# kalsifer-742/sunray

Measured on AMD Instinct MI355X. Metric: Mray/s (closest-hit + any-hit queries traversed per second), 1920x1080, 1 spp, 1M-triangle scene, higher is better.
Workload: dtype f32; 1 GPU; procedural heightfield 999714 triangles (257872 BVH nodes), 1920x1080, 1 spp, full reference frame per step: raytracing_ris + raytracing_final, 10 bounces, 16 RIS candidates, ReSTIR DI+GI on; primary_hit_hand_off=True, parallelism=single GPU, frames_in_flight=2, last_frame_crc32=7e278857

## Files before the change

### sunray_amd/csrc/bvh_build.cpp

```cpp
#include <algorithm>
#include <chrono>
#include <cmath>
#include <cstring>
#include <future>

#include "bvh_layout.h"
#include "host.h"

namespace srh {

namespace {

struct Aabb {
    float lo[3], hi[3];
    void reset() { for (int a = 0; a < 3; a++) { lo[a] = INFINITY; hi[a] = -INFINITY; } }
    void add(const float* p) { for (int a = 0; a < 3; a++) { lo[a] = std::min(lo[a], p[a]); hi[a] = std::max(hi[a], p[a]); } }
    void add(const Aabb& b) { for (int a = 0; a < 3; a++) { lo[a] = std::min(lo[a], b.lo[a]); hi[a] = std::max(hi[a], b.hi[a]); } }
    float half_area() const {
        const float dx = hi[0] - lo[0], dy = hi[1] - lo[1], dz = hi[2] - lo[2];
        if (!(dx >= 0.0f)) return 0.0f;
        return dx * dy + dy * dz + dz * dx;
    }
};

#ifndef SR_SAH_BINS
#define SR_SAH_BINS 16
#endif
constexpr int kBins = SR_SAH_BINS;
constexpr uint32_t kLeafMax = srl::kLeafMax;
constexpr uint32_t kParallelMin = 1u << 15;

struct Builder {
    std::vector<Aabb> bounds;
    std::vector<float> centroid[3];
    std::vector<uint32_t> order;
    uint32_t max_depth;
    double root_area = 1.0;

    struct Sub {
        std::vector<float> nodes;
        uint32_t depth = 0;
        double cost = 0.0;
    };

    explicit Builder(uint32_t md) : max_depth(md) {}

    static int leaf_ref(uint32_t first, uint32_t count) { return (int)~((first << 3) | count); }

    static void put_box(float* n, int which, const Aabb& b) {
        float lo[3], hi[3];
        for (int a = 0; a < 3; a++) {
            lo[a] = std::nextafter(b.lo[a], -INFINITY);
            hi[a] = std::nextafter(b.hi[a], INFINITY);
        }
        if (which == 0) { n[0] = lo[0]; n[1] = hi[0]; n[2] = lo[1]; n[3] = hi[1]; n[8] = lo[2]; n[9] = hi[2]; }
        else { n[4] = lo[0]; n[5] = hi[0]; n[6] = lo[1]; n[7] = hi[1]; n[10] = lo[2]; n[11] = hi[2]; }
    }
    static void put_child(float* n, int which, int ref) { memcpy(n + 12 + which, &ref, 4); }

    Aabb range_bounds(uint32_t first, uint32_t count) const {
        Aabb b; b.reset();
        for (uint32_t i = first; i < first + count; i++) b.add(bounds[order[i]]);
        return b;
    }

    uint32_t partition(uint32_t first, uint32_t count, uint32_t depth) {
        const uint32_t last = first + count;
        uint32_t need = 0;
        for (uint32_t c = (count + kLeafMax - 1) / kLeafMax; c > 1; c = (c + 1) / 2) need++;
        const bool force_median = depth + need + 1 >= max_depth;
        Aabb cb; cb.reset();
        for (uint32_t i = first; i < last; i++) {
            const uint32_t id = order[i];
            const float c[3] = {centroid[0][id], centroid[1][id], centroid[2][id]};
            cb.add(c);
        }
        int best_axis = -1, best_bin = -1;
        float best_cost = INFINITY;
        if (!force_median) {
            for (int ax = 0; ax < 3; ax++) {
                const float lo = cb.lo[ax], ext = cb.hi[ax] - cb.lo[ax];
                if (!(ext > 0.0f)) continue;
                const float scale = (float)kBins * (1.0f - 1e-6f) / ext;
                Aabb bb[kBins]; uint32_t bc[kBins];
                for (int b = 0; b < kBins; b++) { bb[b].reset(); bc[b] = 0; }
                for (uint32_t i = first; i < last; i++) {
                    const uint32_t id = order[i];
                    int b = (int)((centroid[ax][id] - lo) * scale);
                    b = b < 0 ? 0 : (b >= kBins ? kBins - 1 : b);
                    bb[b].add(bounds[id]); bc[b]++;
                }
                float ra[kBins]; uint32_t rc[kBins];
                Aabb acc; acc.reset(); uint32_t n = 0;
                for (int b = kBins - 1; b >= 1; b--) { acc.add(bb[b]); n += bc[b]; ra[b] = acc.half_area(); rc[b] = n; }
                acc.reset(); n = 0;
                for (int b = 0; b < kBins - 1; b++) {
                    acc.add(bb[b]); n += bc[b];
                    if (n == 0 || rc[b + 1] == 0) continue;
                    const float cost = acc.half_area() * (float)n + ra[b + 1] * (float)rc[b + 1];
                    if (cost < best_cost) { best_cost = cost; best_axis = ax; best_bin = b; }
                }
            }
        }
        if (best_axis >= 0) {
            const float lo = cb.lo[best_axis], ext = cb.hi[best_axis] - cb.lo[best_axis];
            const float scale = (float)kBins * (1.0f - 1e-6f) / ext;
            const std::vector<float>& cen = centroid[best_axis];
            auto mid_it = std::partition(order.begin() + first, order.begin() + last, [&](uint32_t id) {
                int b = (int)((cen[id] - lo) * scale);
                b = b < 0 ? 0 : (b >= kBins ? kBins - 1 : b);
                return b <= best_bin;
            });
            const uint32_t mid = (uint32_t)(mid_it - order.begin());
            if (mid != first && mid != last) return mid;
        }
        int ax = 0;
        float e = cb.hi[0] - cb.lo[0];
        for (int a = 1; a < 3; a++) if (cb.hi[a] - cb.lo[a] > e) { e = cb.hi[a] - cb.lo[a]; ax = a; }
        const uint32_t mid = first + count / 2;
        const std::vector<float>& cen = centroid[ax];
        std::nth_element(order.begin() + first, order.begin() + mid, order.begin() + last,
                         [&](uint32_t a, uint32_t b) { return cen[a] < cen[b] || (cen[a] == cen[b] && a < b); });
        return mid;
    }

    void build_sub(uint32_t first, uint32_t count, uint32_t depth, Sub& out) {
        const uint32_t mid = partition(first, count, depth);
        const uint32_t cnt[2] = {mid - first, first + count - mid};
        const uint32_t beg[2] = {first, mid};
        const bool par = cnt[0] >= kParallelMin && cnt[1] >= kParallelMin && depth < 4;
        if (!par) {
            emit_node(beg, cnt, depth, out, out);
            return;
        }
        Sub child[2];
        std::future<void> fut = std::async(std::launch::async, [&] { build_sub(beg[1], cnt[1], depth + 1, child[1]); });
        build_sub(beg[0], cnt[0], depth + 1, child[0]);
        fut.get();
        out.nodes.assign(16, 0.0f);
        uint32_t below = 0;
        for (int c = 0; c < 2; c++) {
            const Aabb cb = range_bounds(beg[c], cnt[c]);
            put_box(&out.nodes[0], c, cb);
            out.cost += cb.half_area() / root_area;
            const size_t at = out.nodes.size();
            const int off = (int)(at / 16);
            out.nodes.insert(out.nodes.end(), child[c].nodes.begin(), child[c].nodes.end());
            for (size_t n = at; n < out.nodes.size(); n += 16)
                for (int k = 0; k < 2; k++) {
                    int ref; memcpy(&ref, &out.nodes[n + 12 + k], 4);
                    if (ref >= 0) { ref += off; memcpy(&out.nodes[n + 12 + k], &ref, 4); }
                }
            std::vector<float>().swap(child[c].nodes);
            out.cost += child[c].cost;
            below = std::max(below, child[c].depth);
            put_child(&out.nodes[0], c, off);
        }
        out.depth = below + 1;
    }
    void emit_node(const uint32_t beg[2], const uint32_t cnt[2], uint32_t depth, Sub& arr, Sub& stats) {
        const size_t self = arr.nodes.size();
        arr.nodes.resize(self + 16, 0.0f);
        uint32_t below = 0;
        for (int c = 0; c < 2; c++) {
            const Aabb cb = range_bounds(beg[c], cnt[c]);
            put_box(&arr.nodes[self], c, cb);
            stats.cost += cb.half_area() / root_area * (cnt[c] <= kLeafMax ? (double)cnt[c] : 1.0);
            if (cnt[c] <= kLeafMax) { put_child(&arr.nodes[self], c, leaf_ref(beg[c], cnt[c])); continue; }
            const int ref = (int)(arr.nodes.size() / 16);
            Sub sub_stats;
            build_sub_inplace(beg[c], cnt[c], depth + 1, arr, sub_stats);
            stats.cost += sub_stats.cost;
            below = std::max(below, sub_stats.depth);
            put_child(&arr.nodes[self], c, ref);
        }
        stats.depth = below + 1;
    }
    void build_sub_inplace(uint32_t first, uint32_t count, uint32_t depth, Sub& arr, Sub& stats) {
        const uint32_t mid = partition(first, count, depth);
        const uint32_t cnt[2] = {mid - first, first + count - mid};
        const uint32_t beg[2] = {first, mid};
        emit_node(beg, cnt, depth, arr, stats);
    }
};

}

namespace {
struct Child4 { float lo[3], hi[3]; int ref; };
inline Child4 child_of(const float* n2, int which) {
    Child4 c;
    if (which == 0) { c.lo[0] = n2[0]; c.hi[0] = n2[1]; c.lo[1] = n2[2]; c.hi[1] = n2[3]; c.lo[2] = n2[8]; c.hi[2] = n2[9]; }
    else { c.lo[0] = n2[4]; c.hi[0] = n2[5]; c.lo[1] = n2[6]; c.hi[1] = n2[7]; c.lo[2] = n2[10]; c.hi[2] = n2[11]; }
    memcpy(&c.ref, n2 + 12 + which, 4);
    return c;
}
inline float area_of(const Child4& c) {
    const float dx = c.hi[0] - c.lo[0], dy = c.hi[1] - c.lo[1], dz = c.hi[2] - c.lo[2];
    if (!(dx >= 0.0f)) return -1.0f;
    return dx * dy + dy * dz + dz * dx;
}
constexpr double kGuardCells = 1.0 / 32.0;

struct Collapser {
    const std::vector<float>& n2;
    std::vector<uint32_t>& out;
    std::vector<uint8_t> height;
    uint32_t max_depth = 0;
    uint32_t height_of(int node2) {
        uint32_t h = 0;
        for (int c = 0; c < 2; c++) {
            int ref; memcpy(&ref, &n2[(size_t)node2 * 16 + 12 + c], 4);
            if (ref >= 0) h = std::max(h, height_of(ref));
        }
        height[node2] = (uint8_t)(h + 1);
        return h + 1;
    }
    uint32_t need_of(const Child4& c) const { return c.ref >= 0 ? height[c.ref] : 0u; }
    uint32_t emit(int node2, uint32_t depth, uint32_t budget, int* out_index) {
        constexpr int W = srl::kBvhWidth;
        Child4 kids[W];
        int nk = 0;
        kids[nk++] = child_of(&n2[(size_t)node2 * 16], 0);
        kids[nk++] = child_of(&n2[(size_t)node2 * 16], 1);
        while (nk < W) {
            int best = -1; float best_area = -1.0f;
            for (int i = 0; i < nk; i++) if (kids[i].ref >= 0) { const float a = area_of(kids[i]); if (a > best_area) { best_area = a; best = i; } }
            if (best < 0) break;
            const Child4 ca = child_of(&n2[(size_t)kids[best].ref * 16], 0), cb = child_of(&n2[(size_t)kids[best].ref * 16], 1);
            bool fits = need_of(ca) + (uint32_t)nk <= budget && need_of(cb) + (uint32_t)nk <= budget;
            for (int i = 0; i < nk && fits; i++) if (i != best && need_of(kids[i]) + (uint32_t)nk > budget) fits = false;
            if (!fits) break;
            kids[best] = ca;
            kids[nk++] = cb;
        }
        bool real[W];
        int n_real = 0;
        float lo_n[3] = {INFINITY, INFINITY, INFINITY}, hi_n[3] = {-INFINITY, -INFINITY, -INFINITY};
        for (int i = 0; i < W; i++) real[i] = false;
        for (int i = 0; i < nk; i++) {
            const bool empty_leaf = kids[i].ref < 0 && ((~(uint32_t)kids[i].ref) & 7u) == 0u;
            real[i] = !empty_leaf;
            if (!real[i]) continue;
            n_real++;
            for (int a = 0; a < 3; a++) { lo_n[a] = std::min(lo_n[a], kids[i].lo[a]); hi_n[a] = std::max(hi_n[a], kids[i].hi[a]); }
        }
        const size_t self = out.size();
        *out_index = (int)(self / srl::kNodeDwords);
        out.resize(self + srl::kNodeDwords, 0u);
        max_depth = std::max(max_depth, depth);
        uint32_t plane[6 * srl::kPlaneDwords];
        for (auto& v : plane) v = 0u;
        uint32_t exps = 0;
        float origin[3] = {0.0f, 0.0f, 0.0f};
        if (n_real > 0) {
            for (int a = 0; a < 3; a++) {
                origin[a] = std::nextafter(lo_n[a] - (hi_n[a] - lo_n[a]) * (1.0f / 2048.0f), -INFINITY);
                const float ext = hi_n[a] - origin[a];
                int e = -126;
                if (ext > 0.0f && ext / 255.0f > 0.0f) { int fe; (void)std::frexp(ext / 255.0f, &fe); e = std::max(fe, -126); }
                for (;;) {
                    const float scale = std::ldexp(1.0f, e);
                    bool ok = true;
                    for (int i = 0; i < nk && ok; i++) {
                        if (!real[i]) continue;
                        int qh = (int)std::ceil(((double)kids[i].hi[a] - (double)origin[a]) / (double)scale + kGuardCells);
                        qh = std::max(qh, 0);
                        while (qh <= 255 && fmaf((float)qh, scale, origin[a]) < kids[i].hi[a]) qh++;
                        if (qh > 255) ok = false;
                    }
                    if (ok) break;
                    e++;
                }
                const float scale = std::ldexp(1.0f, e);
                exps |= (uint32_t)(e + 127) << (8 * a);
                for (int i = 0; i < W; i++) {
                    uint32_t ql = 255u, qh = 0u;
                    if (i < nk && real[i]) {
                        int l = (int)std::floor(((double)kids[i].lo[a] - (double)origin[a]) / (double)scale - kGuardCells);
                        l = std::min(std::max(l, 0), 255);
                        while (l > 0 && fmaf((float)l, scale, origin[a]) > kids[i].lo[a]) l--;
                        int h = (int)std::ceil(((double)kids[i].hi[a] - (double)origin[a]) / (double)scale + kGuardCells);
                        h = std::max(h, 0);
                        while (fmaf((float)h, scale, origin[a]) < kids[i].hi[a]) h++;
                        ql = (uint32_t)l; qh = (uint32_t)h;
                    }
                    plane[a * srl::kPlaneDwords + i / 4] |= ql << (8 * (i % 4));
                    plane[(3 + a) * srl::kPlaneDwords + i / 4] |= qh << (8 * (i % 4));
                }
            }
        } else {
            for (int a = 0; a < 3; a++) {
                for (int d = 0; d < srl::kPlaneDwords; d++) { plane[a * srl::kPlaneDwords + d] = 0xFFFFFFFFu; plane[(3 + a) * srl::kPlaneDwords + d] = 0u; }
                exps |= 127u << (8 * a);
            }
        }
        uint32_t below = 0;
        int refs[W];
        for (int i = 0; i < W; i++) {
            refs[i] = Builder::leaf_ref(0, 0);
            if (i < nk && real[i]) {
                if (kids[i].ref >= 0) {
                    int idx = 0;
                    below = std::max(below, emit(kids[i].ref, depth + 1, budget - (uint32_t)(n_real - 1), &idx));
                    refs[i] = idx;
                } else refs[i] = kids[i].ref;
            }
        }
        uint32_t* q = &out[self];
        memcpy(q + 0, origin, 12); q[3] = exps;
        memcpy(q + srl::kPlaneOffset, plane, sizeof(plane));
        memcpy(q + srl::kChildOffset, refs, sizeof(refs));
        return below + (uint32_t)std::max(n_real - 1, 0);
    }
};
}

static void collapse_to_bvh4(BvhResult& res, uint32_t stack_budget) {
    res.nodes.clear();
    Collapser c{res.nodes2, res.nodes, {}, 0};
    c.height.assign(res.nodes2.size() / 16, 0);
    c.height_of(0);
    int root = 0;
    res.max_stack = c.emit(0, 1, stack_budget, &root);
    res.max_depth = c.max_depth;
    res.n_nodes = (uint32_t)(res.nodes.size() / srl::kNodeDwords);
}

void flatten_instances(const std::vector<HostMesh>& meshes, const FrameInstanceData& fid, std::vector<BuildTri>& out) {
    out.clear();
    out.reserve(fid.n_triangles);
    for (uint32_t ii = 0; ii < fid.instances.size(); ii++) {
        const HostInstance& inst = fid.instances[ii];
        const HostMesh& mesh = meshes[inst.mesh_slot];
        const float* m = inst.o2w.m;
        const uint32_t nprim = mesh.n_indices / 3;
        for (uint32_t p = 0; p < nprim; p++) {
            float w[3][3];
            for (int j = 0; j < 3; j++) {
                const float* q = mesh.vertices[mesh.indices[3 * p + j]].position;
                w[j][0] = ((m[0] * q[0] + m[1] * q[1]) + m[2] * q[2]) + m[3] * 1.0f;
                w[j][1] = ((m[4] * q[0] + m[5] * q[1]) + m[6] * q[2]) + m[7] * 1.0f;
                w[j][2] = ((m[8] * q[0] + m[9] * q[1]) + m[10] * q[2]) + m[11] * 1.0f;
            }
            BuildTri t;
            for (int a = 0; a < 3; a++) { t.v0[a] = w[0][a]; t.e1[a] = w[1][a] - w[0][a]; t.e2[a] = w[2][a] - w[0][a]; }
            t.prim = p; t.inst = ii; t.gid = inst.tri_offset + p;
            out.push_back(t);
        }
    }
}

namespace {
void build_core(Builder& b, uint32_t n, const Aabb& root, uint32_t max_depth, BvhResult& res) {
    b.root_area = std::max((double)root.half_area(), 1e-30);
    Builder::Sub top;
    if (n <= kLeafMax) {
        top.nodes.assign(16, 0.0f);
        if (n > 0) Builder::put_box(top.nodes.data(), 0, root);
        else { float* q = top.nodes.data(); q[0] = q[2] = q[8] = INFINITY; q[1] = q[3] = q[9] = -INFINITY; }
        { float* q = top.nodes.data(); q[4] = q[6] = q[10] = INFINITY; q[5] = q[7] = q[11] = -INFINITY; }
        Builder::put_child(top.nodes.data(), 0, Builder::leaf_ref(0, n));
        Builder::put_child(top.nodes.data(), 1, Builder::leaf_ref(0, 0));
        top.depth = 1;
        top.cost = (double)n;
    } else {
        b.build_sub(0, n, 0, top);
    }
    res.nodes2.swap(top.nodes);
    res.sah_cost = (float)top.cost;
    collapse_to_bvh4(res, max_depth);
    res.order = b.order;
}
}

void build_bvh(const std::vector<BuildTri>& tris, uint32_t max_depth, BvhResult& res) {
    const auto t_start = std::chrono::steady_clock::now();
    const uint32_t n = (uint32_t)tris.size();
    Builder b(max_depth);
    b.bounds.resize(n);
    for (int a = 0; a < 3; a++) b.centroid[a].resize(n);
    b.order.resize(n);
    Aabb root; root.reset();
    for (uint32_t i = 0; i < n; i++) {
        const BuildTri& t = tris[i];
        float p1[3], p2[3];
        for (int a = 0; a < 3; a++) { p1[a] = t.v0[a] + t.e1[a]; p2[a] = t.v0[a] + t.e2[a]; }
        Aabb bb; bb.reset(); bb.add(t.v0); bb.add(p1); bb.add(p2);
        for (int a = 0; a < 3; a++) {
            const float pad = 4e-6f * (std::fabs(t.e1[a]) + std::fabs(t.e2[a]));
            bb.lo[a] -= pad; bb.hi[a] += pad;
        }
        b.bounds[i] = bb;
        for (int a = 0; a < 3; a++) b.centroid[a][i] = 0.5f * bb.lo[a] + 0.5f * bb.hi[a];
        b.order[i] = i;
        root.add(bb);
    }
    build_core(b, n, root, max_depth, res);
    res.tris.resize((size_t)n * 12);
    for (uint32_t i = 0; i < n; i++) {
        const BuildTri& t = tris[b.order[i]];
        float* q = &res.tris[(size_t)i * 12];
        q[0] = t.v0[0]; q[1] = t.v0[1]; q[2] = t.v0[2]; q[3] = t.e1[0];
        q[4] = t.e1[1]; q[5] = t.e1[2]; q[6] = t.e2[0]; q[7] = t.e2[1];
        q[8] = t.e2[2];
        memcpy(q + 9, &t.gid, 4);
        q[10] = 0.0f; q[11] = 0.0f;
    }
    res.build_ms = std::chrono::duration<double, std::milli>(std::chrono::steady_clock::now() - t_start).count();
}

void build_bvh_boxes(const std::vector<BuildBox>& boxes, uint32_t max_depth, BvhResult& res) {
    const auto t_start = std::chrono::steady_clock::now();
    const uint32_t n = (uint32_t)boxes.size();
    Builder b(max_depth);
    b.bounds.resize(n);
    for (int a = 0; a < 3; a++) b.centroid[a].resize(n);
    b.order.resize(n);
    Aabb root; root.reset();
    for (uint32_t i = 0; i < n; i++) {
        Aabb bb;
        for (int a = 0; a < 3; a++) { bb.lo[a] = boxes[i].lo[a]; bb.hi[a] = boxes[i].hi[a]; }
        b.bounds[i] = bb;
        for (int a = 0; a < 3; a++) b.centroid[a][i] = 0.5f * bb.lo[a] + 0.5f * bb.hi[a];
        b.order[i] = i;
        root.add(bb);
    }
    build_core(b, n, root, max_depth, res);
    res.tris.clear();
    res.build_ms = std::chrono::duration<double, std::milli>(std::chrono::steady_clock::now() - t_start).count();
}

}
```

### sunray_amd/csrc/bvh_gpu.hip

```cpp
#include <hip/hip_runtime.h>

#include <cmath>
#include <cstddef>
#include <cstdint>
#include <type_traits>

#include <hipcub/hipcub.hpp>

#include <vector>

#include "bvh_gpu.h"
#include "bvh_layout.h"
#include "tl_record.h"
#include "traverse.h"

namespace srd {

__device__ __forceinline__ void triangle_vertices(const SrMeshInfo* meshes, const FlatInstance& inst, uint32_t prim, const SrVertex* v[3]) {
    const SrMeshInfo mi = meshes[inst.mesh_slot];
    const uint32_t* idx = (const uint32_t*)(uintptr_t)mi.indices;
    const SrVertex* vtx = (const SrVertex*)(uintptr_t)mi.vertices;
    for (int j = 0; j < 3; j++) v[j] = vtx + idx[3 * prim + j];
}

__device__ __forceinline__ void world_triangle(const SrMeshInfo* meshes, const FlatInstance& inst, uint32_t prim, float v0[3], float e1[3], float e2[3],
                                               const SrVertex* v[3]) {
    triangle_vertices(meshes, inst, prim, v);
    const float* m = inst.o2w;
    float w[3][3];
    for (int j = 0; j < 3; j++) {
        const float* q = v[j]->position;
        w[j][0] = ((m[0] * q[0] + m[1] * q[1]) + m[2] * q[2]) + m[3] * 1.0f;
        w[j][1] = ((m[4] * q[0] + m[5] * q[1]) + m[6] * q[2]) + m[7] * 1.0f;
        w[j][2] = ((m[8] * q[0] + m[9] * q[1]) + m[10] * q[2]) + m[11] * 1.0f;
    }
    for (int a = 0; a < 3; a++) { v0[a] = w[0][a]; e1[a] = w[1][a] - w[0][a]; e2[a] = w[2][a] - w[0][a]; }
}

__device__ __forceinline__ void write_shade(float4* shade, const SrVertex* const v[3], float tail_y, float tail_z, float tail_w) {
    shade[0] = make_float4(v[0]->normal[0], v[0]->normal[1], v[0]->normal[2], v[1]->normal[0]);
    shade[1] = make_float4(v[1]->normal[1], v[1]->normal[2], v[2]->normal[0], v[2]->normal[1]);
    shade[2] = make_float4(v[2]->normal[2], tail_y, tail_z, tail_w);
}
__device__ __forceinline__ void write_shade_tex(float4* q, const SrVertex* const v[3]) {
    q[0] = make_float4(v[0]->base_color_tex_coord[0], v[0]->base_color_tex_coord[1], v[1]->base_color_tex_coord[0], v[1]->base_color_tex_coord[1]);
    q[1] = make_float4(v[2]->base_color_tex_coord[0], v[2]->base_color_tex_coord[1], v[0]->normal_tex_coord[0], v[0]->normal_tex_coord[1]);
    q[2] = make_float4(v[1]->normal_tex_coord[0], v[1]->normal_tex_coord[1], v[2]->normal_tex_coord[0], v[2]->normal_tex_coord[1]);
    q[3] = make_float4(v[0]->tangent[0], v[0]->tangent[1], v[0]->tangent[2], v[0]->tangent[3] >= 0.0f ? 1.0f : -1.0f);
    q[4] = make_float4(v[1]->tangent[0], v[1]->tangent[1], v[1]->tangent[2], v[2]->tangent[0]);
    q[5] = make_float4(v[2]->tangent[1], v[2]->tangent[2], 0.0f, 0.0f);
}

template <bool RESHADE, bool TEX>
__global__ void flatten_slots_kernel(float4* tris, typename std::conditional<RESHADE, float4*, const float4*>::type shade, const SrMeshInfo* meshes,
                                     const FlatInstance* instances, uint32_t n_tris, float4* shade_tex) {
    const uint32_t slot = blockIdx.x * blockDim.x + threadIdx.x;
    if (slot >= n_tris) return;
    const uint32_t gid = __float_as_uint(tris[(size_t)slot * 3 + 2].y);
    float4 tail = make_float4(0.0f, 0.0f, 0.0f, 0.0f);
    if constexpr (RESHADE) tail = shade[(size_t)slot * 3 + 2]; else tail.y = shade[(size_t)slot * 3 + 2].y;
    const uint32_t ii = __float_as_uint(tail.y);
    const FlatInstance inst = instances[ii];
    if (gid < inst.tri_offset) return;
    float v0[3], e1[3], e2[3];
    const SrVertex* v[3];
    world_triangle(meshes, inst, gid - inst.tri_offset, v0, e1, e2, v);
    tris[(size_t)slot * 3 + 0] = make_float4(v0[0], v0[1], v0[2], e1[0]);
    tris[(size_t)slot * 3 + 1] = make_float4(e1[1], e1[2], e2[0], e2[1]);
    tris[(size_t)slot * 3 + 2] = make_float4(e2[2], __uint_as_float(gid), 0.0f, 0.0f);
    if constexpr (RESHADE) {
        write_shade(shade + (size_t)slot * 3, v, tail.y, tail.z, tail.w);
        if constexpr (TEX) write_shade_tex(shade_tex + (size_t)slot * 6, v);
    }
}

__device__ __forceinline__ void tri_box(const float4* tris, uint32_t slot, float lo[3], float hi[3]) {
    const float4 a = tris[(size_t)slot * 3 + 0], b = tris[(size_t)slot * 3 + 1], c = tris[(size_t)slot * 3 + 2];
    const float v0[3] = {a.x, a.y, a.z}, e1[3] = {a.w, b.x, b.y}, e2[3] = {b.z, b.w, c.x};
    for (int k = 0; k < 3; k++) {
        const float p1 = v0[k] + e1[k], p2 = v0[k] + e2[k];
        const float pad = 4e-6f * (fabsf(e1[k]) + fabsf(e2[k]));
        const float l = fminf(v0[k], fminf(p1, p2)) - pad, h = fmaxf(v0[k], fmaxf(p1, p2)) + pad;
        lo[k] = fminf(lo[k], nextafterf(l, -INFINITY));
        hi[k] = fmaxf(hi[k], nextafterf(h, INFINITY));
    }
}

struct TriPrims {
    const float4* tris;
    __device__ __forceinline__ void add(uint32_t i, float lo[3], float hi[3]) const { tri_box(tris, i, lo, hi); }
};
struct BoxPrims {
    const float* boxes;
    const uint32_t* map;
    __device__ __forceinline__ void add(uint32_t i, float lo[3], float hi[3]) const {
        const float* b = boxes + (size_t)(map ? map[i] : i) * 6;
        for (int a = 0; a < 3; a++) { lo[a] = fminf(lo[a], b[a]); hi[a] = fmaxf(hi[a], b[3 + a]); }
    }
};

struct VertPrims {
    const float4* tris;
    __device__ __forceinline__ void add(uint32_t i, float lo[3], float hi[3]) const {
        const float4 a = tris[(size_t)i * 3 + 0], b = tris[(size_t)i * 3 + 1], c = tris[(size_t)i * 3 + 2];
        const float v0[3] = {a.x, a.y, a.z}, v1[3] = {a.w, b.x, b.y}, v2[3] = {b.z, b.w, c.x};
        for (int k = 0; k < 3; k++) {
            const float e1 = v1[k] - v0[k], e2 = v2[k] - v0[k];
            const float p1 = v0[k] + e1, p2 = v0[k] + e2;
            const float pad = 4e-6f * (fabsf(e1) + fabsf(e2));
            const float l = fminf(fminf(v0[k], fminf(p1, p2)), fminf(v1[k], v2[k])) - pad;
            const float h = fmaxf(fmaxf(v0[k], fmaxf(p1, p2)), fmaxf(v1[k], v2[k])) + pad;
            lo[k] = fminf(lo[k], nextafterf(l, -INFINITY));
            hi[k] = fmaxf(hi[k], nextafterf(h, INFINITY));
        }
    }
};

constexpr double kGuardCells = 1.0 / 32.0;

template <class Prims>
__global__ void refit_level_kernel(uint32_t* nodes, const Prims prims, float* node_box, const uint32_t* level_nodes, uint32_t first, uint32_t count) {
    constexpr int W = srl::kBvhWidth;
    const uint32_t i = blockIdx.x * blockDim.x + threadIdx.x;
    if (i >= count) return;
    const uint32_t node = level_nodes ? level_nodes[first + i] : first + i;
    uint32_t* q = nodes + (size_t)node * srl::kNodeDwords;
    float lo[W][3], hi[W][3];
    bool real[W];
    float lo_n[3] = {INFINITY, INFINITY, INFINITY}, hi_n[3] = {-INFINITY, -INFINITY, -INFINITY};
    int n_real = 0;
    for (int c = 0; c < W; c++) {
        const int ref = (int)q[srl::kChildOffset + c];
        for (int a = 0; a < 3; a++) { lo[c][a] = INFINITY; hi[c][a] = -INFINITY; }
        real[c] = false;
        if (ref >= 0) {
            const float* b = node_box + (size_t)ref * 6;
            for (int a = 0; a < 3; a++) { lo[c][a] = b[a]; hi[c][a] = b[3 + a]; }
            real[c] = lo[c][0] <= hi[c][0];
        } else {
            const uint32_t v = ~(uint32_t)ref, t0 = v >> 3, cnt = v & 7u;
            for (uint32_t t = 0; t < cnt; t++) prims.add(t0 + t, lo[c], hi[c]);
            real[c] = cnt != 0u;
        }
        if (!real[c]) continue;
        n_real++;
        for (int a = 0; a < 3; a++) { lo_n[a] = fminf(lo_n[a], lo[c][a]); hi_n[a] = fmaxf(hi_n[a], hi[c][a]); }
    }
    uint32_t plane[6 * srl::kPlaneDwords], exps = 0;
    for (int k = 0; k < 6 * srl::kPlaneDwords; k++) plane[k] = 0u;
    float origin[3] = {0.0f, 0.0f, 0.0f};
    if (n_real > 0) {
        for (int a = 0; a < 3; a++) {
            origin[a] = nextafterf(lo_n[a] - (hi_n[a] - lo_n[a]) * (1.0f / 2048.0f), -INFINITY);
            const float ext = hi_n[a] - origin[a];
            int e = -126;
            if (ext > 0.0f && ext < INFINITY && ext / 255.0f > 0.0f) { int fe; (void)frexpf(ext / 255.0f, &fe); e = max(fe, -126); }
            if (!(ext < INFINITY)) e = 127;
            for (; e < 127; e++) {
                const float scale = ldexpf(1.0f, e);
                bool ok = true;
                for (int c = 0; c < W && ok; c++) {
                    if (!real[c]) continue;
                    int qh = (int)ceil(((double)hi[c][a] - (double)origin[a]) / (double)scale + kGuardCells);
                    qh = max(qh, 0);
                    while (qh <= 255 && fmaf((float)qh, scale, origin[a]) < hi[c][a]) qh++;
                    if (qh > 255) ok = false;
                }
                if (ok) break;
            }
            const float scale = ldexpf(1.0f, e);
            exps |= (uint32_t)(e + 127) << (8 * a);
            for (int c = 0; c < W; c++) {
                uint32_t ql = 255u, qh = 0u;
                if (real[c]) {
                    int l = (int)floor(((double)lo[c][a] - (double)origin[a]) / (double)scale - kGuardCells);
                    l = min(max(l, 0), 255);
                    while (l > 0 && fmaf((float)l, scale, origin[a]) > lo[c][a]) l--;
                    int h = (int)ceil(((double)hi[c][a] - (double)origin[a]) / (double)scale + kGuardCells);
                    h = min(max(h, 0), 255);
                    while (h < 255 && fmaf((float)h, scale, origin[a]) < hi[c][a]) h++;
                    ql = (uint32_t)l; qh = (uint32_t)h;
                }
                plane[a * srl::kPlaneDwords + c / 4] |= ql << (8 * (c % 4));
                plane[(3 + a) * srl::kPlaneDwords + c / 4] |= qh << (8 * (c % 4));
            }
        }
    } else {
        for (int a = 0; a < 3; a++) {
            for (int d = 0; d < srl::kPlaneDwords; d++) { plane[a * srl::kPlaneDwords + d] = 0xFFFFFFFFu; plane[(3 + a) * srl::kPlaneDwords + d] = 0u; }
            exps |= 127u << (8 * a);
        }
    }
    q[0] = __float_as_uint(origin[0]); q[1] = __float_as_uint(origin[1]); q[2] = __float_as_uint(origin[2]); q[3] = exps;
    for (int k = 0; k < 6 * srl::kPlaneDwords; k++) q[srl::kPlaneOffset + k] = plane[k];
    float* b = node_box + (size_t)node * 6;
    for (int a = 0; a < 3; a++) { b[a] = lo_n[a]; b[3 + a] = hi_n[a]; }
}


__device__ __forceinline__ uint32_t find_instance(const FlatInstance* inst, uint32_t n_inst, uint32_t gid) {
    uint32_t lo = 0, hi = n_inst;
    while (hi - lo > 1) { const uint32_t mid = (lo + hi) >> 1; if (inst[mid].tri_offset <= gid) lo = mid; else hi = mid; }
    return lo;
}
__device__ __forceinline__ uint32_t enc_f(float f) { const uint32_t b = __float_as_uint(f); return (b & 0x80000000u) ? ~b : (b | 0x80000000u); }
__device__ __forceinline__ float dec_f(uint32_t e) { return __uint_as_float((e & 0x80000000u) ? (e & 0x7FFFFFFFu) : ~e); }

__global__ void lbvh_prims_kernel(const SrMeshInfo* meshes, const FlatInstance* instances, uint32_t n_inst, uint32_t n_tris, float4* W, float4* cent,
                                  uint32_t* bounds_enc) {
    const uint32_t gid = blockIdx.x * blockDim.x + threadIdx.x;
    float lo[3] = {INFINITY, INFINITY, INFINITY}, hi[3] = {-INFINITY, -INFINITY, -INFINITY};
    if (gid < n_tris) {
        const uint32_t ii = find_instance(instances, n_inst, gid);
        const FlatInstance inst = instances[ii];
        float v0[3], e1[3], e2[3];
        const SrVertex* v[3];
        world_triangle(meshes, inst, gid - inst.tri_offset, v0, e1, e2, v);
        W[(size_t)gid * 3 + 0] = make_float4(v0[0], v0[1], v0[2], e1[0]);
        W[(size_t)gid * 3 + 1] = make_float4(e1[1], e1[2], e2[0], e2[1]);
        W[(size_t)gid * 3 + 2] = make_float4(e2[2], __uint_as_float(gid), 0.0f, 0.0f);
        tri_box(W, gid, lo, hi);
        cent[gid] = make_float4(0.5f * lo[0] + 0.5f * hi[0], 0.5f * lo[1] + 0.5f * hi[1], 0.5f * lo[2] + 0.5f * hi[2], __uint_as_float(ii));
    }
    for (int a = 0; a < 3; a++) {
        float l = lo[a], h = hi[a];
        for (int o = 32; o > 0; o >>= 1) { l = fminf(l, __shfl_xor(l, o)); h = fmaxf(h, __shfl_xor(h, o)); }
        if ((threadIdx.x & 63) == 0) {
            if (l <= h) { atomicMin(bounds_enc + a, enc_f(l)); atomicMax(bounds_enc + 3 + a, enc_f(h)); }
        }
    }
}

__device__ __forceinline__ unsigned long long spread21(uint32_t v) {
    unsigned long long x = v & 0x1FFFFFull;
    x = (x | x << 32) & 0x1F00000000FFFFull;
    x = (x | x << 16) & 0x1F0000FF0000FFull;
    x = (x | x << 8) & 0x100F00F00F00F00Full;
    x = (x | x << 4) & 0x10C30C30C30C30C3ull;
    x = (x | x << 2) & 0x1249249249249249ull;
    return x;
}

__global__ void lbvh_morton_kernel(const float4* cent, const uint32_t* bounds_enc, uint32_t n_tris, unsigned long long* keys, uint32_t* vals) {
    const uint32_t gid = blockIdx.x * blockDim.x + threadIdx.x;
    if (gid >= n_tris) return;
    const float4 c = cent[gid];
    const float p[3] = {c.x, c.y, c.z};
    uint32_t q[3];
    for (int a = 0; a < 3; a++) {
        const float lo = dec_f(bounds_enc[a]), hi = dec_f(bounds_enc[3 + a]);
        const float ext = hi - lo;
        float t = ext > 0.0f ? (p[a] - lo) / ext : 0.0f;
        t = fminf(fmaxf(t, 0.0f), 1.0f);
        q[a] = min((uint32_t)(t * 2097152.0f), 2097151u);
    }
    keys[gid] = spread21(q[0]) | (spread21(q[1]) << 1) | (spread21(q[2]) << 2);
    vals[gid] = gid;
}

__device__ __forceinline__ int lbvh_delta(const unsigned long long* keys, int n, int i, int j) {
    if (j < 0 || j >= n) return -1;
    const unsigned long long a = keys[i], b = keys[j];
    if (a != b) return __clzll((long long)(a ^ b));
    return 64 + __clz(i ^ j);
}

__global__ void lbvh_hierarchy_kernel(const unsigned long long* keys, int n, int2* children, uint32_t* parent_of_inner, uint32_t* parent_of_leaf, uint2* range) {
    const int i = blockIdx.x * blockDim.x + threadIdx.x;
    if (i >= n - 1) return;
    const int d = lbvh_delta(keys, n, i, i + 1) - lbvh_delta(keys, n, i, i - 1) >= 0 ? 1 : -1;
    const int dmin = lbvh_delta(keys, n, i, i - d);
    int lmax = 2;
    while (lbvh_delta(keys, n, i, i + lmax * d) > dmin) lmax <<= 1;
    int l = 0;
    for (int t = lmax >> 1; t >= 1; t >>= 1) if (lbvh_delta(keys, n, i, i + (l + t) * d) > dmin) l += t;
    const int j = i + l * d;
    const int dnode = lbvh_delta(keys, n, i, j);
    int s = 0;
    for (int t = l;;) {
        t = (t + 1) >> 1;
        if (lbvh_delta(keys, n, i, i + (s + t) * d) > dnode) s += t;
        if (t <= 1) break;
    }
    const int gamma = i + s * d + min(d, 0);
    const int first = min(i, j), last = max(i, j);
    int2 ch;
    ch.x = first == gamma ? ~gamma : gamma;
    ch.y = last == gamma + 1 ? ~(gamma + 1) : gamma + 1;
    children[i] = ch;
    range[i] = make_uint2((uint32_t)first, (uint32_t)last);
    if (ch.x >= 0) parent_of_inner[ch.x] = (uint32_t)i; else parent_of_leaf[~ch.x] = (uint32_t)i;
    if (ch.y >= 0) parent_of_inner[ch.y] = (uint32_t)i; else parent_of_leaf[~ch.y] = (uint32_t)i;
    if (i == 0) parent_of_inner[0] = 0xFFFFFFFFu;
}

template <class Prims>
__global__ void lbvh_fit_kernel(const Prims prims, const uint32_t* sorted_gid, int n, const int2* children, const uint32_t* parent_of_inner,
                                const uint32_t* parent_of_leaf, const uint2* range, float* bin_box, uint32_t* bin_height, uint32_t* bin_size,
                                uint32_t* flags) {
    const int i = blockIdx.x * blockDim.x + threadIdx.x;
    if (i >= n) return;
    uint32_t node = parent_of_leaf[i];
    while (node != 0xFFFFFFFFu) {
        __threadfence();
        if (atomicAdd(flags + node, 1u) == 0u) return;
        __threadfence();
        const int2 ch = children[node];
        float lo[3] = {INFINITY, INFINITY, INFINITY}, hi[3] = {-INFINITY, -INFINITY, -INFINITY};
        uint32_t h = 0, size = 0;
        const int cc[2] = {ch.x, ch.y};
        for (int c = 0; c < 2; c++) {
            if (cc[c] < 0) { prims.add(sorted_gid[~cc[c]], lo, hi); size += 1u; }
            else {
                const volatile float* b = bin_box + (size_t)cc[c] * 6;
                for (int a = 0; a < 3; a++) { lo[a] = fminf(lo[a], b[a]); hi[a] = fmaxf(hi[a], b[3 + a]); }
                h = max(h, ((const volatile uint32_t*)bin_height)[cc[c]]);
                if (!range) size += ((const volatile uint32_t*)bin_size)[cc[c]];
            }
        }
        if (range) { const uint2 r = range[node]; size = r.y - r.x + 1u; }
        float* b = bin_box + (size_t)node * 6;
        for (int a = 0; a < 3; a++) { b[a] = lo[a]; b[3 + a] = hi[a]; }
        bin_size[node] = size;
        bin_height[node] = (size <= srl::kLeafMax) ? 0u : h + 1u;
        node = parent_of_inner[node];
    }
}

constexpr uint32_t kNoNode = 0xFFFFFFFFu;
constexpr int kMaxBinaryWalk = 4096 + 64;

__device__ __forceinline__ bool binary_ref_ok(int ref, uint32_t n) { return ref < 0 ? (uint32_t)~ref < n : (uint32_t)ref + 1u < n; }

__host__ __device__ __forceinline__ uint32_t median_height(uint32_t k) {
    uint32_t h = 0;
    for (int i = 0; i < 32 && k > srl::kLeafMax; i++) { k = (k + 1u) >> 1; h++; }
    return h;
}

__global__ void rebalance_links_kernel(const int2* children, const uint32_t* bin_size, const uint32_t* bin_height, uint32_t n, uint32_t root, uint4* link,
                                       uint2* leaf_link) {
    const uint32_t u = blockIdx.x * blockDim.x + threadIdx.x;
    if (u + 1u >= n) return;
    const int2 ch = children[u];
    if (!binary_ref_ok(ch.x, n) || !binary_ref_ok(ch.y, n)) return;
    const uint32_t sl = ch.x < 0 ? 1u : bin_size[ch.x], sr = ch.y < 0 ? 1u : bin_size[ch.y];
    if (ch.x < 0) leaf_link[~ch.x] = make_uint2(u, 0u); else { link[ch.x].x = u; link[ch.x].z = 0u; }
    if (ch.y < 0) leaf_link[~ch.y] = make_uint2(u, sl); else { link[ch.y].x = u; link[ch.y].z = sl; }
    link[u].y = min(bin_height[u], 0xFFFFu) | (1u + max(median_height(sl), median_height(sr))) << 16;
    link[u].w = sl;
    if (u == root) { link[u].x = kNoNode; link[u].z = 0u; }
}

__global__ void rebalance_walk_kernel(const uint4* link, const uint2* leaf_link, const uint32_t* bin_size, uint32_t n, int cap, uint32_t* leaf_at_pos,
                                      uint32_t* inner_at_gap, uint2* rb_range, uint32_t* rb_gap, uint32_t* error) {
    const uint32_t t = blockIdx.x * blockDim.x + threadIdx.x;
    if (t >= 2u * n - 1u) return;
    const bool leaf = t < n;
    const uint32_t x = leaf ? t : t - n;
    const uint32_t u0 = leaf ? leaf_link[x].x : x;
    if (!leaf) rb_range[x] = make_uint2(0u, 0u);
    int depth = 0;
    uint32_t cur = u0;
    for (; depth < kMaxBinaryWalk; depth++) {
        if (cur >= n - 1u) { atomicExch(error, 1u); return; }
        const uint32_t p = link[cur].x;
        if (p == kNoNode) break;
        cur = p;
    }
    if (depth >= kMaxBinaryWalk) { atomicExch(error, 1u); return; }
    uint32_t acc = leaf ? leaf_link[x].y : 0u, r = kNoNode, rel = 0u;
    cur = u0;
    for (int d = depth; d >= 0; d--) {
        const uint4 L = link[cur];
        const int allowance = cap - d, h = (int)(L.y & 0xFFFFu), need = (int)(L.y >> 16);
        if (h <= allowance) r = kNoNode;
        else if (need > allowance) { r = cur; rel = acc; }
        acc += L.z;
        cur = L.x;
    }
    if (r == kNoNode) return;
    if (leaf) { if (acc < n) leaf_at_pos[acc] = x; return; }
    const uint32_t gap = acc + link[x].w - 1u;
    if (gap >= n - 1u) { atomicExch(error, 1u); return; }
    inner_at_gap[gap] = x;
    rb_range[x] = make_uint2(acc - rel, bin_size[r]);
    rb_gap[x] = gap | (r == x ? 0x80000000u : 0u);
}

__device__ __forceinline__ uint32_t median_gap(uint32_t lo, uint32_t hi) { return lo + ((hi - lo + 1u) >> 1) - 1u; }
__device__ __forceinline__ int median_child(uint32_t lo, uint32_t hi, const uint32_t* leaf_at_pos, const uint32_t* inner_at_gap) {
    return hi - lo == 1u ? ~(int)leaf_at_pos[lo] : (int)inner_at_gap[median_gap(lo, hi)];
}

__global__ void rebalance_rebuild_kernel(const uint4* link, const uint2* rb_range, const uint32_t* rb_gap, const uint32_t* leaf_at_pos,
                                         const uint32_t* inner_at_gap, uint32_t n, int2* children, uint32_t* stat) {
    const uint32_t x = blockIdx.x * blockDim.x + threadIdx.x;
    if (x + 1u >= n) return;
    const uint2 R = rb_range[x];
    if (R.y < 2u || (uint64_t)R.x + R.y > n) return;
    const uint32_t g = rb_gap[x] & 0x7FFFFFFFu;
    uint32_t lo = R.x, hi = R.x + R.y;
    for (int i = 0; i < 64 && hi - lo >= 2u; i++) {
        const uint32_t m = median_gap(lo, hi);
        if (g == m) break;
        if (g < m) hi = m + 1u; else lo = m + 1u;
    }
    if (hi - lo < 2u || median_gap(lo, hi) != g) return;
    const uint32_t mid = g + 1u;
    const int2 ch = make_int2(median_child(lo, mid, leaf_at_pos, inner_at_gap), median_child(mid, hi, leaf_at_pos, inner_at_gap));
    if (!binary_ref_ok(ch.x, n) || !binary_ref_ok(ch.y, n)) { atomicExch(stat + 4, 1u); return; }
    children[x] = ch;
    if (rb_gap[x] & 0x80000000u) {
        const uint32_t top = inner_at_gap[median_gap(R.x, R.x + R.y)];
        const uint4 L = link[x];
        if (top + 1u >= n || (L.x != kNoNode && L.x + 1u >= n)) { atomicExch(stat + 4, 1u); return; }
        if (L.x == kNoNode) stat[0] = top;
        else ((int*)children)[2 * (size_t)L.x + (L.z ? 1 : 0)] = (int)top;
        atomicAdd(stat + 1, 1u);
        atomicAdd(stat + 2, R.y);
    }
}

__global__ void rebalance_parents_kernel(const int2* children, uint32_t n, const uint32_t* root, uint32_t* parent_of_inner, uint32_t* parent_of_leaf) {
    const uint32_t u = blockIdx.x * blockDim.x + threadIdx.x;
    if (u + 1u >= n) return;
    const int2 ch = children[u];
    if (!binary_ref_ok(ch.x, n) || !binary_ref_ok(ch.y, n)) return;
    if (ch.x >= 0) parent_of_inner[ch.x] = u; else parent_of_leaf[~ch.x] = u;
    if (ch.y >= 0) parent_of_inner[ch.y] = u; else parent_of_leaf[~ch.y] = u;
    if (u == *root) parent_of_inner[u] = kNoNode;
}

__global__ void rebalance_finish_kernel(const uint32_t* bin_height, uint32_t n, uint32_t* stat) {
    if (blockIdx.x != 0 || threadIdx.x != 0) return;
    stat[3] = stat[0] + 1u < n ? bin_height[stat[0]] : kNoNode;
}

struct LbvhKid { int ref; uint32_t size; float area; uint32_t need; bool inner; };

__device__ __forceinline__ LbvhKid lbvh_kid(int ref, const uint32_t* bin_size, const float* bin_box, const uint32_t* bin_height) {
    LbvhKid k;
    k.ref = ref; k.area = 0.0f; k.need = 0; k.inner = false;
    if (ref < 0) { k.size = 1; return k; }
    k.size = bin_size[ref];
    if (k.size <= srl::kLeafMax) return k;
    const float* b = bin_box + (size_t)ref * 6;
    const float dx = b[3] - b[0], dy = b[4] - b[1], dz = b[5] - b[2];
    k.area = dx * dy + dy * dz + dz * dx; k.need = bin_height[ref]; k.inner = true;
    return k;
}

__global__ void lbvh_collapse_kernel(uint32_t* nodes, uint32_t level_first, uint32_t level_count, uint32_t node_cap, int* bin_of_node, uint32_t* budget_of_node,
                                     uint32_t* prefix_of_node, uint32_t* first_of_node, const int2* children, const uint32_t* bin_size, const float* bin_box,
                                     const uint32_t* bin_height, uint32_t* slot_of_sorted, uint32_t* counters) {
    const uint32_t t = blockIdx.x * blockDim.x + threadIdx.x;
    if (t >= level_count) return;
    const uint32_t self = level_first + t;
    const int bin = bin_of_node[self];
    const uint32_t budget = budget_of_node[self];
    constexpr int W = srl::kBvhWidth;
    LbvhKid kids[W];
    int nk = 0;
    const int2 ch = children[bin];
    kids[nk++] = lbvh_kid(ch.x, bin_size, bin_box, bin_height);
    kids[nk++] = lbvh_kid(ch.y, bin_size, bin_box, bin_height);
    while (nk < W) {
        int best = -1; float best_area = -1.0f;
        for (int i = 0; i < nk; i++) if (kids[i].inner && kids[i].area > best_area) { best_area = kids[i].area; best = i; }
        if (best < 0) break;
        const int2 cb = children[kids[best].ref];
        const LbvhKid ka = lbvh_kid(cb.x, bin_size, bin_box, bin_height), kb = lbvh_kid(cb.y, bin_size, bin_box, bin_height);
        bool fits = ka.need + (uint32_t)nk <= budget && kb.need + (uint32_t)nk <= budget;
        for (int i = 0; i < nk && fits; i++) if (i != best && kids[i].need + (uint32_t)nk > budget) fits = false;
        if (!fits) break;
        kids[best] = ka;
        kids[nk++] = kb;
    }
    uint32_t* q = nodes + (size_t)self * srl::kNodeDwords;
    for (int k = 0; k < srl::kNodeDwords; k++) q[k] = 0u;
    const uint32_t mine = prefix_of_node[self] + (uint32_t)(nk - 1);
    atomicMax(counters + 1, mine);
    uint32_t first = first_of_node[self];
    for (int i = 0; i < W; i++) {
        uint32_t ref = 0xFFFFFFFFu;
        if (i < nk) {
            if (kids[i].inner) {
                const uint32_t idx = atomicAdd(counters + 0, 1u);
                if (idx < node_cap) {
                    bin_of_node[idx] = kids[i].ref;
                    budget_of_node[idx] = budget - (uint32_t)(nk - 1);
                    prefix_of_node[idx] = mine;
                    first_of_node[idx] = first;
                    ref = idx;
                } else { atomicExch(counters + 2, 1u); }
            } else {
// ... 582 lines not shown
```

### sunray_amd/csrc/bvh_layout.h

```cpp
#pragma once
namespace srl {
constexpr int kBvhWidth = 4;
constexpr int kPlaneDwords = kBvhWidth / 4;
constexpr int kPlaneOffset = 4;
constexpr int kChildOffset = 12;
constexpr int kNodeDwords = 16;
constexpr int kNodeBytes = kNodeDwords * 4;
#ifndef SR_LEAF_MAX
#define SR_LEAF_MAX 2
#endif
constexpr unsigned kLeafMax = SR_LEAF_MAX;
}
```

### sunray_amd/csrc/kernels.hip

```cpp
#include <algorithm>
#include "kernels.h"

namespace srd {

constexpr int kBlock = 256;
constexpr int kPassBlock = 64;
constexpr int kPassTile = 8;
static int lds_extra_rows(int two_level) { return two_level ? kWsRowsTl : kWsRows; }
#ifndef SR_PASS_WAVES
#define SR_PASS_WAVES 4
#endif
constexpr int kPassWaves = SR_PASS_WAVES;
#ifndef SR_TL_PASS_WAVES
#define SR_TL_PASS_WAVES 3
#endif
constexpr int pass_waves(int v) { return (v & 4) ? (kPassWaves < SR_TL_PASS_WAVES ? kPassWaves : SR_TL_PASS_WAVES) : kPassWaves; }

SRD void flush_counter(unsigned long long* counters, int which, uint32_t v) {
    for (int off = 32; off > 0; off >>= 1) v += __shfl_xor(v, off);
    if ((threadIdx.x & 63) == 0 && v) atomicAdd(counters + (blockIdx.x & (kCounterSlots - 1u)) * kCounterStride + which, (unsigned long long)v);
}

template <bool ANY, bool STATS, bool TL>
__global__ __launch_bounds__(kBlock) void trace_rays_kernel(DevScene sc, const SrRay* __restrict__ rays, uint32_t n,
                                                            SrHit* __restrict__ hits, uint32_t* __restrict__ occluded) {
    extern __shared__ __attribute__((aligned(16))) int s_stack[];
    const int lane = threadIdx.x & 63;
    int* stack = s_stack + threadIdx.x;
    uint32_t n_queries = 0;
    TravStats st; st.boxes = 0; st.tris = 0;
    const uint32_t base = (blockIdx.x * (kBlock / 64) + (threadIdx.x >> 6)) * 64u;
    if (base < n) {
        const uint32_t i = base + lane;
        const uint32_t ic = i < n ? i : n - 1u;
        const float4 ra = reinterpret_cast<const float4*>(rays)[(size_t)ic * 2 + 0];
        const float4 rb = reinterpret_cast<const float4*>(rays)[(size_t)ic * 2 + 1];
        TravHit h;
        const bool found = traverse_ws<ANY, STATS, TL>(sc, i < n, mk3(ra.x, ra.y, ra.z), mk3(rb.x, rb.y, rb.z), ra.w, rb.w, h, stack, kBlock, st);
        if (i < n) {
            n_queries++;
            if (ANY) occluded[i] = found ? 1u : 0u;
            else {
                float4 o;
                o.x = h.t; o.y = h.u; o.z = h.v; o.w = __uint_as_float(h.gid);
                reinterpret_cast<float4*>(hits)[i] = o;
            }
        }
    }
    flush_counter(sc.counters, (ANY ? 1 : 0), n_queries);
    if (STATS) { flush_counter(sc.counters, 2, st.boxes); flush_counter(sc.counters, 3, st.tris); }
}

__global__ __launch_bounds__(kBlock) void shade_closest_hit_kernel(DevScene sc, const SrHit* __restrict__ hits, uint32_t n,
                                                                   SrRayPayload* __restrict__ out) {
    const uint32_t i = blockIdx.x * kBlock + threadIdx.x;
    if (i >= n) return;
    const SrHit h = hits[i];
    TravHit th;
    th.t = h.t; th.u = h.u; th.v = h.v; th.gid = (h.t < 0.0f || h.tri >= sc.n_tris) ? 0xFFFFFFFFu : h.tri;
    th.slot = 0u; th.inst = 0u;
    const bool two_level = sc.tl_instances != nullptr;
    if (th.gid != 0xFFFFFFFFu) { if (two_level) tl_locate(sc, th.gid, th.slot, th.inst); else th.slot = sc.slot_of_gid[th.gid]; }
    const Payload p = two_level ? shade_hit<true, true>(sc, th) : shade_hit<true, false>(sc, th);
    SrRayPayload o;
    o.emission[0] = p.emission.x; o.emission[1] = p.emission.y; o.emission[2] = p.emission.z;
    o.dist = p.dist; o.albedo_packed = p.albedo_packed; o.normal_packed = p.normal_packed;
    o.material_info = p.material_info; o.transmission_ior_packed = p.transmission_ior_packed;
    out[i] = o;
}

__global__ __launch_bounds__(kBlock) void any_hit_kernel(DevScene sc, const SrHit* __restrict__ hits, uint32_t n, uint32_t* __restrict__ ignored) {
    const uint32_t i = blockIdx.x * kBlock + threadIdx.x;
    if (i >= n) return;
    const SrHit h = hits[i];
    const bool hit = !(h.t < 0.0f) && h.tri < sc.n_tris;
    uint32_t slot = 0u, inst = 0u;
    if (hit) { if (sc.tl_instances) tl_locate(sc, h.tri, slot, inst); else slot = sc.slot_of_gid[h.tri]; }
    ignored[i] = (hit && any_hit_ignores(sc, slot, h.u, h.v)) ? 1u : 0u;
}

struct Row4 { float x, y, z, w; };
SRD float dot4(const float* r, float x, float y, float z, float w) { return ((r[0] * x + r[1] * y) + r[2] * z) + r[3] * w; }

SRD void primary_ray(const SrMatrices& m, uint32_t px, uint32_t py, uint32_t W, uint32_t H, f3& origin, f3& dir, f2& inUV) {
    const float cx = (float)px + 0.5f, cy = (float)py + 0.5f;
    inUV.x = cx / (float)W; inUV.y = cy / (float)H;
    const float dx = inUV.x * 2.0f - 1.0f, dy = inUV.y * 2.0f - 1.0f;
    const float* vi = m.view_inverse;
    const float* pi = m.proj_inverse;
    origin = mk3(dot4(vi + 0, 0.0f, 0.0f, 0.0f, 1.0f), dot4(vi + 4, 0.0f, 0.0f, 0.0f, 1.0f), dot4(vi + 8, 0.0f, 0.0f, 0.0f, 1.0f));
    const f3 target = mk3(dot4(pi + 0, dx, dy, 1.0f, 1.0f), dot4(pi + 4, dx, dy, 1.0f, 1.0f), dot4(pi + 8, dx, dy, 1.0f, 1.0f));
    const f3 tn = norm3(target);
    dir = mk3(dot4(vi + 0, tn.x, tn.y, tn.z, 0.0f), dot4(vi + 4, tn.x, tn.y, tn.z, 0.0f), dot4(vi + 8, tn.x, tn.y, tn.z, 0.0f));
}

struct PixelCtx {
    const PassArgs& a;
    int* stack;
    uint32_t n_q;
    TravStats st;
};
constexpr uint32_t kCountAny = 1u, kCountClosest = 1u << 16, kCountReusedAny = 1u << 31;
SRD uint32_t counted_any(uint32_t n_q) { return n_q & 0xFFFFu; }
SRD uint32_t counted_closest(uint32_t n_q) { return (n_q >> 16) & 0x7FFFu; }

template <int V, bool ANY>
SRD bool trace_ray(PixelCtx& cx, bool want, f3 o, f3 d, float tmin, float tmax, TravHit& h) {
    return traverse_ws<ANY, (V & 1) != 0, (V & 4) != 0>(cx.a.sc, want, o, d, tmin, tmax, h, cx.stack, kPassBlock, cx.st);
}
template <int V>
SRD Payload trace_closest_shaded(PixelCtx& cx, f3 o, f3 d, float tmin, float tmax) {
    TravHit h;
    trace_ray<V, false>(cx, true, o, d, tmin, tmax, h);
    cx.n_q += kCountClosest;
    return shade_hit<(V & 2) != 0, (V & 4) != 0>(cx.a.sc, h);
}
template <int V>
SRD float trace_shadow(PixelCtx& cx, f3 o, f3 d, float dist) {
    if (dist > 0.002f) {
        TravHit h;
        cx.n_q += kCountAny;
        return trace_ray<V, true>(cx, true, o, d, 0.001f, dist - 0.001f, h) ? 1.0f : -1.0f;
    }
    return -1.0f;
}

SRD void store_gbuffer(const PassArgs& a, uint32_t pix, float depth, f3 n, float rough, f3 diffuse, float mx, float my) {
    a.depth_img[pix] = (uint16_t)f32_to_f16_bits(depth);
    a.normal_img[pix] = pack_rgba8_snorm(n.x, n.y, n.z, rough);
    a.diffuse_img[pix] = pack_b10g11r11(diffuse.x, diffuse.y, diffuse.z);
    a.motion_vec_img[pix] = pack_half_2x16(mx, my);
}
SRD f3 load_normal(const PassArgs& a, uint32_t pix) {
    const uint32_t v = a.normal_img[pix];
    return mk3(unsnorm8(v), unsnorm8(v >> 8), unsnorm8(v >> 16));
}
SRD float load_depth(const PassArgs& a, uint32_t pix) { return f16_bits_to_f32(a.depth_img[pix]); }

SRD void zero_reservoir(SrReservoir& r) {
    r.light_pos[0] = r.light_pos[1] = r.light_pos[2] = 0.0f; r.w_sum = 0.0f;
    r.light_normal[0] = r.light_normal[1] = r.light_normal[2] = 0.0f; r.M = 0.0f;
    r.light_idx = 0u; r.W = 0.0f; r.hit_normal_packed = 0u; r.depth = 0.0f;
}
SRD void zero_reservoir_gi(SrReservoirGI& r) {
    r.sample_pos[0] = r.sample_pos[1] = r.sample_pos[2] = 0.0f; r.w_sum = 0.0f;
    r.sample_radiance[0] = r.sample_radiance[1] = r.sample_radiance[2] = 0.0f; r.M = 0.0f;
    r.sample_normal_packed = 0u; r.W = 0.0f; r.hit_normal_packed = 0u; r.depth = 0.0f;
}
template <typename T>
SRD T load48(const T* p) {
    T r;
    const float4* s = reinterpret_cast<const float4*>(p);
    float4* d = reinterpret_cast<float4*>(&r);
    d[0] = s[0]; d[1] = s[1]; d[2] = s[2];
    return r;
}
template <typename T>
SRD void store48(T* p, const T& v) {
    float4* d = reinterpret_cast<float4*>(p);
    const float4* s = reinterpret_cast<const float4*>(&v);
    d[0] = s[0]; d[1] = s[1]; d[2] = s[2];
}

SRD void store_payload(SrRayPayload* p, const Payload& v) {
    float4* d = reinterpret_cast<float4*>(p);
    d[0] = make_float4(v.emission.x, v.emission.y, v.emission.z, v.dist);
    d[1] = make_float4(__uint_as_float(v.albedo_packed), __uint_as_float(v.normal_packed), __uint_as_float(v.material_info), __uint_as_float(v.transmission_ior_packed));
}
SRD Payload load_payload(const SrRayPayload* p) {
    const float4* s = reinterpret_cast<const float4*>(p);
    const float4 a = s[0], b = s[1];
    Payload v;
    v.emission = mk3(a.x, a.y, a.z); v.dist = a.w;
    v.albedo_packed = __float_as_uint(b.x); v.normal_packed = __float_as_uint(b.y);
    v.material_info = __float_as_uint(b.z); v.transmission_ior_packed = __float_as_uint(b.w);
    return v;
}

SRD f3 light_emission(const DevScene& sc, uint32_t indirection_idx) { return ld3(sc.lights[indirection_idx].emission); }
struct LightTri { f3 wv0, wv1, wv2, emission, normal; float area; };
SRD LightTri fetch_light(const DevScene& sc, uint32_t idx) {
    const float4* q = reinterpret_cast<const float4*>(sc.lights + idx);
    const float4 a = q[0], b = q[1], c = q[2], e = q[3];
    LightTri r;
    r.wv0 = mk3(a.x, a.y, a.z); r.area = a.w;
    r.wv1 = mk3(b.x, b.y, b.z);
    r.wv2 = mk3(c.x, c.y, c.z);
    r.emission = mk3(e.x, e.y, e.z);
    r.normal = mk3(b.w, c.w, e.w);
    return r;
}

SRD bool thread_pixel(const PassArgs& a, uint32_t& px, uint32_t& py, uint32_t& cost_slot) {
    const uint32_t b = blockIdx.x;
    const uint32_t xcd = b & 7u, k = b >> 3;
    cost_slot = 0xFFFFFFFFu;
    uint32_t tile;
    if (a.tile_order) {
        tile = a.tile_order[xcd * a.order_cap + k];
    } else {
        const uint32_t bx0 = (a.tiles_x * xcd) >> 3, bx1 = (a.tiles_x * (xcd + 1u)) >> 3;
        const uint32_t bw = bx1 - bx0;
        if (bw == 0u || k >= bw * a.tiles_y) return false;
        tile = (k / bw) * a.tiles_x + bx0 + k % bw;
    }
    if (tile >= a.tiles_x * a.tiles_y) return false;
    cost_slot = tile;
    const uint32_t tx = tile % a.tiles_x, ty = tile / a.tiles_x;
    const uint32_t l = threadIdx.x;
    px = a.x0 + tx * (uint32_t)kPassTile + (l & 7u);
    py = a.y0 + ty * (uint32_t)kPassTile + (l >> 3);
    return px < a.x1 && py < a.y1;
}
SRD void record_tile_cost(const PassArgs& a, uint32_t cost_slot, unsigned long long t_start) {
    if (a.tile_cost && cost_slot != 0xFFFFFFFFu && threadIdx.x == 0) {
        const unsigned long long dt = __builtin_amdgcn_s_memtime() - t_start;
        a.tile_cost[cost_slot] = (uint32_t)(dt > 0xFFFFFFFFull ? 0xFFFFFFFFull : dt);
    }
}

SRD uint32_t band_cap_cols_dev(uint32_t tiles_x) { return min(tiles_x, (tiles_x * 3u) / 16u + 2u); }

constexpr uint32_t kMaxScheduleCols = 1024;
__global__ void tile_order_kernel(const uint32_t* __restrict__ cost, uint32_t* __restrict__ order, uint32_t tiles_x, uint32_t tiles_y, uint32_t order_cap) {
    __shared__ unsigned long long s_col[kMaxScheduleCols];
    __shared__ uint32_t s_b[9];
    __shared__ unsigned long long s_sum[2];
    const uint32_t band = blockIdx.x;
    const uint32_t cap_cols = band_cap_cols_dev(tiles_x);
    const bool balance = tiles_x <= kMaxScheduleCols && tiles_x >= 16u;
    if (balance) {
        for (uint32_t x = threadIdx.x; x < tiles_x; x += blockDim.x) {
            unsigned long long c = 0;
            for (uint32_t y = 0; y < tiles_y; y++) c += cost[(size_t)y * tiles_x + x];
            s_col[x] = c + 1ull;
        }
    }
    if (threadIdx.x < 2) s_sum[threadIdx.x] = 0;
    __syncthreads();
    if (threadIdx.x == 0) {
        s_b[0] = 0u; s_b[8] = tiles_x;
        if (balance) {
            unsigned long long total = 0;
            for (uint32_t x = 0; x < tiles_x; x++) total += s_col[x];
            unsigned long long run = 0;
            uint32_t x = 0;
            for (uint32_t i = 1; i < 8u; i++) {
                const unsigned long long target = total / 8ull * i;
                while (x < tiles_x && run + s_col[x] / 2ull < target) run += s_col[x++];
                uint32_t cut = x;
                cut = max(cut, s_b[i - 1] + 1u);
                cut = min(cut, s_b[i - 1] + cap_cols);
                cut = max(cut, tiles_x > (8u - i) * cap_cols ? tiles_x - (8u - i) * cap_cols : 0u);
                cut = min(cut, tiles_x - (8u - i));
                while (x < cut) run += s_col[x++];
                s_b[i] = cut;
            }
        } else {
            for (uint32_t i = 1; i < 8u; i++) s_b[i] = (tiles_x * i) >> 3;
        }
    }
    __syncthreads();
    const uint32_t bx0 = s_b[band], bx1 = s_b[band + 1];
    const uint32_t bw = bx1 - bx0, n = bw * tiles_y;
    uint32_t* const mine = order + (size_t)band * order_cap;
    const uint32_t q = max(tiles_y / 4u, 1u) * bw;
    unsigned long long head = 0, tail = 0;
    for (uint32_t i = threadIdx.x; i < q; i += blockDim.x) {
        const uint32_t r = i / bw, x = bx0 + i % bw;
        head += cost[(size_t)r * tiles_x + x];
        tail += cost[(size_t)(tiles_y - 1u - r) * tiles_x + x];
    }
    atomicAdd(&s_sum[0], head);
    atomicAdd(&s_sum[1], tail);
    __syncthreads();
    const bool bottom_up = s_sum[1] > s_sum[0];
    __shared__ unsigned long long s_key[1024];
    __shared__ uint16_t s_row_at[1024];
    if (tiles_y <= 1024u) {
        for (uint32_t r = threadIdx.x; r < tiles_y; r += blockDim.x) {
            unsigned long long k = 0;
            for (uint32_t x = 0; x < bw; x++) k = max(k, (unsigned long long)cost[(size_t)r * tiles_x + bx0 + x]);
            s_key[r] = k;
        }
        __syncthreads();
        if (threadIdx.x == 0) {
            uint32_t rs = 0;
            for (uint32_t r = 1; r < tiles_y; r++) if (s_key[r] > s_key[rs]) rs = r;
            rs = bottom_up ? (rs > 4u ? rs - 4u : 0u) : min(rs + 4u, tiles_y - 1u);
            uint32_t at = 0;
            if (bottom_up) { for (uint32_t r = rs; r < tiles_y; r++) s_row_at[at++] = (uint16_t)r; for (uint32_t r = rs; r-- > 0;) s_row_at[at++] = (uint16_t)r; }
            else { for (uint32_t r = rs + 1; r-- > 0;) s_row_at[at++] = (uint16_t)r; for (uint32_t r = rs + 1; r < tiles_y; r++) s_row_at[at++] = (uint16_t)r; }
        }
        __syncthreads();
        for (uint32_t i = threadIdx.x; i < order_cap; i += blockDim.x) {
            uint32_t t = 0xFFFFFFFFu;
            if (i < n) t = (uint32_t)s_row_at[i / bw] * tiles_x + bx0 + i % bw;
            mine[i] = t;
        }
        return;
    }
    for (uint32_t i = threadIdx.x; i < order_cap; i += blockDim.x) {
        uint32_t t = 0xFFFFFFFFu;
        if (i < n) {
            const uint32_t r = i / bw, x = i % bw;
            t = (bottom_up ? tiles_y - 1u - r : r) * tiles_x + bx0 + x;
        }
        mine[i] = t;
    }
}

template <int V, bool ANY>
SRD bool ws_query(PixelCtx& cx, bool want, f3 o, f3 d, float tmin, float tmax, TravHit& h) {
    if (want) cx.n_q += ANY ? kCountAny : kCountClosest;
    return trace_ray<V, ANY>(cx, want, o, d, tmin, tmax, h);
}

template <int V>
__global__ __launch_bounds__(kPassBlock, pass_waves(V)) void ris_kernel(const PassArgs a) {
    extern __shared__ __attribute__((aligned(16))) int s_stack[];
    PixelCtx cx{a, s_stack + threadIdx.x, 0u, {0u, 0u}};
    const DevScene& sc = a.sc;
    uint32_t px = 0, py = 0, cost_slot = 0;
    const unsigned long long t_start = __builtin_amdgcn_s_memtime();
    const bool active = thread_pixel(a, px, py, cost_slot);
    if (active) {
        const uint32_t W = a.width, H = a.height;
        const uint32_t pix = py * W + px;
        const uint32_t cur_buf = a.frame_count & 1u, hist_buf = cur_buf ^ 1u;
        SrReservoir* reservoir_cur = a.reservoirs[cur_buf];
        const SrReservoir* reservoir_hist = a.reservoirs[hist_buf];
        SrReservoirGI* reservoir_gi_cur = a.reservoirs_gi[cur_buf];
        const SrReservoirGI* reservoir_gi_hist = a.reservoirs_gi[hist_buf];
        const float* pvp = a.mats.prev_view_proj;

        uint32_t rng = init_rng(px, py, a.frame_count, W);
        f3 origin, direction; f2 inUV;
        primary_ray(a.mats, px, py, W, H, origin, direction, inUV);
        f3 rayOrigin = origin, rayDir = direction;

        Payload prd;
        f3 hitPos = splat(0.0f), hit_normal = splat(0.0f), hit_albedo = splat(0.0f);
        float roughness = 0.5f, metallic = 0.0f;
        f3 V_view = splat(0.0f);
        float prev_u = -1.0f, prev_v = -1.0f;
        bool prev_valid = false, found_diffuse_surface = false;
        float virtual_distance = 0.0f;

        for (uint32_t vb = 0; vb < a.cfg.virtual_bounces; vb++) {
            prd = trace_closest_shaded<V>(cx, rayOrigin, rayDir, 0.001f, 10000.0f);
            if (vb == 0u && a.primary_payload) store_payload(a.primary_payload + pix, prd);
            if (prd.dist < 0.0f) break;
            hitPos = rayOrigin + rayDir * prd.dist;
            hit_normal = unpack_normal(prd.normal_packed);
            hit_albedo = unpack_unorm_rgb(prd.albedo_packed);
            const f2 mat_info = unpack_half_2x16(prd.material_info);
            roughness = fmaxf(mat_info.x, 0.01f);
            metallic = clampf(mat_info.y, 0.0f, 1.0f);
            const f2 trans_ior = unpack_half_2x16(prd.transmission_ior_packed);
            const float transmission = trans_ior.x;
            V_view = -rayDir;
            virtual_distance += prd.dist;
            if (transmission > 0.5f) {
                const float ior = fmaxf(trans_ior.y, 1.0f);
                const bool is_inside = dot3(rayDir, hit_normal) > 0.0f;
                const f3 N = is_inside ? -hit_normal : hit_normal;
                const float eta = is_inside ? (ior / 1.0f) : (1.0f / ior);
                const float cos_theta = fminf(dot3(-rayDir, N), 1.0f);
                float R0 = (1.0f - eta) / (1.0f + eta);
                R0 = R0 * R0;
                float fresnel = R0 + (1.0f - R0) * pow5f(1.0f - cos_theta);
                const f3 refracted = refract3(rayDir, N, eta);
                if (len3(refracted) < 0.01f) fresnel = 1.0f;
                if (rnd(rng) < fresnel) rayDir = reflect3(rayDir, N);
                else rayDir = refracted;
                rayOrigin = hitPos + rayDir * 0.001f;
            } else if (metallic > 0.9f && roughness < 0.1f) {
                rayOrigin = hitPos + hit_normal * 0.001f;
                rayDir = reflect3(rayDir, hit_normal);
            } else {
                const f3 vwp = origin + direction * virtual_distance;
                const float clip_x = dot4(pvp + 0, vwp.x, vwp.y, vwp.z, 1.0f);
                const float clip_y = dot4(pvp + 4, vwp.x, vwp.y, vwp.z, 1.0f);
                const float clip_w = dot4(pvp + 12, vwp.x, vwp.y, vwp.z, 1.0f);
                prev_valid = clip_w > 0.01f;
                if (prev_valid) {
                    const float iw = 1.0f / clip_w;
                    prev_u = (clip_x * iw) * 0.5f + 0.5f;
                    prev_v = (clip_y * iw) * 0.5f + 0.5f;
                    prev_valid = (prev_u >= 0.0f && prev_v >= 0.0f) && (prev_u < 1.0f && prev_v < 1.0f);
                }
                const float mvx = prev_valid ? (inUV.x - prev_u) : (inUV.x + 2.0f);
                const float mvy = prev_valid ? (inUV.y - prev_v) : (inUV.y + 2.0f);
                const f3 denoiser_albedo = lerp3(hit_albedo, splat(1.0f), metallic);
                store_gbuffer(a, pix, virtual_distance, hit_normal, roughness, denoiser_albedo, mvx, mvy);
                found_diffuse_surface = true;
                break;
            }
        }

        if (!found_diffuse_surface) {
            store_gbuffer(a, pix, 100000.0f, splat(0.0f), 0.0f, splat(0.0f), 0.0f, 0.0f);
            SrReservoir empty; zero_reservoir(empty);
            store48(reservoir_cur + pix, empty);
        } else {
            SrReservoir current_r; zero_reservoir(current_r);
            const uint32_t num_lights = sc.num_lights;
            if (num_lights > 0 && roughness > 0.2f) {
                for (uint32_t i = 0; i < a.cfg.ris_candidates; i++) {
                    uint32_t cand_idx = (uint32_t)(rnd(rng) * (float)num_lights);
                    if (cand_idx > num_lights - 1) cand_idx = num_lights - 1;
                    const LightTri lt = fetch_light(sc, cand_idx);
                    const float cand_area = lt.area;
                    const float sqr1 = sqrtf(rnd(rng));
                    const float u = 1.0f - sqr1;
                    const float v = rnd(rng) * sqr1;
                    const float w = 1.0f - u - v;
                    const f3 cand_pos = lt.wv0 * u + lt.wv1 * v + lt.wv2 * w;
                    const f3 cand_normal = lt.normal;
                    const f3 f_y = eval_unshadowed_light(hitPos, hit_normal, V_view, hit_albedo, roughness, metallic, lt.emission, cand_pos, cand_normal);
                    const float p_hat = maxc(f_y);
                    const float p_y = 1.0f / fmaxf((float)num_lights * cand_area, 0.0001f);
                    current_r.w_sum += (p_hat / p_y);
                    current_r.M += 1.0f;
                    if (rnd(rng) < ((p_hat / p_y) / fmaxf(current_r.w_sum, 0.0001f))) {
                        current_r.light_idx = cand_idx;
                        st3(current_r.light_pos, cand_pos);
                        st3(current_r.light_normal, cand_normal);
                    }
                }
                if (current_r.w_sum > 0.0f) {
                    const f3 fw = eval_unshadowed_light(hitPos, hit_normal, V_view, hit_albedo, roughness, metallic,
                                                        light_emission(sc, current_r.light_idx), ld3(current_r.light_pos), ld3(current_r.light_normal));
                    current_r.W = current_r.w_sum / fmaxf(current_r.M * maxc(fw), 0.0001f);
                }
                if (a.frame_count > 0 && prev_valid) {
                    const float ppx = prev_u * (float)W, ppy = prev_v * (float)H;
                    const float j0 = rnd(rng), j1 = rnd(rng);
                    const int pcx = (int)(ppx + (j0 - 0.5f)), pcy = (int)(ppy + (j1 - 0.5f));
                    if (pcx >= 0 && pcy >= 0 && pcx < (int)W && pcy < (int)H) {
                        SrReservoir history_r = load48(reservoir_hist + ((uint32_t)pcy * W + (uint32_t)pcx));
                        history_r.M = fminf(history_r.M, 10.0f);
                        history_r.W = fminf(history_r.W, 20.0f);
                        const f3 hist_normal = unpack_normal(history_r.hit_normal_packed);
                        const float normal_conf_di = smoothstepf(0.9f, 0.99f, dot3(hit_normal, hist_normal));
                        const float depth_diff_di = fabsf(virtual_distance - history_r.depth) / fmaxf(virtual_distance, 1e-4f);
                        const float depth_conf_di = 1.0f - smoothstepf(0.05f, 0.20f, depth_diff_di);
                        const float conf_di = normal_conf_di * depth_conf_di;
                        history_r.M *= conf_di;
                        if (history_r.W > 0.0f) {
                            history_r.light_idx = history_r.light_idx < num_lights - 1 ? history_r.light_idx : num_lights - 1;
                            const f3 fh = eval_unshadowed_light(hitPos, hit_normal, V_view, hit_albedo, roughness, metallic,
                                                                light_emission(sc, history_r.light_idx), ld3(history_r.light_pos), ld3(history_r.light_normal));
                            const float hist_rand = rnd(rng);
                            merge_reservoirs(current_r, history_r, maxc(fh), hist_rand);
                            const f3 fm = eval_unshadowed_light(hitPos, hit_normal, V_view, hit_albedo, roughness, metallic,
                                                                light_emission(sc, current_r.light_idx), ld3(current_r.light_pos), ld3(current_r.light_normal));
                            current_r.W = current_r.w_sum / fmaxf(current_r.M * maxc(fm), 0.0001f);
                        }
                    }
                }
            }
            if (current_r.W > 0.0f) {
                f3 vis_dir = ld3(current_r.light_pos) - hitPos;
                const float vis_dist = fmaxf(len3(vis_dir), 0.0001f);
                vis_dir = vis_dir / vis_dist;
                if (dot3(hit_normal, vis_dir) <= 0.0f) current_r.W = 0.0f;
                else {
                    prd.dist = trace_shadow<V>(cx, hitPos + hit_normal * 0.001f, vis_dir, vis_dist);
                    if (prd.dist >= 0.0f) current_r.W = 0.0f;
                }
            }
            current_r.hit_normal_packed = pack_normal(hit_normal);
            current_r.depth = virtual_distance;
            store48(reservoir_cur + pix, current_r);

            SrReservoirGI gi; zero_reservoir_gi(gi);
            const float gr1 = rnd(rng), gr2 = rnd(rng);
            const f3 gi_dir = get_random_bounce(hit_normal, gr1, gr2);
            const float gi_NdotL = fmaxf(dot3(hit_normal, gi_dir), 0.0f);
            if (gi_NdotL > 0.0f) {
                const f3 gi_origin = hitPos + hit_normal * 0.001f;
                prd = trace_closest_shaded<V>(cx, gi_origin, gi_dir, 0.001f, 10000.0f);
                f3 sample_pos = splat(0.0f), sample_normal = splat(0.0f), sample_radiance = splat(0.0f);
                if (prd.dist > 0.0f) {
                    sample_pos = gi_origin + gi_dir * prd.dist;
                    sample_normal = unpack_normal(prd.normal_packed);
                    const f3 x2_albedo = unpack_unorm_rgb(prd.albedo_packed);
                    sample_radiance = prd.emission;
                    if (num_lights > 0) {
                        uint32_t nee_idx = (uint32_t)(rnd(rng) * (float)num_lights);
                        if (nee_idx > num_lights - 1) nee_idx = num_lights - 1;
                        const LightTri lt = fetch_light(sc, nee_idx);
                        const float sq = sqrtf(rnd(rng));
                        const float nu = 1.0f - sq;
                        const float nv = rnd(rng) * sq;
                        const float nw = 1.0f - nu - nv;
                        const f3 nee_pos = lt.wv0 * nu + lt.wv1 * nv + lt.wv2 * nw;
                        const f3 nee_normal = lt.normal;
                        const float nee_area = lt.area;
                        f3 to_light = nee_pos - sample_pos;
                        const float nee_dist = fmaxf(len3(to_light), 0.0001f);
                        to_light = to_light / nee_dist;
                        const float nee_cos_surf = fmaxf(dot3(sample_normal, to_light), 0.0f);
                        const float nee_cos_light = fmaxf(dot3(nee_normal, -to_light), 0.0f);
                        if (nee_cos_surf > 0.0f && nee_cos_light > 0.0f) {
                            prd.dist = trace_shadow<V>(cx, sample_pos + sample_normal * 0.001f, to_light, nee_dist);
                            if (prd.dist < 0.0f) {
                                const float nee_pdf_sa = (nee_dist * nee_dist) / fmaxf(nee_cos_light * nee_area * (float)num_lights, 0.0001f);
                                sample_radiance = sample_radiance + (lt.emission * x2_albedo * nee_cos_surf) / (nee_pdf_sa * 3.14159f);
                            }
                        }
                    }
                }
                sample_radiance = vmin(sample_radiance, splat(5.0f));
                const float p_hat = gi_target_pdf(hitPos, hit_normal, hit_albedo, metallic, sample_pos, sample_radiance);
                const float pdf = gi_NdotL / 3.14159f;
                gi.M = 1.0f;
                gi.w_sum = (pdf > 0.0f) ? (p_hat / pdf) : 0.0f;
                gi.W = (p_hat > 0.0f) ? (gi.w_sum / (gi.M * p_hat)) : 0.0f;
                st3(gi.sample_pos, sample_pos);
                gi.sample_normal_packed = pack_normal(sample_normal);
                st3(gi.sample_radiance, sample_radiance);
            }
            if (a.frame_count > 0 && prev_valid) {
                const float ppx = prev_u * (float)W, ppy = prev_v * (float)H;
                const float j0 = rnd(rng), j1 = rnd(rng);
                const int gx = (int)(ppx + (j0 - 0.5f)), gy = (int)(ppy + (j1 - 0.5f));
                if (gx >= 0 && gy >= 0 && gx < (int)W && gy < (int)H) {
                    SrReservoirGI hgi = load48(reservoir_gi_hist + ((uint32_t)gy * W + (uint32_t)gx));
                    const f3 gi_hist_normal = unpack_normal(hgi.hit_normal_packed);
                    const float normal_conf = smoothstepf(0.8f, 0.95f, dot3(hit_normal, gi_hist_normal));
                    const float depth_diff = fabsf(virtual_distance - hgi.depth) / fmaxf(virtual_distance, 1e-4f);
                    const float depth_conf = 1.0f - smoothstepf(0.05f, 0.20f, depth_diff);
                    const float conf = normal_conf * depth_conf;
                    hgi.M = fminf(hgi.M, 12.0f) * conf;
                    hgi.W = fminf(hgi.W, 10.0f);
                    if (hgi.W > 0.0f && hgi.M > 0.0f) {
                        const float p_hat_hist = gi_target_pdf(hitPos, hit_normal, hit_albedo, metallic, ld3(hgi.sample_pos), ld3(hgi.sample_radiance));
                        const float mr = rnd(rng);
                        merge_reservoirs_gi(gi, hgi, p_hat_hist, 1.0f, mr);
                        const float p_hat_merged = gi_target_pdf(hitPos, hit_normal, hit_albedo, metallic, ld3(gi.sample_pos), ld3(gi.sample_radiance));
                        gi.W = (p_hat_merged > 1e-6f) ? (gi.w_sum / (gi.M * p_hat_merged)) : 0.0f;
                    }
                }
            }
            gi.hit_normal_packed = pack_normal(hit_normal);
            gi.depth = virtual_distance;
            store48(reservoir_gi_cur + pix, gi);
        }
    }
    record_tile_cost(a, cost_slot, t_start);
    if (!(a.cfg.flags & SR_TRACE_FLAG_UNCOUNTED)) {
        const bool counted = (a.cfg.count_rows == 0u || (py - a.cfg.count_y0) < a.cfg.count_rows) &&
                             (a.cfg.count_cols == 0u || (px - a.cfg.count_x0) < a.cfg.count_cols);
        flush_counter(sc.counters, 0, counted ? counted_closest(cx.n_q) : 0u);
        flush_counter(sc.counters, 1, counted ? counted_any(cx.n_q) : 0u);
        if (V & 1) { flush_counter(sc.counters, 2, counted ? cx.st.boxes : 0u); flush_counter(sc.counters, 3, counted ? cx.st.tris : 0u); }
    }
}
template <int V>
__global__ __launch_bounds__(kPassBlock, pass_waves(V)) void final_kernel(const PassArgs a) {
    extern __shared__ __attribute__((aligned(16))) int s_stack[];
    PixelCtx cx{a, s_stack + threadIdx.x, 0u, {0u, 0u}};
    const DevScene& sc = a.sc;
    uint32_t px = 0, py = 0, cost_slot = 0;
    const unsigned long long t_start = __builtin_amdgcn_s_memtime();
    const bool active = thread_pixel(a, px, py, cost_slot);
    const uint32_t W = a.width, H = a.height;
    const uint32_t pix = active ? py * W + px : 0u;
    const int ipx = (int)px, ipy = (int)py;
    const uint32_t cur_buf = a.frame_count & 1u;
    const SrReservoir* reservoir_cur = a.reservoirs[cur_buf];
    const SrReservoirGI* reservoir_gi_cur = a.reservoirs_gi[cur_buf];
    const uint32_t num_lights = sc.num_lights;

    uint32_t rng = init_rng(px, py, a.frame_count, W);
    const int BOUNCES = (int)a.cfg.max_bounces;
    const int SHADOW_BOUNCES = (int)a.cfg.shadow_bounces;
    f3 origin, rayDir0; f2 inUV;
    primary_ray(a.mats, px, py, W, H, origin, rayDir0, inUV);
    f3 rayOrigin = origin, rayDir = rayDir0;
    f3 throughput = splat(1.0f), radiance = splat(0.0f);
    bool restir_evaluated = (a.cfg.enable_restir == 0);
    bool prev_did_nee = false;
    Payload prd;
    TravHit h; bool occ;

    bool in_loop = active;
    for (int bounce = 0; bounce < BOUNCES; bounce++) {
        if (__builtin_amdgcn_ballot_w64(in_loop) == 0ull) break;
        const bool reuse_primary = bounce == 0 && a.primary_payload != nullptr;
        if (!reuse_primary) ws_query<V, false>(cx, in_loop, rayOrigin, rayDir, 0.001f, 10000.0f, h);
        bool do_restir = false, do_nee = false, do_bounce = false;
        f3 hit_normal = splat(0.0f), hit_albedo = splat(0.0f), hitPos = splat(0.0f), V_view = splat(0.0f);
        float roughness = 0.5f, metallic = 0.0f;
        if (in_loop) {
            if (reuse_primary) prd = load_payload(a.primary_payload + pix);
            else prd = shade_hit<(V & 2) != 0, (V & 4) != 0>(sc, h);
            if (prd.dist < 0.0f) in_loop = false;
            else {
                hit_normal = unpack_normal(prd.normal_packed);
                hit_albedo = unpack_unorm_rgb(prd.albedo_packed);
                hitPos = rayOrigin + rayDir * prd.dist;
                V_view = -rayDir;
                const f2 mat_info = unpack_half_2x16(prd.material_info);
                roughness = fmaxf(mat_info.x, 0.01f);
                metallic = clampf(mat_info.y, 0.0f, 1.0f);
                const f2 trans_ior = unpack_half_2x16(prd.transmission_ior_packed);
                const float transmission = trans_ior.x;
                const float ior = fmaxf(trans_ior.y, 1.0f);
                if (!prev_did_nee) radiance = radiance + prd.emission * throughput;
                prev_did_nee = false;
                const float brightness = maxc(prd.emission);
                if (brightness > 1.0f) in_loop = false;
                else if (transmission > 0.5f) {
                    const bool is_inside = dot3(rayDir, hit_normal) > 0.0f;
                    const f3 N = is_inside ? -hit_normal : hit_normal;
                    const float eta = is_inside ? (ior / 1.0f) : (1.0f / ior);
                    const float cos_theta = fminf(dot3(-rayDir, N), 1.0f);
                    float R0 = (1.0f - eta) / (1.0f + eta);
                    R0 = R0 * R0;
                    float fresnel = R0 + (1.0f - R0) * pow5f(1.0f - cos_theta);
                    const f3 refracted = refract3(rayDir, N, eta);
                    if (len3(refracted) < 0.01f) fresnel = 1.0f;
                    if (rnd(rng) < fresnel) rayDir = reflect3(rayDir, N);
                    else {
                        rayDir = refracted;
                        if (is_inside) {
                            const f3 absorption = 1.0f - hit_albedo;
                            const f3 e = -absorption * prd.dist * 5.0f;
                            throughput = throughput * mk3(exp_pinned(e.x), exp_pinned(e.y), exp_pinned(e.z));
                        } else throughput = throughput * hit_albedo;
                    }
                    rayOrigin = hitPos + rayDir * 0.001f;
                } else {
                    do_bounce = true;
                    if (num_lights > 0 && bounce < SHADOW_BOUNCES) {
                        if (!restir_evaluated && roughness > 0.2f) { restir_evaluated = true; do_restir = true; do_bounce = false; }
                        else if (restir_evaluated && roughness > 0.2f) do_nee = true;
                    }
                }
            }
        }

        if (__builtin_amdgcn_ballot_w64(do_restir) != 0ull) {
            SrReservoir spatial_r; zero_reservoir(spatial_r);
            f3 f_y_winner = splat(0.0f), shadow_dir = splat(0.0f);
            float shadow_dist = 0.0f;
            bool di_pending = false, want_di = false;
            if (do_restir) {
                SrReservoir center_r = load48(reservoir_cur + pix);
                if (center_r.W > 0.0f && center_r.light_idx < num_lights) {
                    center_r.light_idx = center_r.light_idx < num_lights - 1 ? center_r.light_idx : num_lights - 1;
                    const f3 fc = eval_unshadowed_light(hitPos, hit_normal, V_view, hit_albedo, roughness, metallic,
                                                        light_emission(sc, center_r.light_idx), ld3(center_r.light_pos), ld3(center_r.light_normal));
                    const float cr = rnd(rng);
                    merge_reservoirs(spatial_r, center_r, maxc(fc), cr);
                }
                const float current_depth = len3(hitPos - origin);
                for (int s = 0; s < 5; s++) {
                    const float angle = rnd(rng) * 2.0f * 3.14159f;
                    const float radius = sqrtf(rnd(rng)) * 30.0f;
                    float sa, ca; sincos_pinned(angle, sa, ca);
                    const int ncx = ipx + (int)(ca * radius), ncy = ipy + (int)(sa * radius);
                    if (ncx < 0 || ncy < 0 || ncx >= (int)W || ncy >= (int)H) continue;
                    const uint32_t pi_n = (uint32_t)ncy * W + (uint32_t)ncx;
                    const f3 neighbor_normal = load_normal(a, pi_n);
                    const float neighbor_depth = load_depth(a, pi_n);
                    if (dot3(hit_normal, neighbor_normal) < 0.9f) continue;
                    if (fabsf(current_depth - neighbor_depth) > 0.1f * current_depth) continue;
                    SrReservoir nr = load48(reservoir_cur + pi_n);
                    nr.W = fminf(nr.W, 20.0f);
                    nr.M = fminf(nr.M, 10.0f);
                    if (nr.W > 0.0f && nr.light_idx < num_lights) {
                        nr.light_idx = nr.light_idx < num_lights - 1 ? nr.light_idx : num_lights - 1;
                        const f3 fn = eval_unshadowed_light(hitPos, hit_normal, V_view, hit_albedo, roughness, metallic,
                                                            light_emission(sc, nr.light_idx), ld3(nr.light_pos), ld3(nr.light_normal));
                        const float nrnd = rnd(rng);
                        merge_reservoirs(spatial_r, nr, maxc(fn), nrnd);
                    }
                }
                if (spatial_r.w_sum > 0.0f) {
                    f_y_winner = eval_unshadowed_light(hitPos, hit_normal, V_view, hit_albedo, roughness, metallic,
                                                       light_emission(sc, spatial_r.light_idx), ld3(spatial_r.light_pos), ld3(spatial_r.light_normal));
                    spatial_r.W = spatial_r.w_sum / fmaxf(spatial_r.M * maxc(f_y_winner), 1e-3f);
                    spatial_r.W = fminf(spatial_r.W, 50.0f);
                    shadow_dir = ld3(spatial_r.light_pos) - hitPos;
                    shadow_dist = fmaxf(len3(shadow_dir), 0.0001f);
                    shadow_dir = shadow_dir / shadow_dist;
                    if (dot3(hit_normal, shadow_dir) > 0.0f) { di_pending = true; want_di = shadow_dist > 0.002f; }
                }
            }
            occ = ws_query<V, true>(cx, want_di, hitPos, shadow_dir, 0.001f, shadow_dist - 0.001f, h);
            if (di_pending) {
                prd.dist = want_di ? (occ ? 1.0f : -1.0f) : -1.0f;
                if (prd.dist < 0.0f) radiance = radiance + f_y_winner * throughput * spatial_r.W;
                prev_did_nee = true;
            }

            SrReservoirGI combined; zero_reservoir_gi(combined);
            float gi_current_depth = 0.0f;
            bool gi_sample_seen = false;
            if (do_restir) {
                combined = load48(reservoir_gi_cur + pix);
                gi_current_depth = len3(hitPos - origin);
            }
            for (int s = 0; s < 3; s++) {
                bool cand = false, want_g = false;
                uint32_t cand_pix = 0u;
                float jacobian = 0.0f, d_new = 0.0f;
                f3 gi_spatial_dir = splat(0.0f);
                if (do_restir) {
                    const float gi_angle = rnd(rng) * 2.0f * 3.14159f;
                    const float gi_radius = sqrtf(rnd(rng)) * 20.0f;
                    float sa, ca; sincos_pinned(gi_angle, sa, ca);
                    const int ncx = ipx + (int)(ca * gi_radius), ncy = ipy + (int)(sa * gi_radius);
                    bool ok = !(ncx == ipx && ncy == ipy);
                    ok = ok && !(ncx < 0 || ncy < 0 || ncx >= (int)W || ncy >= (int)H);
                    if (ok) {
                        const uint32_t pi_nn = (uint32_t)ncy * W + (uint32_t)ncx;
                        const f3 neighbor_normal = load_normal(a, pi_nn);
                        const float neighbor_depth = load_depth(a, pi_nn);
                        ok = !(dot3(hit_normal, neighbor_normal) < 0.9f);
                        ok = ok && !(fabsf(gi_current_depth - neighbor_depth) > 0.1f * gi_current_depth);
                        if (ok) {
                            SrReservoirGI nr = load48(reservoir_gi_cur + pi_nn);
                            ok = !(nr.W <= 0.0f);
                            if (ok) {
                                nr.W = fminf(nr.W, 10.0f);
                                nr.M = fminf(nr.M, 10.0f);
                                f3 n_origin, n_dir; f2 n_uv;
                                primary_ray(a.mats, (uint32_t)ncx, (uint32_t)ncy, W, H, n_origin, n_dir, n_uv);
                                const f3 neighbor_x1 = origin + n_dir * neighbor_depth;
                                const f3 nsp = ld3(nr.sample_pos);
                                const f3 w_new = nsp - hitPos;
                                const f3 w_old = nsp - neighbor_x1;
                                d_new = fmaxf(len3(w_new), 1e-4f);
                                const float d_old = fmaxf(len3(w_old), 1e-4f);
                                const f3 n_x2 = unpack_normal(nr.sample_normal_packed);
                                const float cos_new = fmaxf(dot3(n_x2, (-w_new) / d_new), 0.0f);
                                const float cos_old = fmaxf(dot3(n_x2, (-w_old) / d_old), 0.0f);
                                ok = !(cos_new <= 0.0f || cos_old <= 0.0f);
                                if (ok) {
                                    jacobian = (cos_new * d_old * d_old) / fmaxf(cos_old * d_new * d_new, 1e-4f);
                                    jacobian = clampf(jacobian, 0.0f, 10.0f);
                                    gi_spatial_dir = w_new / d_new;
                                    ok = !(dot3(hit_normal, gi_spatial_dir) <= 0.0f);
                                    if (ok) { cand = true; cand_pix = pi_nn; want_g = d_new > 0.002f; }
                                }
                            }
                        }
                    }
                }
                occ = ws_query<V, true>(cx, want_g, hitPos, gi_spatial_dir, 0.001f, d_new - 0.001f, h);
                if (cand) {
                    prd.dist = want_g ? (occ ? 1.0f : -1.0f) : -1.0f;
                    if (!(prd.dist >= 0.0f)) {
                        SrReservoirGI nr = load48(reservoir_gi_cur + cand_pix);
                        nr.W = fminf(nr.W, 10.0f);
                        nr.M = fminf(nr.M, 10.0f);
                        const float p_hat_neighbor = gi_target_pdf(hitPos, hit_normal, hit_albedo, metallic, ld3(nr.sample_pos), ld3(nr.sample_radiance));
                        const float gr = rnd(rng);
                        if (merge_reservoirs_gi(combined, nr, p_hat_neighbor, jacobian, gr)) gi_sample_seen = true;
                    }
                }
            }
            bool gif_pending = false, want_gif = false;
            f3 gi_x2_dir = splat(0.0f);
            float gi_x2_dist = 0.0f, gi_NdotL = 0.0f;
            if (do_restir) {
                const float p_hat_final = gi_target_pdf(hitPos, hit_normal, hit_albedo, metallic, ld3(combined.sample_pos), ld3(combined.sample_radiance));
                combined.W = (p_hat_final > 1e-3f) ? (combined.w_sum / fmaxf(combined.M, 1.0f) / p_hat_final) : 0.0f;
                combined.W = fminf(combined.W, 20.0f);
                if (combined.W > 0.0f) {
                    gi_x2_dir = ld3(combined.sample_pos) - hitPos;
                    gi_x2_dist = fmaxf(len3(gi_x2_dir), 0.0001f);
                    gi_x2_dir = gi_x2_dir / gi_x2_dist;
                    gi_NdotL = fmaxf(dot3(hit_normal, gi_x2_dir), 0.0f);
                    if (gi_NdotL > 0.0f) {
                        gif_pending = true; want_gif = gi_x2_dist > 0.002f;
                        if (gi_sample_seen && !(a.cfg.flags & SR_TRACE_FLAG_TRACE_EVERY_QUERY)) { if (want_gif) cx.n_q |= kCountReusedAny; want_gif = false; }
                    }
                }
            }
            occ = ws_query<V, true>(cx, want_gif, hitPos, gi_x2_dir, 0.001f, gi_x2_dist - 0.001f, h);
            if (gif_pending) {
                prd.dist = want_gif ? (occ ? 1.0f : -1.0f) : -1.0f;
                if (prd.dist < 0.0f) {
                    const f3 gi_f_diffuse = hit_albedo * (1.0f - metallic) / 3.14159f;
                    radiance = radiance + ld3(combined.sample_radiance) * gi_f_diffuse * gi_NdotL * combined.W * throughput;
                }
            }
            if (do_restir) in_loop = false;
        }

        if (__builtin_amdgcn_ballot_w64(do_nee) != 0ull) {
            bool nee_pending = false, want_nee = false;
            f3 shadow_ray_dir = splat(0.0f), nee_emission = splat(0.0f);
            float light_dist = 0.0f, cos_theta_light = 0.0f, cos_theta_surface = 0.0f, light_area = 0.0f;
            if (do_nee) {
                uint32_t light_idx = (uint32_t)(rnd(rng) * (float)num_lights);
                if (light_idx > num_lights - 1) light_idx = num_lights - 1;
                const LightTri lt = fetch_light(sc, light_idx);
                light_area = lt.area;
                nee_emission = lt.emission;
                const float r1_nee = rnd(rng);
                const float r2_nee = rnd(rng);
                const float sqr1 = sqrtf(r1_nee);
                const float u = 1.0f - sqr1;
                const float v = r2_nee * sqr1;
                const float w = 1.0f - u - v;
                const f3 light_pos = lt.wv0 * u + lt.wv1 * v + lt.wv2 * w;
                const f3 light_normal = lt.normal;
                shadow_ray_dir = light_pos - hitPos;
                light_dist = len3(shadow_ray_dir);
                shadow_ray_dir = shadow_ray_dir / light_dist;
                cos_theta_light = fmaxf(dot3(light_normal, -shadow_ray_dir), 0.0f);
                cos_theta_surface = fmaxf(dot3(hit_normal, shadow_ray_dir), 0.0f);
                if (cos_theta_light > 0.0f && cos_theta_surface > 0.0f) { nee_pending = true; want_nee = light_dist > 0.002f; }
            }
            occ = ws_query<V, true>(cx, want_nee, hitPos, shadow_ray_dir, 0.001f, light_dist - 0.001f, h);
            if (nee_pending) {
                prd.dist = want_nee ? (occ ? 1.0f : -1.0f) : -1.0f;
                if (prd.dist < 0.0f) {
                    const float solid_angle_pdf = (light_dist * light_dist) / fmaxf(cos_theta_light * light_area * (float)num_lights, 1e-4f);
                    const f3 nee_contrib = (nee_emission * hit_albedo * throughput * cos_theta_surface) / (solid_angle_pdf * 3.14159f);
                    radiance = radiance + vmin(nee_contrib, splat(5.0f));
                }
                prev_did_nee = true;
            }
        }

        if (in_loop && do_bounce) {
            const f3 N = hit_normal;
            const f3 F0 = lerp3(splat(0.04f), hit_albedo, metallic);
            const float cos_theta = fmaxf(dot3(N, V_view), 0.0f);
            const f3 F = F0 + (1.0f - F0) * pow5f(clampf(1.0f - cos_theta, 0.0f, 1.0f));
            const float p_specular = clampf(maxc(F), 0.05f, 1.0f);
            float r1, r2;
            if (bounce == 0) {
                const int bw = (int)a.blue_noise_w, bh = (int)a.blue_noise_h;
                const int n1x = ipx % bw, n1y = ipy % bh;
                const int n2x = (ipx + 47) % bw, n2y = (ipy + 71) % bh;
                const float bn_1 = (float)a.blue_noise_tex[((size_t)n1y * bw + n1x) * 4] / 255.0f;
                const float bn_2 = (float)a.blue_noise_tex[((size_t)n2y * bw + n2x) * 4] / 255.0f;
                r1 = fracf(bn_1 + (float)(a.frame_count % 1024u) * 0.75487766f);
                r2 = fracf(bn_2 + (float)(a.frame_count % 1024u) * 0.56984029f);
            } else {
                r1 = rnd(rng);
                r2 = rnd(rng);
            }
            if (rnd(rng) < p_specular) {
                const f3 Hh = sample_ggx_vndf(N, V_view, roughness, r1, r2);
                rayDir = reflect3(-V_view, Hh);
                if (dot3(N, rayDir) <= 0.0f) {
                    rayDir = get_random_bounce(N, r1, r2);
                    throughput = throughput * (hit_albedo * (1.0f - metallic) * (1.0f - F) / (1.0f - p_specular));
                } else {
                    const float NdotL_b = fmaxf(dot3(N, rayDir), 0.001f);
                    const float alpha_b = roughness * roughness;
                    const float G1_L = smith_g1_ggx(NdotL_b, alpha_b);
                    throughput = throughput * ((F * G1_L) / p_specular);
                }
            } else {
                rayDir = get_random_bounce(N, r1, r2);
                throughput = throughput * (hit_albedo * (1.0f - metallic) * (1.0f - F) / (1.0f - p_specular));
            }
            const float p = maxc(throughput);
            if (p < 0.001f) in_loop = false;
            else {
                bool cont = true;
                if (bounce > 2) {
                    if (rnd(rng) > p) cont = false;
                    else throughput = throughput / p;
                }
                if (cont) rayOrigin = hitPos + hit_normal * 0.001f;
                else in_loop = false;
            }
        }
    }
    if (active) {
        f3 total_radiance = splat(0.0f) + radiance;
        total_radiance = vmin(total_radiance, splat(10.0f));
        const f3 color = total_radiance / 1.0f;
        float4 o;
        o.x = color.x; o.y = color.y; o.z = color.z; o.w = 1.0f;
        reinterpret_cast<float4*>(a.raw_color)[pix] = o;
    }
    record_tile_cost(a, cost_slot, t_start);
    if (!(a.cfg.flags & SR_TRACE_FLAG_UNCOUNTED)) {
        const bool counted = (a.cfg.count_rows == 0u || (py - a.cfg.count_y0) < a.cfg.count_rows) &&
                             (a.cfg.count_cols == 0u || (px - a.cfg.count_x0) < a.cfg.count_cols);
        flush_counter(sc.counters, 0, counted ? counted_closest(cx.n_q) : 0u);
        flush_counter(sc.counters, 1, counted ? counted_any(cx.n_q) : 0u);
        flush_counter(sc.counters, 4, (counted && active && BOUNCES > 0 && a.primary_payload != nullptr) ? 1u : 0u);
        flush_counter(sc.counters, 5, counted ? cx.n_q >> 31 : 0u);
        if (V & 1) { flush_counter(sc.counters, 2, counted ? cx.st.boxes : 0u); flush_counter(sc.counters, 3, counted ? cx.st.tris : 0u); }
    }
}

}

using namespace srd;

int srk_launch_trace(const DevScene& sc, const SrRay* rays, uint32_t n, SrHit* hits, uint32_t* occluded,
                     int any, int stats, int two_level, int stack_entries, hipStream_t stream) {
    if (n == 0) return 0;
    dim3 grid((n + kBlock - 1) / kBlock), block(kBlock);
    const size_t lds = (size_t)(stack_entries + lds_extra_rows(two_level)) * kBlock * sizeof(int);
    const int v = (any ? 1 : 0) | (stats ? 2 : 0) | (two_level ? 4 : 0);
    switch (v) {
        case 0: trace_rays_kernel<false, false, false><<<grid, block, lds, stream>>>(sc, rays, n, hits, occluded); break;
        case 1: trace_rays_kernel<true, false, false><<<grid, block, lds, stream>>>(sc, rays, n, hits, occluded); break;
        case 2: trace_rays_kernel<false, true, false><<<grid, block, lds, stream>>>(sc, rays, n, hits, occluded); break;
        case 3: trace_rays_kernel<true, true, false><<<grid, block, lds, stream>>>(sc, rays, n, hits, occluded); break;
        case 4: trace_rays_kernel<false, false, true><<<grid, block, lds, stream>>>(sc, rays, n, hits, occluded); break;
        case 5: trace_rays_kernel<true, false, true><<<grid, block, lds, stream>>>(sc, rays, n, hits, occluded); break;
        case 6: trace_rays_kernel<false, true, true><<<grid, block, lds, stream>>>(sc, rays, n, hits, occluded); break;
        default: trace_rays_kernel<true, true, true><<<grid, block, lds, stream>>>(sc, rays, n, hits, occluded); break;
    }
    return (int)hipGetLastError();
}

int srk_launch_shade(const DevScene& sc, const SrHit* hits, uint32_t n, SrRayPayload* out, hipStream_t stream) {
    if (n == 0) return 0;
    shade_closest_hit_kernel<<<dim3((n + kBlock - 1) / kBlock), dim3(kBlock), 0, stream>>>(sc, hits, n, out);
    return (int)hipGetLastError();
}

int srk_launch_any_hit(const DevScene& sc, const SrHit* hits, uint32_t n, uint32_t* ignored, hipStream_t stream) {
    if (n == 0) return 0;
    any_hit_kernel<<<dim3((n + kBlock - 1) / kBlock), dim3(kBlock), 0, stream>>>(sc, hits, n, ignored);
    return (int)hipGetLastError();
}

int srk_launch_pass(const PassArgs& args_in, int which, int stats, int textured, int two_level, int stack_entries, hipStream_t stream) {
    PassArgs args = args_in;
    args.tiles_x = (args.x1 - args.x0 + kPassTile - 1) / kPassTile;
    args.tiles_y = (args.y1 - args.y0 + kPassTile - 1) / kPassTile;
    args.order_cap = srk_pass_order_cap(args.x1 - args.x0, args.y1 - args.y0);
    const uint32_t n_tiles = args.tiles_x * args.tiles_y;
    if (n_tiles == 0) return 0;
    dim3 grid(args.order_cap * 8), block(kPassBlock);
    const size_t lds = (size_t)(stack_entries + lds_extra_rows(two_level)) * kPassBlock * sizeof(int);
    const int v = (stats ? 1 : 0) | (textured ? 2 : 0) | (two_level ? 4 : 0);
    if (which == 0) {
        switch (v) {
            case 0: ris_kernel<0><<<grid, block, lds, stream>>>(args); break;
            case 1: ris_kernel<1><<<grid, block, lds, stream>>>(args); break;
            case 2: ris_kernel<2><<<grid, block, lds, stream>>>(args); break;
            case 3: ris_kernel<3><<<grid, block, lds, stream>>>(args); break;
            case 4: ris_kernel<4><<<grid, block, lds, stream>>>(args); break;
            case 5: ris_kernel<5><<<grid, block, lds, stream>>>(args); break;
            case 6: ris_kernel<6><<<grid, block, lds, stream>>>(args); break;
            default: ris_kernel<7><<<grid, block, lds, stream>>>(args); break;
        }
    } else {
        switch (v) {
            case 0: final_kernel<0><<<grid, block, lds, stream>>>(args); break;
            case 1: final_kernel<1><<<grid, block, lds, stream>>>(args); break;
            case 2: final_kernel<2><<<grid, block, lds, stream>>>(args); break;
            case 3: final_kernel<3><<<grid, block, lds, stream>>>(args); break;
            case 4: final_kernel<4><<<grid, block, lds, stream>>>(args); break;
            case 5: final_kernel<5><<<grid, block, lds, stream>>>(args); break;
            case 6: final_kernel<6><<<grid, block, lds, stream>>>(args); break;
            default: final_kernel<7><<<grid, block, lds, stream>>>(args); break;
        }
    }
    return (int)hipGetLastError();
}

int srk_lds_rows(int stack_entries, int two_level) { return stack_entries + lds_extra_rows(two_level); }

uint32_t srk_pass_tile_count(uint32_t width, uint32_t rows) { return ((width + kPassTile - 1) / kPassTile) * ((rows + kPassTile - 1) / kPassTile); }

uint32_t srk_pass_order_cap(uint32_t width, uint32_t rows) {
    const uint32_t tiles_x = (width + kPassTile - 1) / kPassTile, tiles_y = (rows + kPassTile - 1) / kPassTile;
    const uint32_t cap_cols = std::max(std::min(tiles_x, (tiles_x * 3u) / 16u + 2u), (tiles_x + 7u) / 8u);
    return cap_cols * tiles_y;
}

int srk_launch_tile_order(const uint32_t* tile_cost, uint32_t* tile_order, uint32_t width, uint32_t rows, hipStream_t stream) {
    const uint32_t tiles_x = (width + kPassTile - 1) / kPassTile, tiles_y = (rows + kPassTile - 1) / kPassTile;
    if (tiles_x * tiles_y == 0) return 0;
    tile_order_kernel<<<dim3(8), dim3(256), 0, stream>>>(tile_cost, tile_order, tiles_x, tiles_y, srk_pass_order_cap(width, rows));
    return (int)hipGetLastError();
}
```

### sunray_amd/csrc/rt_device.h

```cpp
#pragma once
#include <hip/hip_runtime.h>
#include <hip/hip_fp16.h>
#include <stdint.h>

#include "../../include/sunray_hip.h"

namespace srd {

struct f3 { float x, y, z; };
struct f2 { float x, y; };

#define SRD __device__ __forceinline__

SRD f3 mk3(float x, float y, float z) { f3 r; r.x = x; r.y = y; r.z = z; return r; }
SRD f3 splat(float s) { return mk3(s, s, s); }
SRD f3 ld3(const float* p) { return mk3(p[0], p[1], p[2]); }
SRD void st3(float* p, f3 v) { p[0] = v.x; p[1] = v.y; p[2] = v.z; }
SRD f3 operator+(f3 a, f3 b) { return mk3(a.x + b.x, a.y + b.y, a.z + b.z); }
SRD f3 operator-(f3 a, f3 b) { return mk3(a.x - b.x, a.y - b.y, a.z - b.z); }
SRD f3 operator*(f3 a, f3 b) { return mk3(a.x * b.x, a.y * b.y, a.z * b.z); }
SRD f3 operator*(f3 a, float s) { return mk3(a.x * s, a.y * s, a.z * s); }
SRD f3 operator*(float s, f3 a) { return mk3(s * a.x, s * a.y, s * a.z); }
SRD f3 operator-(f3 a) { return mk3(-a.x, -a.y, -a.z); }
SRD f3 operator-(float s, f3 a) { return mk3(s - a.x, s - a.y, s - a.z); }
SRD f3 operator/(f3 a, float s) { float r = 1.0f / s; return mk3(a.x * r, a.y * r, a.z * r); }

SRD float dot3(f3 a, f3 b) { return (a.x * b.x + a.y * b.y) + a.z * b.z; }
SRD f3 cross3(f3 a, f3 b) { return mk3(a.y * b.z - a.z * b.y, a.z * b.x - a.x * b.z, a.x * b.y - a.y * b.x); }
SRD float len3(f3 a) { return sqrtf(dot3(a, a)); }
SRD f3 norm3(f3 a) { float r = 1.0f / sqrtf(dot3(a, a)); return a * r; }
SRD float clampf(float x, float lo, float hi) { return fminf(fmaxf(x, lo), hi); }
SRD f3 vmin(f3 a, f3 b) { return mk3(fminf(a.x, b.x), fminf(a.y, b.y), fminf(a.z, b.z)); }
SRD float maxc(f3 a) { return fmaxf(a.x, fmaxf(a.y, a.z)); }
SRD f3 lerp3(f3 a, f3 b, float t) { return a + (b - a) * t; }
SRD float fracf(float x) { return x - floorf(x); }
SRD float smoothstepf(float a, float b, float x) {
    float t = clampf((x - a) / (b - a), 0.0f, 1.0f);
    return t * t * (3.0f - 2.0f * t);
}
SRD f3 reflect3(f3 i, f3 n) { return i - (2.0f * dot3(n, i)) * n; }
SRD f3 refract3(f3 i, f3 n, float eta) {
    float ni = dot3(n, i);
    float k = 1.0f - eta * eta * (1.0f - ni * ni);
    if (k < 0.0f) return splat(0.0f);
    return eta * i - (eta * ni + sqrtf(k)) * n;
}
SRD float pow5f(float x) { float x2 = x * x; float x4 = x2 * x2; return x4 * x; }

SRD void sincos_pinned(float x, float& s, float& c) {
    float kf = rintf(x * 0.63661977236758134f);
    int k = (int)kf;
    float r = fmaf(-kf, 1.5703125f, x);
    r = fmaf(-kf, 4.837512969970703125e-4f, r);
    r = fmaf(-kf, 7.54978995489188216e-8f, r);
    float z = r * r;
    float ps = fmaf(fmaf(-1.9515295891e-4f, z, 8.3321608736e-3f), z, -1.6666654611e-1f);
    float sr = fmaf(r * z, ps, r);
    float pc = fmaf(fmaf(2.443315711809948e-5f, z, -1.388731625493765e-3f), z, 4.166664568298827e-2f);
    float cr = fmaf(z * z, pc, fmaf(-0.5f, z, 1.0f));
    int q = k & 3;
    float s0 = (q & 1) ? cr : sr;
    float c0 = (q & 1) ? sr : cr;
    s = (q & 2) ? -s0 : s0;
    c = ((q == 1) || (q == 2)) ? -c0 : c0;
}
SRD float exp_pinned(float x) {
    if (!(x == x)) return x;
    if (x > 88.72283935546875f) return __builtin_inff();
    if (x < -103.9720840454f) return 0.0f;
    float kf = rintf(x * 1.44269504088896341f);
    float r = fmaf(-kf, 0.693359375f, x);
    r = fmaf(-kf, -2.12194440e-4f, r);
    float z = r * r;
    float p = fmaf(1.9875691500e-4f, r, 1.3981999507e-3f);
    p = fmaf(p, r, 8.3334519073e-3f);
    p = fmaf(p, r, 4.1665795894e-2f);
    p = fmaf(p, r, 1.6666665459e-1f);
    p = fmaf(p, r, 5.0000001201e-1f);
    float y = fmaf(p, z, r) + 1.0f;
    int k = (int)kf;
    int k1 = k / 2, k2 = k - k1;
    return ldexpf(ldexpf(y, k1), k2);
}

SRD float log_pinned(float x) {
    if (!(x == x)) return x;
    if (x < 0.0f) return __builtin_nanf("");
    if (x == 0.0f) return -__builtin_inff();
    if (x == __builtin_inff()) return x;
    int e = 0;
    if (x < 1.17549435e-38f) { x = x * 33554432.0f; e = -25; }
    const uint32_t u = __float_as_uint(x);
    e += (int)(u >> 23) - 126;
    float m = __uint_as_float((u & 0x007fffffu) | 0x3f000000u);
    if (m < 0.707106781186547524f) { e -= 1; m = m + m - 1.0f; }
    else m = m - 1.0f;
    const float z = m * m;
    float y = fmaf(7.0376836292e-2f, m, -1.1514610310e-1f);
    y = fmaf(y, m, 1.1676998740e-1f);
    y = fmaf(y, m, -1.2420140846e-1f);
    y = fmaf(y, m, 1.4249322787e-1f);
    y = fmaf(y, m, -1.6668057665e-1f);
    y = fmaf(y, m, 2.0000714765e-1f);
    y = fmaf(y, m, -2.4999993993e-1f);
    y = fmaf(y, m, 3.3333331174e-1f);
    y = y * m * z;
    const float fe = (float)e;
    y = fmaf(-2.12194440e-4f, fe, y);
    y = fmaf(-0.5f, z, y);
    float r = m + y;
    r = fmaf(0.693359375f, fe, r);
    return r;
}

SRD float pow_pinned(float x, float y) { return exp_pinned(y * log_pinned(x)); }

SRD uint32_t f32_to_f16_bits(float f) { return (uint32_t)__half_as_ushort(__float2half_rn(f)); }
SRD float f16_bits_to_f32(uint32_t h) { return __half2float(__ushort_as_half((unsigned short)(h & 0xFFFFu))); }

SRD uint32_t pcg_hash(uint32_t x) {
    x ^= x >> 16; x *= 0x7feb352du; x ^= x >> 15; x *= 0x846ca68bu; x ^= x >> 16;
    return x;
}
SRD uint32_t init_rng(uint32_t px, uint32_t py, uint32_t frame, uint32_t launch_w) {
    return pcg_hash((py * launch_w + px) ^ pcg_hash(frame));
}
SRD float rnd(uint32_t& seed) {
    seed = seed * 747796405u + 2891336453u;
    uint32_t word = ((seed >> ((seed >> 28u) + 4u)) ^ seed) * 277803737u;
    uint32_t result = (word >> 22u) ^ word;
    return (float)result * 2.3283064365386963e-10f;
}

SRD uint32_t pack_snorm_2x16(float x, float y) {
    int ix = (int)rintf(clampf(x, -1.0f, 1.0f) * 32767.0f);
    int iy = (int)rintf(clampf(y, -1.0f, 1.0f) * 32767.0f);
    return ((uint32_t)ix & 0xFFFFu) | (((uint32_t)iy & 0xFFFFu) << 16);
}
SRD f2 unpack_snorm_2x16(uint32_t p) {
    int x = (int)(p << 16) >> 16;
    int y = (int)p >> 16;
    f2 r;
    r.x = clampf((float)x / 32767.0f, -1.0f, 1.0f);
    r.y = clampf((float)y / 32767.0f, -1.0f, 1.0f);
    return r;
}
SRD uint32_t pack_unorm_4x8(float x, float y, float z, float w) {
    uint32_t cx = (uint32_t)rintf(clampf(x, 0.0f, 1.0f) * 255.0f);
    uint32_t cy = (uint32_t)rintf(clampf(y, 0.0f, 1.0f) * 255.0f);
    uint32_t cz = (uint32_t)rintf(clampf(z, 0.0f, 1.0f) * 255.0f);
    uint32_t cw = (uint32_t)rintf(clampf(w, 0.0f, 1.0f) * 255.0f);
    return cx | (cy << 8) | (cz << 16) | (cw << 24);
}
SRD f3 unpack_unorm_rgb(uint32_t p) {
    return mk3((float)(p & 0xFFu) / 255.0f, (float)((p >> 8) & 0xFFu) / 255.0f, (float)((p >> 16) & 0xFFu) / 255.0f);
}
SRD uint32_t pack_half_2x16(float x, float y) { return f32_to_f16_bits(x) | (f32_to_f16_bits(y) << 16); }
SRD f2 unpack_half_2x16(uint32_t p) { f2 r; r.x = f16_bits_to_f32(p & 0xFFFFu); r.y = f16_bits_to_f32(p >> 16); return r; }

SRD uint32_t pack_normal(f3 n) {
    n = n / (fabsf(n.x) + fabsf(n.y) + fabsf(n.z));
    float px, py;
    if (n.z >= 0.0f) { px = n.x; py = n.y; }
    else {
        px = (1.0f - fabsf(n.y)) * (n.x >= 0.0f ? 1.0f : -1.0f);
        py = (1.0f - fabsf(n.x)) * (n.y >= 0.0f ? 1.0f : -1.0f);
    }
    return pack_snorm_2x16(px, py);
}
SRD f3 unpack_normal(uint32_t p) {
    f2 v = unpack_snorm_2x16(p);
    f3 n = mk3(v.x, v.y, 1.0f - fabsf(v.x) - fabsf(v.y));
    float t = fmaxf(-n.z, 0.0f);
    n.x += (n.x >= 0.0f) ? -t : t;
    n.y += (n.y >= 0.0f) ? -t : t;
    return norm3(n);
}

SRD uint32_t snorm8(float x) {
    if (!(x == x)) return 0u;
    int i = (int)rintf(clampf(x, -1.0f, 1.0f) * 127.0f);
    return (uint32_t)i & 0xFFu;
}
SRD uint32_t pack_rgba8_snorm(float x, float y, float z, float w) {
    return snorm8(x) | (snorm8(y) << 8) | (snorm8(z) << 16) | (snorm8(w) << 24);
}
SRD float unsnorm8(uint32_t b) { int i = (int)(int8_t)(b & 0xFFu); return fmaxf((float)i / 127.0f, -1.0f); }
template <int MANT>
SRD uint32_t to_ufloat(float f) {
    uint32_t u = __float_as_uint(f);
    const uint32_t max_finite = (30u << MANT) | ((1u << MANT) - 1u);
    if ((u & 0x7fffffffu) > 0x7f800000u) return (31u << MANT) | 1u;
    if (u & 0x80000000u) return 0u;
    if (u == 0x7f800000u) return 31u << MANT;
    if (u >= 0x47800000u) return max_finite;
    uint32_t r;
    if (u >= 0x38800000u) {
        uint32_t t = u - 0x38000000u;
        const uint32_t sh = 23u - MANT;
        t = t + ((1u << (sh - 1u)) - 1u) + ((t >> sh) & 1u);
        r = t >> sh;
    } else {
        if (u < 0x30000000u) return 0u;
        uint32_t e = u >> 23;
        uint32_t m = (u & 0x7fffffu) | 0x800000u;
        uint32_t s = 136u - MANT - e;
        if (s > 31u) return 0u;
        r = m >> s;
        uint32_t lower = m & ((1u << s) - 1u);
        uint32_t half = 1u << (s - 1u);
        if (lower > half || (lower == half && (r & 1u))) r++;
    }
    return r > max_finite ? max_finite : r;
}
SRD uint32_t pack_b10g11r11(float r, float g, float b) {
    return to_ufloat<6>(r) | (to_ufloat<6>(g) << 11) | (to_ufloat<5>(b) << 22);
}

template <int MANT>
SRD float from_ufloat(uint32_t v) {
    const uint32_t e = v >> MANT, m = v & ((1u << MANT) - 1u);
    if (e == 0u) return (float)m * __uint_as_float((uint32_t)(127 - 14 - MANT) << 23);
    if (e == 31u) return __uint_as_float(0x7f800000u | (m << (23 - MANT)));
    return __uint_as_float(((e + 112u) << 23) | (m << (23 - MANT)));
}
SRD f3 unpack_b10g11r11(uint32_t v) { return mk3(from_ufloat<6>(v & 0x7ffu), from_ufloat<6>((v >> 11) & 0x7ffu), from_ufloat<5>(v >> 22)); }

SRD void build_onb(f3 n, f3& t, f3& b) {
    float sign_n = n.z >= 0.0f ? 1.0f : -1.0f;
    float a = -1.0f / (sign_n + n.z);
    float bb = n.x * n.y * a;
    t = mk3(1.0f + sign_n * n.x * n.x * a, sign_n * bb, -sign_n * n.x);
    b = mk3(bb, sign_n + n.y * n.y * a, -n.y);
}
SRD float smith_v_ggx(float NdotV, float NdotL, float alpha) {
    float a2 = alpha * alpha;
    float ggxV = NdotL * sqrtf(NdotV * NdotV * (1.0f - a2) + a2);
    float ggxL = NdotV * sqrtf(NdotL * NdotL * (1.0f - a2) + a2);
    return 0.5f / fmaxf(ggxV + ggxL, 0.0001f);
}
SRD float smith_g1_ggx(float NdotX, float alpha) {
    float a2 = alpha * alpha;
    float denom = NdotX + sqrtf(a2 + (1.0f - a2) * NdotX * NdotX);
    return 2.0f * NdotX / fmaxf(denom, 0.0001f);
}
SRD f3 get_random_bounce(f3 normal, float r1, float r2) {
    float phi = 2.0f * 3.14159f * r1;
    float r = sqrtf(r2);
    f3 u, v;
    build_onb(normal, u, v);
    float s, c;
    sincos_pinned(phi, s, c);
    return norm3(u * c * r + v * s * r + normal * sqrtf(1.0f - r2));
}
SRD f3 sample_ggx_vndf(f3 normal, f3 V_world, float roughness, float r1, float r2) {
    f3 T, B;
    build_onb(normal, T, B);
    f3 Vl = mk3(dot3(V_world, T), dot3(V_world, B), dot3(V_world, normal));
    float a = fmaxf(roughness * roughness, 0.001f);
    f3 Vh = norm3(mk3(a * Vl.x, a * Vl.y, Vl.z));
    float lensq = Vh.x * Vh.x + Vh.y * Vh.y;
    f3 T1 = lensq > 0.0f ? mk3(-Vh.y, Vh.x, 0.0f) * (1.0f / sqrtf(lensq)) : mk3(1.0f, 0.0f, 0.0f);
    f3 T2 = cross3(Vh, T1);
    float rr = sqrtf(r1);
    float phi = 2.0f * 3.14159265f * r2;
    float sp, cp;
    sincos_pinned(phi, sp, cp);
    float t1 = rr * cp;
    float t2 = rr * sp;
    float s = 0.5f * (1.0f + Vh.z);
    t2 = (1.0f - s) * sqrtf(1.0f - t1 * t1) + s * t2;
    f3 Nh = t1 * T1 + t2 * T2 + sqrtf(fmaxf(0.0f, 1.0f - t1 * t1 - t2 * t2)) * Vh;
    f3 Hl = norm3(mk3(a * Nh.x, a * Nh.y, fmaxf(0.0f, Nh.z)));
    return T * Hl.x + B * Hl.y + normal * Hl.z;
}
SRD f3 eval_unshadowed_light(f3 hit_pos, f3 hit_normal, f3 V_view, f3 hit_albedo, float roughness, float metallic,
                             f3 emission, f3 light_pos, f3 light_normal) {
    f3 L = light_pos - hit_pos;
    float dist = fmaxf(len3(L), 0.0001f);
    L = L / dist;
    float NdotL = fmaxf(dot3(hit_normal, L), 0.0f);
    float cos_light = fmaxf(dot3(light_normal, -L), 0.0f);
    if (NdotL <= 0.0f || cos_light <= 0.0f) return splat(0.0f);
    f3 H = norm3(V_view + L);
    float NdotH = fmaxf(dot3(hit_normal, H), 0.0f);
    float VdotH = fmaxf(dot3(V_view, H), 0.0f);
    float NdotV = fmaxf(dot3(hit_normal, V_view), 0.001f);
    float a = roughness * roughness;
    float a2 = a * a;
    float denom = (NdotH * NdotH * (a2 - 1.0f) + 1.0f);
    float D = a2 / (3.14159f * denom * denom);
    f3 F0 = lerp3(splat(0.04f), hit_albedo, metallic);
    f3 F = F0 + (1.0f - F0) * pow5f(1.0f - VdotH);
    float V_term = smith_v_ggx(NdotV, NdotL, a);
    f3 specular_brdf = (D * V_term) * F;
    f3 diffuse_brdf = hit_albedo * (1.0f - metallic) * (splat(1.0f) - F) / 3.14159f;
    float geometry = (NdotL * cos_light) / fmaxf(dist * dist, 0.0001f);
    return emission * (diffuse_brdf + specular_brdf) * geometry;
}
SRD float gi_target_pdf(f3 shade_pos, f3 shade_normal, f3 albedo, float metallic, f3 sample_pos, f3 sample_radiance) {
    f3 w = sample_pos - shade_pos;
    float d = fmaxf(len3(w), 0.0001f);
    w = w / d;
    float NdotL = fmaxf(dot3(shade_normal, w), 0.0f);
    f3 f_diffuse = albedo * (1.0f - metallic) / 3.14159f;
    f3 contrib = sample_radiance * f_diffuse * NdotL;
    return maxc(contrib);
}
SRD void merge_reservoirs(SrReservoir& r, const SrReservoir& nr, float p_hat_new, float random_val) {
    r.M += nr.M;
    float weight = p_hat_new * nr.W * nr.M;
    r.w_sum += weight;
    if (random_val < (weight / fmaxf(r.w_sum, 0.0001f))) {
        r.light_idx = nr.light_idx;
        r.light_pos[0] = nr.light_pos[0]; r.light_pos[1] = nr.light_pos[1]; r.light_pos[2] = nr.light_pos[2];
        r.light_normal[0] = nr.light_normal[0]; r.light_normal[1] = nr.light_normal[1]; r.light_normal[2] = nr.light_normal[2];
    }
}
SRD bool merge_reservoirs_gi(SrReservoirGI& r, const SrReservoirGI& nr, float p_hat_new, float jacobian, float random_val) {
    r.M += nr.M;
    float weight = p_hat_new * nr.W * nr.M * jacobian;
    r.w_sum += weight;
    const bool taken = random_val < (weight / fmaxf(r.w_sum, 0.0001f));
    if (taken) {
        r.sample_pos[0] = nr.sample_pos[0]; r.sample_pos[1] = nr.sample_pos[1]; r.sample_pos[2] = nr.sample_pos[2];
        r.sample_radiance[0] = nr.sample_radiance[0]; r.sample_radiance[1] = nr.sample_radiance[1]; r.sample_radiance[2] = nr.sample_radiance[2];
        r.sample_normal_packed = nr.sample_normal_packed;
    }
    return taken;
}
SRD f3 transform_point(const float* m, f3 p) {
    return mk3(((m[0] * p.x + m[1] * p.y) + m[2] * p.z) + m[3] * 1.0f,
               ((m[4] * p.x + m[5] * p.y) + m[6] * p.z) + m[7] * 1.0f,
               ((m[8] * p.x + m[9] * p.y) + m[10] * p.z) + m[11] * 1.0f);
}

}
```

### sunray_amd/csrc/traverse.h

```cpp
#pragma once
#include "bvh_layout.h"
#include "rt_device.h"

namespace srd {

constexpr int kStackMax = 31;
constexpr int kMaxBinaryDepth = 31;
constexpr int kSentinel = 0x7fffffff;

struct DevInstance {
    float w2o[12];
    float o2w[12];
};
struct DevMeshConst {
    float emission[3];
    uint32_t albedo_packed;
    uint32_t material_info;
    uint32_t transmission_ior_packed;
    uint32_t textured;
    uint32_t _pad;
};
struct DevMeshTex {
    float base_color[4];
    float emissive_factor[3], emissive_strength;
    float roughness, metallic;
    uint32_t img_base, img_mr;
    uint32_t img_normal, img_emissive;
    uint32_t samplers;
    uint32_t alpha_mode;
    float alpha_cutoff;
    uint32_t _pad;
};
struct DevTexture {
    const uint32_t* texels;
    uint32_t w, h;
};

struct DevLight {
    float wv0[3], area;
    float wv1[3], nx;
    float wv2[3], ny;
    float emission[3], nz;
};

constexpr uint32_t kCounterSlots = 256, kCounterStride = 8;

struct DevScene {
    const float4* nodes;
    const float4* tris;
    const float4* shade;
    const float4* shade_tex;
    const DevMeshConst* mesh_const;
    const DevMeshTex* mesh_tex;
    const DevTexture* textures;
    const DevInstance* instances;
    const DevLight* lights;
    const uint32_t* slot_of_gid;
    const float4* blas_nodes;
    const uint32_t* tl_inst;
    const struct DevTlInstance* tl_instances;
    unsigned long long* counters;
    uint32_t num_lights;
    uint32_t n_tris;
    uint32_t n_instances;
    uint32_t _pad;
};

struct TravHit {
    float t, u, v;
    uint32_t gid, slot;
    uint32_t inst;
};

struct DevTlInstance {
    float w2o[12];
    float o2w[12];
    uint32_t blas_root;
    uint32_t tri_offset;
    float pad_a, pad_b;
    uint32_t mesh_slot;
    uint32_t prim_base;
    uint32_t flags;
    uint32_t _pad;
};

struct TravStats { uint32_t boxes, tris; };

constexpr float kBaryEps = 1e-6f;
SRD float dot_fma(f3 a, f3 b) { return fmaf(a.z, b.z, fmaf(a.y, b.y, a.x * b.x)); }
SRD f3 cross_fma(f3 a, f3 b) {
    return mk3(fmaf(a.y, b.z, -(a.z * b.y)), fmaf(a.z, b.x, -(a.x * b.z)), fmaf(a.x, b.y, -(a.y * b.x)));
}
SRD bool intersect_tri(f3 o, f3 d, f3 v0, f3 e1, f3 e2, float tmin, float tmax, float& t, float& u, float& v) {
    f3 pvec = cross_fma(d, e2);
    float det = dot_fma(e1, pvec);
    float inv = 1.0f / det;
    f3 tvec = o - v0;
    u = dot_fma(tvec, pvec) * inv;
    f3 qvec = cross_fma(tvec, e1);
    v = dot_fma(d, qvec) * inv;
    t = dot_fma(e2, qvec) * inv;
    return (u >= -kBaryEps) && (v >= -kBaryEps) && (u + v <= 1.0f + kBaryEps) && (t > tmin) && (t < tmax);
}

struct RaySetup {
    f3 inv;
};
SRD float box_dir(float d) { return fabsf(d) >= 7.888609e-31f ? d : copysignf(7.888609e-31f, d); }
SRD RaySetup ray_setup(f3 o, f3 d) {
    RaySetup r;
    r.inv = mk3(1.0f / box_dir(d.x), 1.0f / box_dir(d.y), 1.0f / box_dir(d.z));
    return r;
}
template <int C>
SRD float plane_q(uint32_t packed) { return (float)((packed >> (8 * C)) & 0xFFu); }
struct NodePlanes {
    uint32_t nx, ny, nz, fx, fy, fz;
    float ax, ay, az;
    float bx, by, bz;
};
template <int C>
SRD bool child_hit(const NodePlanes& p, float t_lo, float t_hi, float& tnear) {
    const float t0 = fmaxf(fmaxf(fmaf(plane_q<C>(p.nx), p.ax, p.bx), fmaf(plane_q<C>(p.ny), p.ay, p.by)),
                           fmaxf(fmaf(plane_q<C>(p.nz), p.az, p.bz), t_lo));
    float far = fminf(fminf(fmaf(plane_q<C>(p.fx), p.ax, p.bx), fmaf(plane_q<C>(p.fy), p.ay, p.by)), fmaf(plane_q<C>(p.fz), p.az, p.bz));
    far = fmaf(fabsf(far), 5e-7f, far);
    tnear = t0;
    return t0 <= fminf(far, t_hi);
}

SRD int pick(int4 c, uint32_t i) {
    const int lo = (i & 1u) ? c.y : c.x;
    const int hi = (i & 1u) ? c.w : c.z;
    return (i & 2u) ? hi : lo;
}

constexpr int kWsRows = 7, kWsRowsTl = 8;
constexpr int kEarlyTriWalking = 16, kEarlyTriBlocked = 16;
SRD uint32_t ord_f32(float f) { const uint32_t b = __float_as_uint(f + 0.0f); return b ^ ((b >> 31) ? 0xFFFFFFFFu : 0x80000000u); }
SRD float unord_f32(uint32_t k) { return __uint_as_float(k ^ ((k >> 31) ? 0x80000000u : 0xFFFFFFFFu)); }
SRD uint32_t lanes_below(unsigned long long m) { return __builtin_amdgcn_mbcnt_hi((uint32_t)(m >> 32), __builtin_amdgcn_mbcnt_lo((uint32_t)m, 0u)); }
struct NodePlanesTl {
    uint32_t nx, ny, nz, fx, fy, fz;
    float ax, ay, az;
    float bnx, bny, bnz, bfx, bfy, bfz;
};
template <int C>
SRD bool child_hit_tl(const NodePlanesTl& p, float t_lo, float t_hi, float& tnear) {
    const float t0 = fmaxf(fmaxf(fmaf(plane_q<C>(p.nx), p.ax, p.bnx), fmaf(plane_q<C>(p.ny), p.ay, p.bny)),
                           fmaxf(fmaf(plane_q<C>(p.nz), p.az, p.bnz), t_lo));
    float far = fminf(fminf(fmaf(plane_q<C>(p.fx), p.ax, p.bfx), fmaf(plane_q<C>(p.fy), p.ay, p.bfy)), fmaf(plane_q<C>(p.fz), p.az, p.bfz));
    far = fmaf(fabsf(far), 5e-7f, far);
    tnear = t0;
    return t0 <= fminf(far, t_hi);
}

template <bool ANY, bool STATS, bool TL = false>
SRD bool traverse_ws(const DevScene& sc, bool want, f3 o, f3 d, float tmin, float tmax, TravHit& hit, int* lds_col, int stride, TravStats& st) {
    const float4* __restrict__ nodes = sc.nodes;
    const float4* __restrict__ tris = sc.tris;
    const uint32_t tid = threadIdx.x, lane = tid & 63u;
    int* const blk = lds_col - tid;
    unsigned long long* const keys = reinterpret_cast<unsigned long long*>(blk);
    int* const xch = blk + 2 * stride + (tid & ~63u);
    int* const pay = blk + 3 * stride;
    int* const stack_base = lds_col + (TL ? kWsRowsTl : kWsRows) * stride;
    keys[tid] = ~0ull;
    uint32_t root = tid;
    RaySetup rs = ray_setup(o, d);
    float t_lo = fminf(tmin, 0.0f) - fabsf(tmin);
    float cull = fmaf(fabsf(tmax), 1e-5f, tmax);
    float best_t = tmax;
    uint32_t best_gid = 0xFFFFFFFFu;
    int sp = 0, sb = 0, leaf = 0;
    int node = want ? 0 : kSentinel;
    bool in_blas = false;
    int lsp = 0;
    uint32_t inst = 0u, leaf_inst = 0u;
    f3 ro = o;
    f3 winv = rs.inv;
    f3 pad = splat(0.0f);
    auto leave = [&]() { in_blas = false; ro = o; rs.inv = winv; pad = splat(0.0f); };
    auto pop = [&]() -> int {
        if (TL) { if (in_blas && sp == lsp) leave(); }
        return sp == sb ? kSentinel : stack_base[(--sp) * stride];
    };
    for (;;) {
        if (node != kSentinel) {
            const unsigned long long k = keys[root];
            if (ANY) { if (k == 0ull) { node = kSentinel; sp = sb; if (TL) { in_blas = false; } } }
            else if (k != ~0ull) { const float ts = unord_f32((uint32_t)(k >> 32)); cull = fminf(cull, fmaf(fabsf(ts), 1e-5f, ts)); }
        }
        if (__builtin_amdgcn_ballot_w64(node != kSentinel || (TL && leaf != 0)) == 0ull) break;
        for (;;) {
            const bool inner = node != kSentinel && (node >= 0 || (TL && !in_blas));
            {
                const unsigned long long walking = __builtin_amdgcn_ballot_w64(inner && leaf == 0);
                if (walking == 0ull) break;
                if ((int)__popcll(walking) <= kEarlyTriWalking &&
                    (int)__popcll(__builtin_amdgcn_ballot_w64(node != kSentinel && node < 0 && leaf != 0 && (!TL || in_blas))) >= kEarlyTriBlocked) break;
            }
            const bool idle = node == kSentinel && leaf == 0;
            const unsigned long long idle_mask = __builtin_amdgcn_ballot_w64(idle);
            if (idle_mask != 0ull) {
                const bool can_give = node != kSentinel && sp > sb;
                const unsigned long long donor_mask = __builtin_amdgcn_ballot_w64(can_give);
                if (donor_mask != 0ull) {
                    const uint32_t n = min((uint32_t)__popcll(idle_mask), (uint32_t)__popcll(donor_mask));
                    const uint32_t drank = lanes_below(donor_mask), irank = lanes_below(idle_mask);
                    const bool gives = can_give && drank < n, takes = idle && irank < n;
                    if (gives) xch[drank] = (int)lane;
                    __builtin_amdgcn_fence(__ATOMIC_SEQ_CST, "wavefront");
                    const int dl = takes ? xch[irank] : (int)lane;
                    const int d_sb = __shfl(sb, dl);
                    const uint32_t d_root = (uint32_t)__shfl((int)root, dl);
                    const float ox = __shfl(o.x, dl), oy = __shfl(o.y, dl), oz = __shfl(o.z, dl);
                    const float dx = __shfl(d.x, dl), dy = __shfl(d.y, dl), dz = __shfl(d.z, dl);
                    const float d_tmin = __shfl(tmin, dl), d_tmax = __shfl(tmax, dl), d_cull = __shfl(cull, dl);
                    const float ix = __shfl(rs.inv.x, dl), iy = __shfl(rs.inv.y, dl), iz = __shfl(rs.inv.z, dl);
                    bool d_blas = false;
                    uint32_t d_inst = 0u;
                    f3 d_ro = splat(0.0f), d_pad = splat(0.0f), d_winv = splat(0.0f);
                    if (TL) {
                        d_blas = __shfl((int)(in_blas && sb == lsp), dl) != 0;
                        d_inst = (uint32_t)__shfl((int)inst, dl);
                        d_ro = mk3(__shfl(ro.x, dl), __shfl(ro.y, dl), __shfl(ro.z, dl));
                        d_pad = mk3(__shfl(pad.x, dl), __shfl(pad.y, dl), __shfl(pad.z, dl));
                        d_winv = mk3(__shfl(winv.x, dl), __shfl(winv.y, dl), __shfl(winv.z, dl));
                    }
                    if (takes) {
                        node = stack_base[d_sb * stride + (dl - (int)lane)];
                        o = mk3(ox, oy, oz); d = mk3(dx, dy, dz); tmin = d_tmin; tmax = d_tmax; cull = d_cull; root = d_root;
                        rs.inv = mk3(ix, iy, iz);
                        t_lo = fminf(tmin, 0.0f) - fabsf(tmin);
                        best_t = tmax; best_gid = 0xFFFFFFFFu;
                        sp = 0; sb = 0;
                        if (TL) {
                            winv = d_winv; lsp = 0;
                            in_blas = d_blas; inst = d_inst; leaf_inst = d_inst;
                            if (d_blas) { ro = d_ro; pad = d_pad; }
                            else { ro = o; rs.inv = d_winv; pad = splat(0.0f); }
                        }
                        if (node < 0 && (!TL || in_blas)) { leaf = node; node = kSentinel; }
                    }
                    __builtin_amdgcn_fence(__ATOMIC_SEQ_CST, "wavefront");
                    if (gives) { if (TL) { if (in_blas && sb == lsp) lsp++; } sb++; }
                }
            }
            if (TL && node != kSentinel && node < 0 && !in_blas) {
                const uint32_t lv = ~(uint32_t)node;
                const uint32_t first = lv >> 3, cnt = lv & 7u;
                if (cnt == 0u) node = pop();
                else {
                    for (uint32_t k = 1; k < cnt; k++) { stack_base[sp * stride] = (int)~(((first + k) << 3) | 1u); sp++; }
                    inst = sc.tl_inst[first];
                    const float4* q = reinterpret_cast<const float4*>(sc.tl_instances + inst);
                    const float4 r0 = q[0], r1 = q[1], r2 = q[2], m6 = q[6];
                    if ((__float_as_uint(q[7].z) & 1u) == 0u) {
                        ro = mk3(((r0.x * o.x + r0.y * o.y) + r0.z * o.z) + r0.w, ((r1.x * o.x + r1.y * o.y) + r1.z * o.z) + r1.w,
                                 ((r2.x * o.x + r2.y * o.y) + r2.z * o.z) + r2.w);
                        const f3 rd = mk3((r0.x * d.x + r0.y * d.y) + r0.z * d.z, (r1.x * d.x + r1.y * d.y) + r1.z * d.z, (r2.x * d.x + r2.y * d.y) + r2.z * d.z);
                        rs = ray_setup(ro, rd);
                        const float pd = fmaf(m6.z, fmaxf(fmaxf(fabsf(o.x), fabsf(o.y)), fabsf(o.z)), m6.w);
                        pad = mk3(pd * fabsf(rs.inv.x), pd * fabsf(rs.inv.y), pd * fabsf(rs.inv.z));
                    }
                    lsp = sp;
                    in_blas = true;
                    node = (int)__float_as_uint(m6.x);
                }
            } else if (node >= 0 && node != kSentinel) {
                const float4* n = ((TL && in_blas) ? sc.blas_nodes : nodes) + (size_t)node * 4;
                const float4 h0 = n[0], q1 = n[1], q2 = n[2], qc = n[3];
                const int4 child = make_int4(__float_as_int(qc.x), __float_as_int(qc.y), __float_as_int(qc.z), __float_as_int(qc.w));
                if (STATS) st.boxes += 4;
                const uint32_t ex = __float_as_uint(h0.w);
                const uint32_t LX = __float_as_uint(q1.x), LY = __float_as_uint(q1.y), LZ = __float_as_uint(q1.z);
                const uint32_t HX = __float_as_uint(q1.w), HY = __float_as_uint(q2.x), HZ = __float_as_uint(q2.y);
                const bool sgx = __float_as_int(rs.inv.x) < 0, sgy = __float_as_int(rs.inv.y) < 0, sgz = __float_as_int(rs.inv.z) < 0;
                float n0, n1, n2, n3;
                bool b0, b1, b2, b3;
                if (TL) {
                    NodePlanesTl p;
                    p.nx = sgx ? HX : LX; p.fx = sgx ? LX : HX;
                    p.ny = sgy ? HY : LY; p.fy = sgy ? LY : HY;
                    p.nz = sgz ? HZ : LZ; p.fz = sgz ? LZ : HZ;
                    p.ax = __uint_as_float((ex & 0xFFu) << 23) * rs.inv.x; p.ay = __uint_as_float(((ex >> 8) & 0xFFu) << 23) * rs.inv.y;
                    p.az = __uint_as_float(((ex >> 16) & 0xFFu) << 23) * rs.inv.z;
                    const float bx = (h0.x - ro.x) * rs.inv.x, by = (h0.y - ro.y) * rs.inv.y, bz = (h0.z - ro.z) * rs.inv.z;
                    p.bnx = bx - pad.x; p.bfx = bx + pad.x; p.bny = by - pad.y; p.bfy = by + pad.y; p.bnz = bz - pad.z; p.bfz = bz + pad.z;
                    b0 = child_hit_tl<0>(p, t_lo, cull, n0) && child.x != -1;
                    b1 = child_hit_tl<1>(p, t_lo, cull, n1) && child.y != -1;
                    b2 = child_hit_tl<2>(p, t_lo, cull, n2) && child.z != -1;
                    b3 = child_hit_tl<3>(p, t_lo, cull, n3) && child.w != -1;
                } else {
                    NodePlanes p;
                    p.nx = sgx ? HX : LX; p.fx = sgx ? LX : HX;
                    p.ny = sgy ? HY : LY; p.fy = sgy ? LY : HY;
                    p.nz = sgz ? HZ : LZ; p.fz = sgz ? LZ : HZ;
                    p.ax = __uint_as_float((ex & 0xFFu) << 23) * rs.inv.x; p.ay = __uint_as_float(((ex >> 8) & 0xFFu) << 23) * rs.inv.y;
                    p.az = __uint_as_float(((ex >> 16) & 0xFFu) << 23) * rs.inv.z;
                    p.bx = (h0.x - o.x) * rs.inv.x; p.by = (h0.y - o.y) * rs.inv.y; p.bz = (h0.z - o.z) * rs.inv.z;
                    b0 = child_hit<0>(p, t_lo, cull, n0);
                    b1 = child_hit<1>(p, t_lo, cull, n1);
                    b2 = child_hit<2>(p, t_lo, cull, n2);
                    b3 = child_hit<3>(p, t_lo, cull, n3);
                }
                uint32_t k0, k1, k2, k3;
                if (ANY) {
                    k0 = b0 ? ((~__float_as_uint(n0) & 0x7FFFFFFCu) | 0u) : 0xFFFFFFFFu;
                    k1 = b1 ? ((~__float_as_uint(n1) & 0x7FFFFFFCu) | 1u) : 0xFFFFFFFFu;
                    k2 = b2 ? ((~__float_as_uint(n2) & 0x7FFFFFFCu) | 2u) : 0xFFFFFFFFu;
                    k3 = b3 ? ((~__float_as_uint(n3) & 0x7FFFFFFCu) | 3u) : 0xFFFFFFFFu;
                } else {
                    k0 = b0 ? ((__float_as_uint(fmaxf(n0, 0.0f)) & ~3u) | 0u) : 0xFFFFFFFFu;
                    k1 = b1 ? ((__float_as_uint(fmaxf(n1, 0.0f)) & ~3u) | 1u) : 0xFFFFFFFFu;
                    k2 = b2 ? ((__float_as_uint(fmaxf(n2, 0.0f)) & ~3u) | 2u) : 0xFFFFFFFFu;
                    k3 = b3 ? ((__float_as_uint(fmaxf(n3, 0.0f)) & ~3u) | 3u) : 0xFFFFFFFFu;
                }
                const uint32_t kmin = min(min(k0, k1), min(k2, k3));
                const uint32_t slot = kmin & 3u;
                stack_base[sp * stride] = child.x; sp += (b0 && k0 != kmin) ? 1 : 0;
                stack_base[sp * stride] = child.y; sp += (b1 && k1 != kmin) ? 1 : 0;
                stack_base[sp * stride] = child.z; sp += (b2 && k2 != kmin) ? 1 : 0;
                stack_base[sp * stride] = child.w; sp += (b3 && k3 != kmin) ? 1 : 0;
                node = (kmin != 0xFFFFFFFFu) ? pick(child, slot) : pop();
                if (node < 0 && node != kSentinel && leaf == 0 && (!TL || in_blas)) { leaf = node; leaf_inst = inst; node = pop(); }
            }
        }
        while (leaf != 0) {
            const uint32_t lv = ~(uint32_t)leaf;
            const uint32_t slot = lv >> 3, cnt = lv & 7u;
            const bool two = cnt >= 2u;
            leaf = cnt > 2u ? (int)~(((slot + 2u) << 3) | (cnt - 2u)) : 0;
            const uint32_t cur_inst = leaf_inst;
            if (leaf == 0 && node < 0 && (!TL || in_blas)) { leaf = node; leaf_inst = inst; node = pop(); }
            if (cnt == 0u) continue;
            const uint32_t slot_b = two ? slot + 1u : slot;
            const float4 t0 = tris[(size_t)slot * 3 + 0], t1 = tris[(size_t)slot * 3 + 1], t2 = tris[(size_t)slot * 3 + 2];
            const float4 s0 = tris[(size_t)slot_b * 3 + 0], s1 = tris[(size_t)slot_b * 3 + 1], s2 = tris[(size_t)slot_b * 3 + 2];
            float ta, ua, va, tb, ub, vb;
            if (STATS) st.tris += two ? 2u : 1u;
            bool hit_a, hit_b;
            uint32_t gid_a, gid_b;
            if (TL) {
                const float4* q = reinterpret_cast<const float4*>(sc.tl_instances + cur_inst);
                const float4 m0 = q[3], m1 = q[4], m2 = q[5];
                const bool baked = (__float_as_uint(q[7].z) & 1u) != 0u;
                auto to_world = [&](f3 p) {
                    return baked ? p : mk3(((m0.x * p.x + m0.y * p.y) + m0.z * p.z) + m0.w * 1.0f, ((m1.x * p.x + m1.y * p.y) + m1.z * p.z) + m1.w * 1.0f,
                                           ((m2.x * p.x + m2.y * p.y) + m2.z * p.z) + m2.w * 1.0f);
                };
                const f3 wa = to_world(mk3(t0.x, t0.y, t0.z)), wb = to_world(mk3(t0.w, t1.x, t1.y)), wc = to_world(mk3(t1.z, t1.w, t2.x));
                hit_a = intersect_tri(o, d, wa, wb - wa, wc - wa, tmin, tmax, ta, ua, va);
                const f3 xa = to_world(mk3(s0.x, s0.y, s0.z)), xb = to_world(mk3(s0.w, s1.x, s1.y)), xc = to_world(mk3(s1.z, s1.w, s2.x));
                hit_b = intersect_tri(o, d, xa, xb - xa, xc - xa, tmin, tmax, tb, ub, vb) && two;
                const uint32_t off = sc.tl_instances[cur_inst].tri_offset;
                gid_a = off + __float_as_uint(t2.y); gid_b = off + __float_as_uint(s2.y);
            } else {
                hit_a = intersect_tri(o, d, mk3(t0.x, t0.y, t0.z), mk3(t0.w, t1.x, t1.y), mk3(t1.z, t1.w, t2.x), tmin, tmax, ta, ua, va);
                hit_b = intersect_tri(o, d, mk3(s0.x, s0.y, s0.z), mk3(s0.w, s1.x, s1.y), mk3(s1.z, s1.w, s2.x), tmin, tmax, tb, ub, vb) && two;
                gid_a = __float_as_uint(t2.y); gid_b = __float_as_uint(s2.y);
            }
            if (hit_a || hit_b) {
                if (ANY) { keys[root] = 0ull; node = kSentinel; sp = sb; leaf = 0; if (TL) { in_blas = false; } break; }
                const bool take_b = hit_b && (!hit_a || tb < ta || (tb == ta && gid_b < gid_a));
                const float t = take_b ? tb : ta, u = take_b ? ub : ua, v = take_b ? vb : va;
                const uint32_t gid = take_b ? gid_b : gid_a, hit_slot = take_b ? slot_b : slot;
                if (t < best_t || (t == best_t && gid < best_gid)) {
                    best_t = t; best_gid = gid;
                    cull = fminf(cull, fmaf(fabsf(t), 1e-5f, t));
                    const unsigned long long key = ((unsigned long long)ord_f32(t) << 32) | gid;
                    atomicMin(&keys[root], key);
                    if (keys[root] == key) {
                        pay[0 * stride + root] = __float_as_int(t); pay[1 * stride + root] = __float_as_int(u);
                        pay[2 * stride + root] = __float_as_int(v); pay[3 * stride + root] = (int)hit_slot;
                        if (TL) pay[4 * stride + root] = (int)cur_inst;
                    }
                }
            }
        }
    }
    __builtin_amdgcn_fence(__ATOMIC_SEQ_CST, "wavefront");
    const unsigned long long k = keys[tid];
    hit.t = -1.0f; hit.u = 0.0f; hit.v = 0.0f; hit.gid = 0xFFFFFFFFu; hit.slot = 0u; hit.inst = 0u;
    if (ANY) return k == 0ull;
    if (k != ~0ull) {
        hit.gid = (uint32_t)k;
        hit.t = __int_as_float(pay[0 * stride + tid]); hit.u = __int_as_float(pay[1 * stride + tid]);
        hit.v = __int_as_float(pay[2 * stride + tid]); hit.slot = (uint32_t)pay[3 * stride + tid];
        if (TL) hit.inst = (uint32_t)pay[4 * stride + tid];
    }
    return k != ~0ull;
}

SRD void tl_locate(const DevScene& sc, uint32_t gid, uint32_t& slot, uint32_t& inst) {
    uint32_t lo = 0u, hi = sc.n_instances;
    while (hi - lo > 1u) { const uint32_t mid = (lo + hi) >> 1; if (sc.tl_instances[mid].tri_offset <= gid) lo = mid; else hi = mid; }
    inst = lo;
    slot = sc.slot_of_gid[sc.tl_instances[lo].prim_base + (gid - sc.tl_instances[lo].tri_offset)];
}

struct Payload {
    f3 emission;
    float dist;
    uint32_t albedo_packed, normal_packed, material_info, transmission_ior_packed;
};

SRD float wrap_coord(float s, uint32_t mode) {
    if (!(fabsf(s) < 3.0e38f)) s = 0.0f;
    if (mode == 0u) return s - floorf(s);
    if (mode == 1u) return s - 2.0f * floorf(s * 0.5f);
    return fminf(fmaxf(s, -1.0f), 2.0f);
}
SRD uint32_t wrap_index(int i, int n, uint32_t mode) {
    if (mode == 0u) { int m = i % n; return (uint32_t)(m < 0 ? m + n : m); }
    if (mode == 1u) {
        int m = i % (2 * n);
        if (m < 0) m += 2 * n;
        return (uint32_t)(m < n ? m : 2 * n - 1 - m);
    }
    return (uint32_t)(i < 0 ? 0 : (i > n - 1 ? n - 1 : i));
}
SRD float4 texel_unorm(uint32_t p) {
    return make_float4((float)(p & 0xFFu) / 255.0f, (float)((p >> 8) & 0xFFu) / 255.0f, (float)((p >> 16) & 0xFFu) / 255.0f,
                       (float)(p >> 24) / 255.0f);
}
SRD float4 sample_texture(const DevScene& sc, uint32_t image_slot, uint32_t sampler_code, float s, float t, float4 fallback) {
    if (image_slot == 0xFFFFFFFFu) return fallback;
    const DevTexture tx = sc.textures[image_slot];
    const uint32_t mode_u = (sampler_code >> 1) & 3u, mode_v = (sampler_code >> 3) & 3u;
    const int W = (int)tx.w, H = (int)tx.h;
    float u = wrap_coord(s, mode_u) * (float)W;
    float v = wrap_coord(t, mode_v) * (float)H;
    if ((sampler_code & 1u) == 0u) {
        const uint32_t i = wrap_index((int)floorf(u), W, mode_u), j = wrap_index((int)floorf(v), H, mode_v);
        return texel_unorm(tx.texels[(size_t)j * tx.w + i]);
    }
    u = u - 0.5f; v = v - 0.5f;
    const float fu = floorf(u), fv = floorf(v);
    const float a = u - fu, b = v - fv;
    const uint32_t i0 = wrap_index((int)fu, W, mode_u), i1 = wrap_index((int)fu + 1, W, mode_u);
    const uint32_t j0 = wrap_index((int)fv, H, mode_v), j1 = wrap_index((int)fv + 1, H, mode_v);
    const float4 t00 = texel_unorm(tx.texels[(size_t)j0 * tx.w + i0]), t10 = texel_unorm(tx.texels[(size_t)j0 * tx.w + i1]);
    const float4 t01 = texel_unorm(tx.texels[(size_t)j1 * tx.w + i0]), t11 = texel_unorm(tx.texels[(size_t)j1 * tx.w + i1]);
    const float na = 1.0f - a, nb = 1.0f - b;
    return make_float4((t00.x * na + t10.x * a) * nb + (t01.x * na + t11.x * a) * b, (t00.y * na + t10.y * a) * nb + (t01.y * na + t11.y * a) * b,
                       (t00.z * na + t10.z * a) * nb + (t01.z * na + t11.z * a) * b, (t00.w * na + t10.w * a) * nb + (t01.w * na + t11.w * a) * b);
}

SRD void shade_textured(const DevScene& sc, uint32_t slot, uint32_t inst, uint32_t mesh, f3 bary, f3 world_normal, Payload& pl) {
    const float4* q = sc.shade_tex + (size_t)slot * 6;
    const float4 q0 = q[0], q1 = q[1], q2 = q[2];
    const DevMeshTex mt = sc.mesh_tex[mesh];
    const float uv_s = (q0.x * bary.x + q0.z * bary.y) + q1.x * bary.z;
    const float uv_t = (q0.y * bary.x + q0.w * bary.y) + q1.y * bary.z;
    const float4 base_color = sample_texture(sc, mt.img_base, mt.samplers & 0xFFu, uv_s, uv_t,
                                             make_float4(mt.base_color[0], mt.base_color[1], mt.base_color[2], mt.base_color[3]));
    const float4 emissive = sample_texture(sc, mt.img_emissive, mt.samplers >> 24, uv_s, uv_t,
                                           make_float4(mt.emissive_factor[0], mt.emissive_factor[1], mt.emissive_factor[2], 1.0f));
    pl.emission = mk3(emissive.x, emissive.y, emissive.z) * mt.emissive_strength;
    pl.albedo_packed = pack_unorm_4x8(base_color.x, base_color.y, base_color.z, 1.0f);
    if (mt.img_normal != 0xFFFFFFFFu) {
        const float4 q3 = q[3], q4 = q[4], q5 = q[5];
        const f3 ta = mk3(q3.x, q3.y, q3.z), tb = mk3(q4.x, q4.y, q4.z), tc = mk3(q4.w, q5.x, q5.y);
        const f3 tangent_dir = ta * bary.x + tb * bary.y + tc * bary.z;
        if (len3(tangent_dir) > 0.001f) {
            const float handedness = q3.w;
            const float nuv_s = (q1.z * bary.x + q2.x * bary.y) + q2.z * bary.z;
            const float nuv_t = (q1.w * bary.x + q2.y * bary.y) + q2.w * bary.z;
            const float* M = sc.instances[inst].o2w;
            f3 wt = norm3(mk3((M[0] * tangent_dir.x + M[1] * tangent_dir.y) + M[2] * tangent_dir.z,
                              (M[3] * tangent_dir.x + M[4] * tangent_dir.y) + M[5] * tangent_dir.z,
                              (M[6] * tangent_dir.x + M[7] * tangent_dir.y) + M[8] * tangent_dir.z));
            wt = norm3(wt - world_normal * dot3(wt, world_normal));
            const f3 wb = cross3(world_normal, wt) * handedness;
            const float4 raw = sample_texture(sc, mt.img_normal, (mt.samplers >> 16) & 0xFFu, nuv_s, nuv_t, make_float4(0.5f, 0.5f, 1.0f, 1.0f));
            f3 sn = mk3(raw.x * 2.0f - 1.0f, raw.y * 2.0f - 1.0f, raw.z * 2.0f - 1.0f);
            sn.z = sqrtf(fminf(fmaxf(1.0f - (sn.x * sn.x + sn.y * sn.y), 0.0f), 1.0f));
            sn = norm3(sn);
            pl.normal_packed = pack_normal(norm3(mk3((sn.x * wt.x + sn.y * wb.x) + sn.z * world_normal.x,
                                                     (sn.x * wt.y + sn.y * wb.y) + sn.z * world_normal.y,
                                                     (sn.x * wt.z + sn.y * wb.z) + sn.z * world_normal.z)));
        }
    }
    float roughness = mt.roughness, metallic = mt.metallic;
    if (mt.img_mr != 0xFFFFFFFFu) {
        const float4 mr = sample_texture(sc, mt.img_mr, (mt.samplers >> 8) & 0xFFu, uv_s, uv_t, make_float4(1.0f, 1.0f, 1.0f, 1.0f));
        roughness = roughness * mr.y;
        metallic = metallic * mr.z;
    }
    pl.material_info = pack_half_2x16(roughness, metallic);
}

SRD bool any_hit_ignores(const DevScene& sc, uint32_t slot, float u, float v) {
    const float4 s2 = sc.shade[(size_t)slot * 3 + 2];
    const uint32_t mesh = __float_as_uint(s2.z);
    const DevMeshTex mt = sc.mesh_tex[mesh];
    if (mt.alpha_mode == 0u) return false;
    float4 base_color = make_float4(mt.base_color[0], mt.base_color[1], mt.base_color[2], mt.base_color[3]);
    if (mt.img_base != 0xFFFFFFFFu) {
        const f3 bary = mk3(1.0f - u - v, u, v);
        const float4* q = sc.shade_tex + (size_t)slot * 6;
        const float4 q0 = q[0], q1 = q[1];
        const float uv_s = (q0.x * bary.x + q0.z * bary.y) + q1.x * bary.z;
        const float uv_t = (q0.y * bary.x + q0.w * bary.y) + q1.y * bary.z;
        base_color = sample_texture(sc, mt.img_base, mt.samplers & 0xFFu, uv_s, uv_t, base_color);
    }
    return base_color.w < mt.alpha_cutoff;
}

template <bool TEX, bool TL = false>
SRD Payload shade_hit(const DevScene& sc, const TravHit& h) {
    Payload pl;
    pl.emission = splat(0.0f);
    pl.albedo_packed = 0; pl.normal_packed = 0; pl.material_info = 0; pl.transmission_ior_packed = 0;
    if (h.gid == 0xFFFFFFFFu) { pl.dist = -1.0f; return pl; }
    const float4 s0 = sc.shade[(size_t)h.slot * 3 + 0];
    const float4 s1 = sc.shade[(size_t)h.slot * 3 + 1];
    const float4 s2 = sc.shade[(size_t)h.slot * 3 + 2];
    const uint32_t inst = TL ? h.inst : __float_as_uint(s2.y), mesh = __float_as_uint(s2.z);
    const f3 bary = mk3(1.0f - h.u - h.v, h.u, h.v);
    const f3 na = mk3(s0.x, s0.y, s0.z), nb = mk3(s0.w, s1.x, s1.y), nc = mk3(s1.z, s1.w, s2.x);
    const f3 normal = na * bary.x + nb * bary.y + nc * bary.z;
    const float* W = sc.instances[inst].w2o;
    const f3 world_normal = norm3(mk3((normal.x * W[0] + normal.y * W[3]) + normal.z * W[6],
                                      (normal.x * W[1] + normal.y * W[4]) + normal.z * W[7],
                                      (normal.x * W[2] + normal.y * W[5]) + normal.z * W[8]));
    const DevMeshConst mc = sc.mesh_const[mesh];
    pl.dist = h.t;
    pl.emission = mk3(mc.emission[0], mc.emission[1], mc.emission[2]);
    pl.albedo_packed = mc.albedo_packed;
    pl.normal_packed = pack_normal(world_normal);
    pl.material_info = mc.material_info;
    pl.transmission_ior_packed = mc.transmission_ior_packed;
    if (TEX) { if (mc.textured) shade_textured(sc, h.slot, inst, mesh, bary, world_normal, pl); }
    return pl;
}

}
```

### sunray_amd/runtime.py

```python
import ctypes as C

import numpy as np

from . import abi
from ._lib import SunrayError, check, lib


def _p(a):
    return a.ctypes.data_as(C.c_void_p)


def _f3(v):
    return (C.c_float * 3)(*[float(x) for x in v])


def _device_vertices(tensor, device_index):
    if not getattr(tensor, "is_cuda", False):
        raise ValueError("update_mesh_device: the vertices must be a tensor on the scene's GPU, not host memory")
    if tensor.device.index != device_index:
        raise ValueError("update_mesh_device: the tensor is on %s, the scene on cuda:%d" % (tensor.device, device_index))
    if not tensor.is_contiguous():
        raise ValueError("update_mesh_device: the tensor must be contiguous")
    nbytes = tensor.numel() * tensor.element_size()
    if nbytes == 0 or nbytes % abi.VERTEX.itemsize:
        raise ValueError("update_mesh_device: %d bytes are not a whole number of %d-byte vertices" % (nbytes, abi.VERTEX.itemsize))
    return C.c_void_p(tensor.data_ptr()), nbytes // abi.VERTEX.itemsize


def _skin_influences(influences):
    if not isinstance(influences, np.ndarray) or influences.dtype != abi.SKIN_INFLUENCE:
        raise ValueError("set_mesh_skin: the influences must be a numpy array of abi.SKIN_INFLUENCE records")
    if influences.ndim != 1 or len(influences) == 0:
        raise ValueError("set_mesh_skin: the influences must be one record per vertex, in one dimension (shape %s given)" % (influences.shape,))
    return np.ascontiguousarray(influences)


def _joint_matrices(matrices):
    if not isinstance(matrices, np.ndarray) or matrices.dtype not in (np.dtype(np.float32), abi.TRANSFORM):
        raise ValueError("skin_mesh: the joint matrices must be a numpy float32 array (or abi.TRANSFORM records)")
    if matrices.dtype == abi.TRANSFORM:
        ok = matrices.ndim == 1
    else:
        ok = (matrices.ndim == 2 and matrices.shape[1] == 12) or (matrices.ndim == 3 and matrices.shape[1:] == (3, 4))
    if not ok or len(matrices) == 0:
        raise ValueError("skin_mesh: the joint matrices must be (n_joints, 12) or (n_joints, 3, 4), row-major 3x4 (shape %s given)" % (matrices.shape,))
    return np.ascontiguousarray(matrices), len(matrices)


def camera_matrices(pos, target, fov_y, width, height, prev_view_proj=None):
    m = abi.SrMatrices()
    prev = None
    if prev_view_proj is not None:
        prev = (C.c_float * 16)(*[float(x) for x in prev_view_proj])
    check(lib().sr_camera_matrices(_f3(pos), _f3(target), C.c_float(fov_y), C.c_uint32(width), C.c_uint32(height), prev, C.byref(m)))
    return m


def material_new(base_color, metallic, roughness, emissive_factor, emissive_strength, transmission, ior):
    m = np.zeros((), dtype=abi.MATERIAL)
    check(lib().sr_material_new((C.c_float * 4)(*base_color), C.c_float(metallic), C.c_float(roughness), _f3(emissive_factor),
                                C.c_float(emissive_strength), C.c_float(transmission), C.c_float(ior), _p(m)))
    return m


def decode_image(data):
    buf = (C.c_uint8 * len(data)).from_buffer_copy(bytes(data))
    w, h, c = C.c_uint32(), C.c_uint32(), C.c_uint32()
    check(lib().sr_decode_image(buf, C.c_size_t(len(data)), C.byref(w), C.byref(h), C.byref(c), None, C.c_size_t(0)))
    out = np.zeros((h.value, w.value, c.value), dtype=np.uint8)
    check(lib().sr_decode_image(buf, C.c_size_t(len(data)), C.byref(w), C.byref(h), C.byref(c), _p(out), C.c_size_t(out.size)))
    return out


def decode_image_rgba8(data):
    buf = (C.c_uint8 * len(data)).from_buffer_copy(bytes(data))
    w, h = C.c_uint32(), C.c_uint32()
    check(lib().sr_decode_image_rgba8(buf, C.c_size_t(len(data)), C.byref(w), C.byref(h), None, C.c_size_t(0)))
    out = np.zeros((h.value, w.value, 4), dtype=np.uint8)
    check(lib().sr_decode_image_rgba8(buf, C.c_size_t(len(data)), C.byref(w), C.byref(h), _p(out), C.c_size_t(out.size)))
    return out


def emissive_triangles_from_mesh(vertices, indices, material):
    v = np.ascontiguousarray(vertices, dtype=abi.VERTEX)
    i = np.ascontiguousarray(indices, dtype=np.uint32)
    m = np.ascontiguousarray(material, dtype=abi.MATERIAL)
    out = np.zeros(max(len(i) // 3, 1), dtype=abi.EMISSIVE_TRIANGLE)
    n = C.c_uint32()
    check(lib().sr_emissive_triangles_from_mesh(_p(v), C.c_uint32(len(v)), _p(i), C.c_uint32(len(i)), _p(m), _p(out), C.c_uint32(len(out)), C.byref(n)))
    return out[: n.value].copy()


def bvh_layout():
    w, nd, po, co = (C.c_uint32() for _ in range(4))
    check(lib().sr_bvh_layout(C.byref(w), C.byref(nd), C.byref(po), C.byref(co)))
    return w.value, nd.value, po.value, co.value


def host_bvh(v0_e1_e2):
    v = np.ascontiguousarray(v0_e1_e2, dtype=np.float32).reshape(-1, 9)
    h = C.c_void_p()
    check(lib().sr_host_bvh_build(_p(v), C.c_uint32(len(v)), C.byref(h)))
    try:
        np_, tp = C.POINTER(C.c_uint32)(), C.POINTER(C.c_float)()
        nn, nt, md, ms = C.c_uint32(), C.c_uint32(), C.c_uint32(), C.c_uint32()
        check(lib().sr_host_bvh_get(h, C.byref(np_), C.byref(nn), C.byref(tp), C.byref(nt), C.byref(md), C.byref(ms)))
        nodes = np.ctypeslib.as_array(np_, shape=(nn.value, bvh_layout()[1])).copy()
        tris = np.ctypeslib.as_array(tp, shape=(nt.value, 12)).copy() if nt.value else np.zeros((0, 12), np.float32)
    finally:
        lib().sr_host_bvh_destroy(h)
    return nodes, tris, md.value, ms.value


def decode_node(node):
    W, _, po, co = bvh_layout()
    n = np.asarray(node, dtype=np.uint32)
    origin = n[0:3].view(np.float32)
    ex = int(n[3])
    scale = np.array([np.uint32(((ex >> (8 * a)) & 0xFF) << 23) for a in range(3)], dtype=np.uint32).view(np.float32)
    pd = W // 4
    lo = np.zeros((W, 3), np.float32)
    hi = np.zeros((W, 3), np.float32)
    for c in range(W):
        for a in range(3):
            ql = np.float32((int(n[po + a * pd + c // 4]) >> (8 * (c % 4))) & 0xFF)
            qh = np.float32((int(n[po + (3 + a) * pd + c // 4]) >> (8 * (c % 4))) & 0xFF)
            lo[c, a] = np.float32(np.float64(ql) * np.float64(scale[a]) + np.float64(origin[a]))
            hi[c, a] = np.float32(np.float64(qh) * np.float64(scale[a]) + np.float64(origin[a]))
    return lo, hi, n[co:co + W].view(np.int32)


class DeviceFrame:

    def __init__(self, width, height, blue_noise, device="cuda:0", primary=None):
        import os
        import torch
        self.width, self.height = width, height
        n = width * height
        self.device = torch.device(device)
        z = lambda *shape, dtype: torch.zeros(*shape, dtype=dtype, device=self.device)
        self.raw_color = z(n, 4, dtype=torch.float32)
        self.depth = z(n, dtype=torch.int16)
        self.normal = z(n, dtype=torch.int32)
        self.diffuse = z(n, dtype=torch.int32)
        self.motion = z(n, dtype=torch.int32)
        self.reservoirs = [z(n, 12, dtype=torch.int32), z(n, 12, dtype=torch.int32)]
        self.reservoirs_gi = [z(n, 12, dtype=torch.int32), z(n, 12, dtype=torch.int32)]
        self.accum = [z(n, dtype=torch.int32), z(n, dtype=torch.int32)]
        self.denoise = [z(n, dtype=torch.int32), z(n, dtype=torch.int32)]
        self.output = z(n, dtype=torch.int32)
        if primary is None:
            primary = os.environ.get("SUNRAY_PRIMARY_REUSE", "1") != "0"
        self.primary = z(n, 8, dtype=torch.int32) if primary else None
        bn = np.ascontiguousarray(blue_noise, dtype=np.uint8)
        self.blue_noise_shape = bn.shape[:2]
        self.blue_noise = torch.from_numpy(bn.copy()).to(self.device)

    def host(self):
        out = {
            "raw_color": self.raw_color.cpu().numpy(),
            "depth": self.depth.cpu().numpy().view(np.uint16),
            "normal": self.normal.cpu().numpy().view(np.uint32),
            "diffuse": self.diffuse.cpu().numpy().view(np.uint32),
            "motion": self.motion.cpu().numpy().view(np.uint32),
            "reservoirs": [r.cpu().numpy().view(np.uint32).reshape(-1).view(abi.RESERVOIR) for r in self.reservoirs],
            "reservoirs_gi": [r.cpu().numpy().view(np.uint32).reshape(-1).view(abi.RESERVOIR_GI) for r in self.reservoirs_gi],
            "accum": [a.cpu().numpy().view(np.uint32) for a in self.accum],
            "denoise": [a.cpu().numpy().view(np.uint32) for a in self.denoise],
            "output": self.output.cpu().numpy().view(np.uint32),
        }
        return out


class Scene:

    def __init__(self, device_index=0, instancing=None):
        self._h = C.c_void_p()
        check(lib().sr_scene_create(C.c_int(device_index), C.byref(self._h)))
        self.device_index = device_index
        if instancing is not None:
            self.set_instancing(instancing)

    def close(self):
        if getattr(self, "_h", None):
            lib().sr_scene_destroy(self._h)
            self._h = None

    def __del__(self):
        try:
            self.close()
        except Exception:
            pass

    def add_mesh(self, key, vertices, indices, material):
        v = np.ascontiguousarray(vertices, dtype=abi.VERTEX)
        i = np.ascontiguousarray(indices, dtype=np.uint32)
        m = np.ascontiguousarray(material, dtype=abi.MATERIAL)
        slot = C.c_uint32()
        check(lib().sr_scene_add_mesh(self._h, C.c_uint64(key), _p(v), C.c_uint32(len(v)), _p(i), C.c_uint32(len(i)), _p(m), C.byref(slot)))
        return slot.value

    def add_blas(self, key, vertices, indices, material, emissive):
        v = np.ascontiguousarray(vertices, dtype=abi.VERTEX)
        i = np.ascontiguousarray(indices, dtype=np.uint32)
        m = np.ascontiguousarray(material, dtype=abi.MATERIAL)
        e = np.ascontiguousarray(emissive, dtype=abi.EMISSIVE_TRIANGLE)
        slot = C.c_uint32()
        check(lib().sr_scene_add_blas(self._h, C.c_uint64(key), _p(v), C.c_uint32(len(v)), _p(i), C.c_uint32(len(i)), _p(m),
                                      _p(e) if len(e) else None, C.c_uint32(len(e)), C.byref(slot)))
        return slot.value

    def remove(self, key):
        check(lib().sr_scene_remove(self._h, C.c_uint64(key)))

    def update_mesh(self, key, vertices):
        v = np.ascontiguousarray(vertices, dtype=abi.VERTEX)
        check(lib().sr_scene_update_mesh(self._h, C.c_uint64(key), _p(v), C.c_uint32(len(v))))

    def update_mesh_device(self, key, tensor):
        import torch
        ptr, n = _device_vertices(tensor, self.device_index)
        check(lib().sr_scene_update_mesh_device(self._h, C.c_uint64(key), ptr, C.c_uint32(n),
                                                C.c_void_p(torch.cuda.current_stream(tensor.device).cuda_stream)))

    def mesh_vertex_info(self, key):
        info = abi.SrMeshVertexInfo()
        check(lib().sr_scene_mesh_vertex_info(self._h, C.c_uint64(key), C.byref(info)))
        return info

    def set_mesh_skin(self, key, influences, n_joints):
        if influences is None:
            check(lib().sr_scene_set_mesh_skin(self._h, C.c_uint64(key), None, C.c_uint32(0), C.c_uint32(0)))
            return
        a = _skin_influences(influences)
        check(lib().sr_scene_set_mesh_skin(self._h, C.c_uint64(key), _p(a), C.c_uint32(len(a)), C.c_uint32(int(n_joints))))

    def skin_mesh(self, key, joint_matrices):
        m, n = _joint_matrices(joint_matrices)
        check(lib().sr_scene_skin_mesh(self._h, C.c_uint64(key), _p(m), C.c_uint32(n), self._stream()))

    def mesh_skin_info(self, key):
        info = abi.SrMeshSkinInfo()
        check(lib().sr_scene_mesh_skin_info(self._h, C.c_uint64(key), C.byref(info)))
        return info

    def mesh_update_info(self):
        info = abi.SrMeshUpdateInfo()
        check(lib().sr_scene_mesh_update_info(self._h, C.byref(info)))
        return info

    def set_mesh_build_type(self, key, build_type):
        check(lib().sr_scene_set_mesh_build_type(self._h, C.c_uint64(key), C.c_uint32(build_type)))
        return self

    def set_mesh_tree_build(self, mode):
        check(lib().sr_scene_set_mesh_tree_build(self._h, C.c_uint32({"auto": 0, "host": 1, "device": 2}[mode])))
        return self

    def mesh_tree_info(self):
        info = abi.SrMeshTreeInfo()
        check(lib().sr_scene_mesh_tree_info(self._h, C.byref(info)))
        return info

    def set_tree_height_bound(self, mode, cap=0):
        check(lib().sr_scene_set_tree_height_bound(self._h, C.c_uint32({"refuse": 0, "rebalance": 1}[mode]), C.c_uint32(cap)))
        return self

    def tree_height_info(self, kind):
        info = abi.SrTreeHeightInfo()
        check(lib().sr_scene_tree_height_info(self._h, C.c_uint32(kind), C.byref(info)))
        return info

    def mesh_as_state(self, key):
        bt, st, op = C.c_uint32(), abi.SrAsState(), C.c_uint32()
        check(lib().sr_scene_mesh_as_state(self._h, C.c_uint64(key), C.byref(bt), C.byref(st), C.byref(op)))
        return bt.value, st, op.value

    def read_mesh_tree(self, key):
        nn, nt = C.c_uint32(), C.c_uint32()
        check(lib().sr_scene_read_mesh_tree(self._h, C.c_uint64(key), C.byref(nn), C.byref(nt), None, None, None, None, None))
        nodes = np.zeros((max(nn.value, 1), bvh_layout()[1]), dtype=np.uint32)
        tris, shade = np.zeros((max(nt.value, 1), 12), dtype=np.float32), np.zeros((max(nt.value, 1), 12), dtype=np.float32)
        shade_tex, slot_of_prim = np.zeros((max(nt.value, 1), 24), dtype=np.float32), np.zeros(max(nt.value, 1), dtype=np.uint32)
        check(lib().sr_scene_read_mesh_tree(self._h, C.c_uint64(key), None, None, _p(nodes), _p(tris), _p(shade), _p(shade_tex), _p(slot_of_prim)))
        return {"nodes": nodes[:nn.value], "tris": tris[:nt.value], "shade": shade[:nt.value], "shade_tex": shade_tex[:nt.value],
                "slot_of_prim": slot_of_prim[:nt.value]}

    def add_image(self, pixels):
        a = np.ascontiguousarray(pixels, dtype=np.uint8)
        h, w = a.shape[0], a.shape[1]
        ch = 1 if a.ndim == 2 else a.shape[2]
        slot = C.c_uint32()
        check(lib().sr_scene_add_image(self._h, _p(a), C.c_uint32(w), C.c_uint32(h), C.c_uint32(ch), C.byref(slot)))
        return slot.value

    def add_sampler(self, min_filter, mag_filter, address_mode_u, address_mode_v):
        d = abi.SrSamplerDesc(min_filter, mag_filter, address_mode_u, address_mode_v)
        slot = C.c_uint32()
        check(lib().sr_scene_add_sampler(self._h, C.byref(d), C.byref(slot)))
        return slot.value

    def set_instances(self, instances):
        keys = np.array([k for k, _ in instances], dtype=np.uint64)
        counts = np.array([len(t) for _, t in instances], dtype=np.uint32)
        xf = np.array([np.asarray(t, dtype=np.float32).reshape(12) for _, ts in instances for t in ts], dtype=np.float32).reshape(-1, 12)
        if len(xf) == 0:
            xf = np.zeros((1, 12), dtype=np.float32)
        check(lib().sr_scene_set_instances(self._h, _p(keys), _p(counts), C.c_uint32(len(keys)), _p(np.ascontiguousarray(xf))))

    def tile_row_costs(self, which, width, y0, rows):
        out = np.zeros((rows + 7) // 8 + 1, dtype=np.float64)
        n = C.c_uint32()
        check(lib().sr_scene_read_tile_row_costs(self._h, C.c_int(which), C.c_uint32(width), C.c_uint32(y0), C.c_uint32(rows), _p(out),
                                                 C.c_uint32(len(out)), C.byref(n)))
        return out[:n.value]

    def tile_costs(self, which, width, y0, rows):
        out = np.zeros(((width + 7) // 8) * ((rows + 7) // 8), dtype=np.uint32)
        n = C.c_uint32()
        check(lib().sr_scene_read_tile_costs(self._h, C.c_int(which), C.c_uint32(width), C.c_uint32(y0), C.c_uint32(rows), _p(out),
                                             C.c_uint32(len(out)), C.byref(n)))
        return out[:n.value]

    def set_tile_costs(self, which, x0, width, y0, rows, costs):
        c = None if costs is None else np.ascontiguousarray(costs, dtype=np.uint32).reshape(-1)
        check(lib().sr_scene_set_tile_costs(self._h, C.c_int(which), C.c_uint32(x0), C.c_uint32(width), C.c_uint32(y0), C.c_uint32(rows),
                                            None if c is None else _p(c), C.c_uint32(0 if c is None else len(c))))
        return self

    def tile_order(self, which, x0, width, y0, rows):
        tiles_x, tiles_y = (width + 7) // 8, (rows + 7) // 8
        out = np.zeros(8 * max(tiles_x, 1) * max(tiles_y, 1), dtype=np.uint32)
        cap = C.c_uint32()
        check(lib().sr_scene_read_tile_order(self._h, C.c_int(which), C.c_uint32(x0), C.c_uint32(width), C.c_uint32(y0), C.c_uint32(rows),
                                             _p(out), C.c_uint32(len(out)), C.byref(cap)))
        return out[:8 * cap.value].reshape(8, cap.value).copy(), cap.value

    def set_instancing(self, mode):
        check(lib().sr_scene_set_instancing(self._h, C.c_uint32({"auto": 0, "flat": 1, "two_level": 2}[mode])))
        return self

    def two_level(self):
        now = C.c_uint32()
        check(lib().sr_scene_instancing(self._h, None, C.byref(now)))
        return bool(now.value)

    def set_top_level_build(self, mode):
        check(lib().sr_scene_set_top_level_build(self._h, C.c_uint32({"auto": 0, "host": 1, "device": 2}[mode])))
        return self

    def top_level_info(self):
        info = abi.SrTopLevelInfo()
        check(lib().sr_scene_top_level_info(self._h, C.byref(info)))
        return info

    def read_top_level(self):
        info = self.top_level_info()
        nodes = np.zeros((max(info.n_nodes, 1), bvh_layout()[1]), dtype=np.uint32)
        tl_inst = np.zeros(max(info.n_boxes, 1), dtype=np.uint32)
        records = np.zeros(max(info.n_instances, 1), dtype=abi.TL_INSTANCE)
        boxes = np.zeros((max(info.n_instances, 1), 6), dtype=np.float32)
        check(lib().sr_scene_read_top_level(self._h, _p(nodes), _p(tl_inst), _p(records), _p(boxes)))
        return nodes[:info.n_nodes], tl_inst[:info.n_boxes], records[:info.n_instances], boxes[:info.n_instances]

    def force_next_op(self, op):
        check(lib().sr_scene_force_next_op(self._h, C.c_uint32(op)))

    def end_frame(self):
        check(lib().sr_scene_end_frame(self._h))

    def as_state(self):
        st, op = abi.SrAsState(), C.c_uint32()
        check(lib().sr_scene_as_state(self._h, C.byref(st), C.byref(op)))
        return st, op.value

    def read_bvh(self):
        st = self.bvh_stats()
        nodes = np.zeros((st.n_nodes, bvh_layout()[1]), dtype=np.uint32)
        tris = np.zeros((max(st.n_triangles, 1), 12), dtype=np.float32)
        check(lib().sr_scene_read_bvh(self._h, _p(nodes), _p(tris)))
        return nodes, tris[:st.n_triangles]

    def load(self, desc):
        for img in desc.images:
            self.add_image(img)
        for smp in desc.samplers:
            self.add_sampler(*smp)
        for m in desc.meshes:
            self.add_mesh(m.key, m.vertices, m.indices, m.material)
        self.set_instances(desc.instances)
        return self

    def tables(self):
        tp, ip, ep, mp = C.c_void_p(), C.c_void_p(), C.c_void_p(), C.c_void_p()
        nt, nl, ne, nm = C.c_uint32(), C.c_uint32(), C.c_uint32(), C.c_uint32()
        check(lib().sr_scene_get_tables(self._h, C.byref(tp), C.byref(nt), C.byref(ip), C.byref(nl), C.byref(ep), C.byref(ne), C.byref(mp), C.byref(nm)))

        def arr(ptr, n, dt):
            if n == 0:
                return np.zeros(0, dtype=dt)
            buf = (C.c_char * (n * dt.itemsize)).from_address(ptr.value)
            return np.frombuffer(buf, dtype=dt).copy()
        return {"transforms": arr(tp, nt.value, abi.TRANSFORM), "indirection": arr(ip, nl.value, abi.EMISSIVE_INDIRECTION),
                "emissive_triangles": arr(ep, ne.value, abi.EMISSIVE_TRIANGLE), "num_lights": nl.value,
                "meshes_info": arr(mp, nm.value, abi.MESH_INFO)}

    def bvh_stats(self):
        s = abi.SrBvhStats()
        check(lib().sr_scene_bvh_stats(self._h, C.byref(s)))
        return s

    @staticmethod
    def _stream():
        import torch
        return C.c_void_p(torch.cuda.current_stream().cuda_stream)

    def trace_closest(self, rays_t, n):
        import torch
        hits = torch.empty(n, 4, dtype=torch.float32, device=rays_t.device)
        check(lib().sr_trace_closest(self._h, C.c_void_p(rays_t.data_ptr()), C.c_uint32(n), C.c_void_p(hits.data_ptr()), self._stream()))
        return hits

# ... 480 lines not shown
```

Measured before the change: 6383 Mray/s.

## Store per-axis node scales as floats, fix ray bounds, reuse reservoir target pdfs

The BVH node layout now stores each axis scale as a full float in spare dwords (3, 10, 11) instead of packed 8-bit exponents, which removes the shift/mask decode in the inner box test. Closest-hit traversal gets compile-time tmin/tmax constants, so it skips the related shuffles during work stealing. The ReSTIR paths keep the winning candidate's target pdf from merge_reservoirs instead of re-evaluating the light BRDF after each merge. Wave ballots are split into ANDs of simpler ballots. The new layout depends on dwords 10 and 11 being unused padding in the plane area, and the reservoir change assumes the held pdf matches what re-evaluation would return.

Result: faster. 6582 Mray/s (median of 6 runs) (+3.1%).

```diff
diff --git a/sunray_amd/csrc/bvh_build.cpp b/sunray_amd/csrc/bvh_build.cpp
--- a/sunray_amd/csrc/bvh_build.cpp
+++ b/sunray_amd/csrc/bvh_build.cpp
@@ -251,7 +251,7 @@
         max_depth = std::max(max_depth, depth);
         uint32_t plane[6 * srl::kPlaneDwords];
         for (auto& v : plane) v = 0u;
-        uint32_t exps = 0;
+        uint32_t scale_bits[3] = {0u, 0u, 0u};
         float origin[3] = {0.0f, 0.0f, 0.0f};
         if (n_real > 0) {
             for (int a = 0; a < 3; a++) {
@@ -273,7 +273,7 @@
                     e++;
                 }
                 const float scale = std::ldexp(1.0f, e);
-                exps |= (uint32_t)(e + 127) << (8 * a);
+                scale_bits[a] = (uint32_t)(e + 127) << 23;
                 for (int i = 0; i < W; i++) {
                     uint32_t ql = 255u, qh = 0u;
                     if (i < nk && real[i]) {
@@ -292,7 +292,7 @@
         } else {
             for (int a = 0; a < 3; a++) {
                 for (int d = 0; d < srl::kPlaneDwords; d++) { plane[a * srl::kPlaneDwords + d] = 0xFFFFFFFFu; plane[(3 + a) * srl::kPlaneDwords + d] = 0u; }
-                exps |= 127u << (8 * a);
+                scale_bits[a] = 127u << 23;
             }
         }
         uint32_t below = 0;
@@ -308,7 +308,8 @@
             }
         }
         uint32_t* q = &out[self];
-        memcpy(q + 0, origin, 12); q[3] = exps;
+        memcpy(q + 0, origin, 12);
+        for (int a = 0; a < 3; a++) q[srl::kScaleOffset[a]] = scale_bits[a];
         memcpy(q + srl::kPlaneOffset, plane, sizeof(plane));
         memcpy(q + srl::kChildOffset, refs, sizeof(refs));
         return below + (uint32_t)std::max(n_real - 1, 0);
diff --git a/sunray_amd/csrc/bvh_gpu.hip b/sunray_amd/csrc/bvh_gpu.hip
--- a/sunray_amd/csrc/bvh_gpu.hip
+++ b/sunray_amd/csrc/bvh_gpu.hip
@@ -146,7 +146,7 @@
         n_real++;
         for (int a = 0; a < 3; a++) { lo_n[a] = fminf(lo_n[a], lo[c][a]); hi_n[a] = fmaxf(hi_n[a], hi[c][a]); }
     }
-    uint32_t plane[6 * srl::kPlaneDwords], exps = 0;
+    uint32_t plane[6 * srl::kPlaneDwords], scale_bits[3] = {0u, 0u, 0u};
     for (int k = 0; k < 6 * srl::kPlaneDwords; k++) plane[k] = 0u;
     float origin[3] = {0.0f, 0.0f, 0.0f};
     if (n_real > 0) {
@@ -169,7 +169,7 @@
                 if (ok) break;
             }
             const float scale = ldexpf(1.0f, e);
-            exps |= (uint32_t)(e + 127) << (8 * a);
+            scale_bits[a] = (uint32_t)(e + 127) << 23;
             for (int c = 0; c < W; c++) {
                 uint32_t ql = 255u, qh = 0u;
                 if (real[c]) {
@@ -188,10 +188,11 @@
     } else {
         for (int a = 0; a < 3; a++) {
             for (int d = 0; d < srl::kPlaneDwords; d++) { plane[a * srl::kPlaneDwords + d] = 0xFFFFFFFFu; plane[(3 + a) * srl::kPlaneDwords + d] = 0u; }
-            exps |= 127u << (8 * a);
-        }
-    }
-    q[0] = __float_as_uint(origin[0]); q[1] = __float_as_uint(origin[1]); q[2] = __float_as_uint(origin[2]); q[3] = exps;
+            scale_bits[a] = 127u << 23;
+        }
+    }
+    q[0] = __float_as_uint(origin[0]); q[1] = __float_as_uint(origin[1]); q[2] = __float_as_uint(origin[2]);
+    q[srl::kScaleOffset[0]] = scale_bits[0]; q[srl::kScaleOffset[1]] = scale_bits[1]; q[srl::kScaleOffset[2]] = scale_bits[2];
     for (int k = 0; k < 6 * srl::kPlaneDwords; k++) q[srl::kPlaneOffset + k] = plane[k];
     float* b = node_box + (size_t)node * 6;
     for (int a = 0; a < 3; a++) { b[a] = lo_n[a]; b[3 + a] = hi_n[a]; }
diff --git a/sunray_amd/csrc/bvh_layout.h b/sunray_amd/csrc/bvh_layout.h
--- a/sunray_amd/csrc/bvh_layout.h
+++ b/sunray_amd/csrc/bvh_layout.h
@@ -4,6 +4,7 @@
 constexpr int kPlaneDwords = kBvhWidth / 4;
 constexpr int kPlaneOffset = 4;
 constexpr int kChildOffset = 12;
+constexpr int kScaleOffset[3] = {3, 10, 11};
 constexpr int kNodeDwords = 16;
 constexpr int kNodeBytes = kNodeDwords * 4;
 #ifndef SR_LEAF_MAX
diff --git a/sunray_amd/csrc/kernels.hip b/sunray_amd/csrc/kernels.hip
--- a/sunray_amd/csrc/kernels.hip
+++ b/sunray_amd/csrc/kernels.hip
@@ -105,13 +105,13 @@
 SRD uint32_t counted_closest(uint32_t n_q) { return (n_q >> 16) & 0x7FFFu; }
 
 template <int V, bool ANY>
-SRD bool trace_ray(PixelCtx& cx, bool want, f3 o, f3 d, float tmin, float tmax, TravHit& h) {
-    return traverse_ws<ANY, (V & 1) != 0, (V & 4) != 0>(cx.a.sc, want, o, d, tmin, tmax, h, cx.stack, kPassBlock, cx.st);
+SRD bool trace_ray(PixelCtx& cx, bool want, f3 o, f3 d, float tmax, TravHit& h) {
+    return traverse_ws<ANY, (V & 1) != 0, (V & 4) != 0, true, !ANY>(cx.a.sc, want, o, d, kPassTmin, ANY ? tmax : kPassTmax, h, cx.stack, kPassBlock, cx.st);
 }
 template <int V>
-SRD Payload trace_closest_shaded(PixelCtx& cx, f3 o, f3 d, float tmin, float tmax) {
+SRD Payload trace_closest_shaded(PixelCtx& cx, f3 o, f3 d) {
     TravHit h;
-    trace_ray<V, false>(cx, true, o, d, tmin, tmax, h);
+    trace_ray<V, false>(cx, true, o, d, kPassTmax, h);
     cx.n_q += kCountClosest;
     return shade_hit<(V & 2) != 0, (V & 4) != 0>(cx.a.sc, h);
 }
@@ -120,7 +120,7 @@
     if (dist > 0.002f) {
         TravHit h;
         cx.n_q += kCountAny;
-        return trace_ray<V, true>(cx, true, o, d, 0.001f, dist - 0.001f, h) ? 1.0f : -1.0f;
+        return trace_ray<V, true>(cx, true, o, d, dist - 0.001f, h) ? 1.0f : -1.0f;
     }
     return -1.0f;
 }
@@ -311,9 +311,9 @@
 }
 
 template <int V, bool ANY>
-SRD bool ws_query(PixelCtx& cx, bool want, f3 o, f3 d, float tmin, float tmax, TravHit& h) {
+SRD bool ws_query(PixelCtx& cx, bool want, f3 o, f3 d, float tmax, TravHit& h) {
     if (want) cx.n_q += ANY ? kCountAny : kCountClosest;
-    return trace_ray<V, ANY>(cx, want, o, d, tmin, tmax, h);
+    return trace_ray<V, ANY>(cx, want, o, d, tmax, h);
 }
 
 template <int V>
@@ -348,7 +348,7 @@
         float virtual_distance = 0.0f;
 
         for (uint32_t vb = 0; vb < a.cfg.virtual_bounces; vb++) {
-            prd = trace_closest_shaded<V>(cx, rayOrigin, rayDir, 0.001f, 10000.0f);
+            prd = trace_closest_shaded<V>(cx, rayOrigin, rayDir);
             if (vb == 0u && a.primary_payload) store_payload(a.primary_payload + pix, prd);
             if (prd.dist < 0.0f) break;
             hitPos = rayOrigin + rayDir * prd.dist;
@@ -407,6 +407,7 @@
             SrReservoir current_r; zero_reservoir(current_r);
             const uint32_t num_lights = sc.num_lights;
             if (num_lights > 0 && roughness > 0.2f) {
+                float p_hat_held = 0.0f;
                 for (uint32_t i = 0; i < a.cfg.ris_candidates; i++) {
                     uint32_t cand_idx = (uint32_t)(rnd(rng) * (float)num_lights);
                     if (cand_idx > num_lights - 1) cand_idx = num_lights - 1;
@@ -427,13 +428,10 @@
                         current_r.light_idx = cand_idx;
                         st3(current_r.light_pos, cand_pos);
                         st3(current_r.light_normal, cand_normal);
+                        p_hat_held = p_hat;
                     }
                 }
-                if (current_r.w_sum > 0.0f) {
-                    const f3 fw = eval_unshadowed_light(hitPos, hit_normal, V_view, hit_albedo, roughness, metallic,
-                                                        light_emission(sc, current_r.light_idx), ld3(current_r.light_pos), ld3(current_r.light_normal));
-                    current_r.W = current_r.w_sum / fmaxf(current_r.M * maxc(fw), 0.0001f);
-                }
+                if (current_r.w_sum > 0.0f) current_r.W = current_r.w_sum / fmaxf(current_r.M * p_hat_held, 0.0001f);
                 if (a.frame_count > 0 && prev_valid) {
                     const float ppx = prev_u * (float)W, ppy = prev_v * (float)H;
                     const float j0 = rnd(rng), j1 = rnd(rng);
@@ -453,10 +451,8 @@
                             const f3 fh = eval_unshadowed_light(hitPos, hit_normal, V_view, hit_albedo, roughness, metallic,
                                                                 light_emission(sc, history_r.light_idx), ld3(history_r.light_pos), ld3(history_r.light_normal));
                             const float hist_rand = rnd(rng);
-                            merge_reservoirs(current_r, history_r, maxc(fh), hist_rand);
-                            const f3 fm = eval_unshadowed_light(hitPos, hit_normal, V_view, hit_albedo, roughness, metallic,
-                                                                light_emission(sc, current_r.light_idx), ld3(current_r.light_pos), ld3(current_r.light_normal));
-                            current_r.W = current_r.w_sum / fmaxf(current_r.M * maxc(fm), 0.0001f);
+                            if (merge_reservoirs(current_r, history_r, maxc(fh), hist_rand)) p_hat_held = maxc(fh);
+                            current_r.W = current_r.w_sum / fmaxf(current_r.M * p_hat_held, 0.0001f);
                         }
                     }
                 }
@@ -481,7 +477,7 @@
             const float gi_NdotL = fmaxf(dot3(hit_normal, gi_dir), 0.0f);
             if (gi_NdotL > 0.0f) {
                 const f3 gi_origin = hitPos + hit_normal * 0.001f;
-                prd = trace_closest_shaded<V>(cx, gi_origin, gi_dir, 0.001f, 10000.0f);
+                prd = trace_closest_shaded<V>(cx, gi_origin, gi_dir);
                 f3 sample_pos = splat(0.0f), sample_normal = splat(0.0f), sample_radiance = splat(0.0f);
                 if (prd.dist > 0.0f) {
                     sample_pos = gi_origin + gi_dir * prd.dist;
@@ -591,7 +587,7 @@
     for (int bounce = 0; bounce < BOUNCES; bounce++) {
         if (__builtin_amdgcn_ballot_w64(in_loop) == 0ull) break;
         const bool reuse_primary = bounce == 0 && a.primary_payload != nullptr;
-        if (!reuse_primary) ws_query<V, false>(cx, in_loop, rayOrigin, rayDir, 0.001f, 10000.0f, h);
+        if (!reuse_primary) ws_query<V, false>(cx, in_loop, rayOrigin, rayDir, kPassTmax, h);
         bool do_restir = false, do_nee = false, do_bounce = false;
         f3 hit_normal = splat(0.0f), hit_albedo = splat(0.0f), hitPos = splat(0.0f), V_view = splat(0.0f);
         float roughness = 0.5f, metallic = 0.0f;
@@ -656,7 +652,7 @@
                     const f3 fc = eval_unshadowed_light(hitPos, hit_normal, V_view, hit_albedo, roughness, metallic,
                                                         light_emission(sc, center_r.light_idx), ld3(center_r.light_pos), ld3(center_r.light_normal));
                     const float cr = rnd(rng);
-                    merge_reservoirs(spatial_r, center_r, maxc(fc), cr);
+                    if (merge_reservoirs(spatial_r, center_r, maxc(fc), cr)) f_y_winner = fc;
                 }
                 const float current_depth = len3(hitPos - origin);
                 for (int s = 0; s < 5; s++) {
@@ -678,12 +674,10 @@
                         const f3 fn = eval_unshadowed_light(hitPos, hit_normal, V_view, hit_albedo, roughness, metallic,
                                                             light_emission(sc, nr.light_idx), ld3(nr.light_pos), ld3(nr.light_normal));
                         const float nrnd = rnd(rng);
-                        merge_reservoirs(spatial_r, nr, maxc(fn), nrnd);
+                        if (merge_reservoirs(spatial_r, nr, maxc(fn), nrnd)) f_y_winner = fn;
                     }
                 }
                 if (spatial_r.w_sum > 0.0f) {
-                    f_y_winner = eval_unshadowed_light(hitPos, hit_normal, V_view, hit_albedo, roughness, metallic,
-                                                       light_emission(sc, spatial_r.light_idx), ld3(spatial_r.light_pos), ld3(spatial_r.light_normal));
                     spatial_r.W = spatial_r.w_sum / fmaxf(spatial_r.M * maxc(f_y_winner), 1e-3f);
                     spatial_r.W = fminf(spatial_r.W, 50.0f);
                     shadow_dir = ld3(spatial_r.light_pos) - hitPos;
@@ -692,7 +686,7 @@
                     if (dot3(hit_normal, shadow_dir) > 0.0f) { di_pending = true; want_di = shadow_dist > 0.002f; }
                 }
             }
-            occ = ws_query<V, true>(cx, want_di, hitPos, shadow_dir, 0.001f, shadow_dist - 0.001f, h);
+            occ = ws_query<V, true>(cx, want_di, hitPos, shadow_dir, shadow_dist - 0.001f, h);
             if (di_pending) {
                 prd.dist = want_di ? (occ ? 1.0f : -1.0f) : -1.0f;
                 if (prd.dist < 0.0f) radiance = radiance + f_y_winner * throughput * spatial_r.W;
@@ -753,7 +747,7 @@
                         }
                     }
                 }
-                occ = ws_query<V, true>(cx, want_g, hitPos, gi_spatial_dir, 0.001f, d_new - 0.001f, h);
+                occ = ws_query<V, true>(cx, want_g, hitPos, gi_spatial_dir, d_new - 0.001f, h);
                 if (cand) {
                     prd.dist = want_g ? (occ ? 1.0f : -1.0f) : -1.0f;
                     if (!(prd.dist >= 0.0f)) {
@@ -784,7 +778,7 @@
                     }
                 }
             }
-            occ = ws_query<V, true>(cx, want_gif, hitPos, gi_x2_dir, 0.001f, gi_x2_dist - 0.001f, h);
+            occ = ws_query<V, true>(cx, want_gif, hitPos, gi_x2_dir, gi_x2_dist - 0.001f, h);
             if (gif_pending) {
                 prd.dist = want_gif ? (occ ? 1.0f : -1.0f) : -1.0f;
                 if (prd.dist < 0.0f) {
@@ -820,7 +814,7 @@
                 cos_theta_surface = fmaxf(dot3(hit_normal, shadow_ray_dir), 0.0f);
                 if (cos_theta_light > 0.0f && cos_theta_surface > 0.0f) { nee_pending = true; want_nee = light_dist > 0.002f; }
             }
-            occ = ws_query<V, true>(cx, want_nee, hitPos, shadow_ray_dir, 0.001f, light_dist - 0.001f, h);
+            occ = ws_query<V, true>(cx, want_nee, hitPos, shadow_ray_dir, light_dist - 0.001f, h);
             if (nee_pending) {
                 prd.dist = want_nee ? (occ ? 1.0f : -1.0f) : -1.0f;
                 if (prd.dist < 0.0f) {
diff --git a/sunray_amd/csrc/rt_device.h b/sunray_amd/csrc/rt_device.h
--- a/sunray_amd/csrc/rt_device.h
+++ b/sunray_amd/csrc/rt_device.h
@@ -307,15 +307,17 @@
     f3 contrib = sample_radiance * f_diffuse * NdotL;
     return maxc(contrib);
 }
-SRD void merge_reservoirs(SrReservoir& r, const SrReservoir& nr, float p_hat_new, float random_val) {
+SRD bool merge_reservoirs(SrReservoir& r, const SrReservoir& nr, float p_hat_new, float random_val) {
     r.M += nr.M;
     float weight = p_hat_new * nr.W * nr.M;
     r.w_sum += weight;
-    if (random_val < (weight / fmaxf(r.w_sum, 0.0001f))) {
+    const bool taken = random_val < (weight / fmaxf(r.w_sum, 0.0001f));
+    if (taken) {
         r.light_idx = nr.light_idx;
         r.light_pos[0] = nr.light_pos[0]; r.light_pos[1] = nr.light_pos[1]; r.light_pos[2] = nr.light_pos[2];
         r.light_normal[0] = nr.light_normal[0]; r.light_normal[1] = nr.light_normal[1]; r.light_normal[2] = nr.light_normal[2];
     }
+    return taken;
 }
 SRD bool merge_reservoirs_gi(SrReservoirGI& r, const SrReservoirGI& nr, float p_hat_new, float jacobian, float random_val) {
     r.M += nr.M;
diff --git a/sunray_amd/csrc/traverse.h b/sunray_amd/csrc/traverse.h
--- a/sunray_amd/csrc/traverse.h
+++ b/sunray_amd/csrc/traverse.h
@@ -155,8 +155,13 @@
     return t0 <= fminf(far, t_hi);
 }
 
-template <bool ANY, bool STATS, bool TL = false>
+SRD unsigned long long ballot(bool p) { return __builtin_amdgcn_ballot_w64(p); }
+
+constexpr float kPassTmin = 0.001f, kPassTmax = 10000.0f;
+template <bool ANY, bool STATS, bool TL = false, bool FIXED_TMIN = false, bool FIXED_TMAX = false>
 SRD bool traverse_ws(const DevScene& sc, bool want, f3 o, f3 d, float tmin, float tmax, TravHit& hit, int* lds_col, int stride, TravStats& st) {
+    if (FIXED_TMIN) tmin = kPassTmin;
+    if (FIXED_TMAX) tmax = kPassTmax;
     const float4* __restrict__ nodes = sc.nodes;
     const float4* __restrict__ tris = sc.tris;
     const uint32_t tid = threadIdx.x, lane = tid & 63u;
@@ -195,16 +200,16 @@
         for (;;) {
             const bool inner = node != kSentinel && (node >= 0 || (TL && !in_blas));
             {
-                const unsigned long long walking = __builtin_amdgcn_ballot_w64(inner && leaf == 0);
+                const unsigned long long walking = ballot(inner) & ballot(leaf == 0);
                 if (walking == 0ull) break;
                 if ((int)__popcll(walking) <= kEarlyTriWalking &&
-                    (int)__popcll(__builtin_amdgcn_ballot_w64(node != kSentinel && node < 0 && leaf != 0 && (!TL || in_blas))) >= kEarlyTriBlocked) break;
+                    (int)__popcll(ballot(node != kSentinel && node < 0 && (!TL || in_blas)) & ballot(leaf != 0)) >= kEarlyTriBlocked) break;
             }
             const bool idle = node == kSentinel && leaf == 0;
-            const unsigned long long idle_mask = __builtin_amdgcn_ballot_w64(idle);
+            const unsigned long long idle_mask = ballot(node == kSentinel) & ballot(leaf == 0);
             if (idle_mask != 0ull) {
                 const bool can_give = node != kSentinel && sp > sb;
-                const unsigned long long donor_mask = __builtin_amdgcn_ballot_w64(can_give);
+                const unsigned long long donor_mask = ballot(node != kSentinel) & ballot(sp > sb);
                 if (donor_mask != 0ull) {
                     const uint32_t n = min((uint32_t)__popcll(idle_mask), (uint32_t)__popcll(donor_mask));
                     const uint32_t drank = lanes_below(donor_mask), irank = lanes_below(idle_mask);
@@ -216,7 +221,8 @@
                     const uint32_t d_root = (uint32_t)__shfl((int)root, dl);
                     const float ox = __shfl(o.x, dl), oy = __shfl(o.y, dl), oz = __shfl(o.z, dl);
                     const float dx = __shfl(d.x, dl), dy = __shfl(d.y, dl), dz = __shfl(d.z, dl);
-                    const float d_tmin = __shfl(tmin, dl), d_tmax = __shfl(tmax, dl), d_cull = __shfl(cull, dl);
+                    const float d_tmin = FIXED_TMIN ? kPassTmin : __shfl(tmin, dl), d_tmax = FIXED_TMAX ? kPassTmax : __shfl(tmax, dl);
+                    const float d_cull = __shfl(cull, dl);
                     const float ix = __shfl(rs.inv.x, dl), iy = __shfl(rs.inv.y, dl), iz = __shfl(rs.inv.z, dl);
                     bool d_blas = false;
                     uint32_t d_inst = 0u;
@@ -273,7 +279,7 @@
                 const float4 h0 = n[0], q1 = n[1], q2 = n[2], qc = n[3];
                 const int4 child = make_int4(__float_as_int(qc.x), __float_as_int(qc.y), __float_as_int(qc.z), __float_as_int(qc.w));
                 if (STATS) st.boxes += 4;
-                const uint32_t ex = __float_as_uint(h0.w);
+                const float sx = h0.w, sy = q2.z, sz = q2.w;
                 const uint32_t LX = __float_as_uint(q1.x), LY = __float_as_uint(q1.y), LZ = __float_as_uint(q1.z);
                 const uint32_t HX = __float_as_uint(q1.w), HY = __float_as_uint(q2.x), HZ = __float_as_uint(q2.y);
                 const bool sgx = __float_as_int(rs.inv.x) < 0, sgy = __float_as_int(rs.inv.y) < 0, sgz = __float_as_int(rs.inv.z) < 0;
@@ -284,8 +290,7 @@
                     p.nx = sgx ? HX : LX; p.fx = sgx ? LX : HX;
                     p.ny = sgy ? HY : LY; p.fy = sgy ? LY : HY;
                     p.nz = sgz ? HZ : LZ; p.fz = sgz ? LZ : HZ;
-                    p.ax = __uint_as_float((ex & 0xFFu) << 23) * rs.inv.x; p.ay = __uint_as_float(((ex >> 8) & 0xFFu) << 23) * rs.inv.y;
-                    p.az = __uint_as_float(((ex >> 16) & 0xFFu) << 23) * rs.inv.z;
+                    p.ax = sx * rs.inv.x; p.ay = sy * rs.inv.y; p.az = sz * rs.inv.z;
                     const float bx = (h0.x - ro.x) * rs.inv.x, by = (h0.y - ro.y) * rs.inv.y, bz = (h0.z - ro.z) * rs.inv.z;
                     p.bnx = bx - pad.x; p.bfx = bx + pad.x; p.bny = by - pad.y; p.bfy = by + pad.y; p.bnz = bz - pad.z; p.bfz = bz + pad.z;
                     b0 = child_hit_tl<0>(p, t_lo, cull, n0) && child.x != -1;
@@ -297,8 +302,7 @@
                     p.nx = sgx ? HX : LX; p.fx = sgx ? LX : HX;
                     p.ny = sgy ? HY : LY; p.fy = sgy ? LY : HY;
                     p.nz = sgz ? HZ : LZ; p.fz = sgz ? LZ : HZ;
-                    p.ax = __uint_as_float((ex & 0xFFu) << 23) * rs.inv.x; p.ay = __uint_as_float(((ex >> 8) & 0xFFu) << 23) * rs.inv.y;
-                    p.az = __uint_as_float(((ex >> 16) & 0xFFu) << 23) * rs.inv.z;
+                    p.ax = sx * rs.inv.x; p.ay = sy * rs.inv.y; p.az = sz * rs.inv.z;
                     p.bx = (h0.x - o.x) * rs.inv.x; p.by = (h0.y - o.y) * rs.inv.y; p.bz = (h0.z - o.z) * rs.inv.z;
                     b0 = child_hit<0>(p, t_lo, cull, n0);
                     b1 = child_hit<1>(p, t_lo, cull, n1);
diff --git a/sunray_amd/runtime.py b/sunray_amd/runtime.py
--- a/sunray_amd/runtime.py
+++ b/sunray_amd/runtime.py
@@ -116,8 +116,7 @@
     W, _, po, co = bvh_layout()
     n = np.asarray(node, dtype=np.uint32)
     origin = n[0:3].view(np.float32)
-    ex = int(n[3])
-    scale = np.array([np.uint32(((ex >> (8 * a)) & 0xFF) << 23) for a in range(3)], dtype=np.uint32).view(np.float32)
+    scale = n[[3, 10, 11]].view(np.float32)
     pd = W // 4
     lo = np.zeros((W, 3), np.float32)
     hi = np.zeros((W, 3), np.float32)
```
